# chrischoy/DeepGlobalRegistration

Measured on AMD Instinct MI355X. Metric: pair registrations/sec (FCGF x2 + 1-NN + 6-D inlier net + gate + weighted Procrustes + SE(3) refinement), higher is better.
Workload: dtype f32 results via 2 x f16 split operands (3 f16 MFMA products per MAC, f32 accumulate); k = 1 convs, kNN re-evaluation and registration in exact f32, SVD in f64

## Files before the change

### deepglobalregistration_amd/_lib.py

```python
import ctypes as C
import os
import threading

import torch

_HERE = os.path.dirname(os.path.abspath(__file__))
LIB_PATH = os.environ.get('DGR_HIP_LIB') or os.path.join(_HERE, 'lib', 'libdgr_hip.so')

DGR_OK, DGR_EINVAL, DGR_EHIP, DGR_ENOMEM, DGR_ESVD, DGR_EINTERNAL = 0, -1, -2, -3, -4, -5
STATUS_OK, STATUS_LOW_CONFIDENCE, STATUS_SVD_FAILED, STATUS_SAFEGUARD = 0, 1, 2, 3
STATUS_FLAG_ICP_SKIPPED, STATUS_MASK = 0x100, 0xff

c_i32p, c_i64p, c_f32p, c_f64p = (C.POINTER(C.c_int32), C.POINTER(C.c_int64),
                                  C.POINTER(C.c_float), C.POINTER(C.c_double))
vp = C.c_void_p


class WeightDesc(C.Structure):
    _fields_ = [('name', C.c_char_p), ('data', vp), ('numel', C.c_int64)]


class Params(C.Structure):
    _fields_ = [('clip_weight_thresh', C.c_float), ('voxel_size', C.c_float),
                ('inlier_feature_type', C.c_int), ('max_iter', C.c_int),
                ('max_break_count', C.c_int), ('break_threshold_ratio', C.c_double),
                ('skip_refinement', C.c_int), ('safeguard', C.c_int), ('ransac_hypotheses', C.c_int64),
                ('ransac_seed', C.c_uint32), ('use_icp', C.c_int)]


class PgParams(C.Structure):
    _fields_ = [('mu', C.c_double), ('reference_node', C.c_int), ('max_iter', C.c_int), ('rel_tol', C.c_double)]


SIGNATURES = {
    'dgr_last_error': (C.c_char_p, []),
    'dgr_version': (C.c_char_p, []),
    'dgr_ctx_create': (C.c_int, [C.c_int, C.POINTER(vp)]),
    'dgr_ctx_destroy': (None, [vp]),
    'dgr_ctx_workspace_bytes': (C.c_int64, [vp]),
    'dgr_ctx_create_partition_stream': (C.c_int, [vp, C.c_int, C.c_int, C.POINTER(vp)]),
    'dgr_voxelize': (C.c_int, [vp, vp, C.c_int, C.c_int64, C.c_double, C.c_int32, vp, vp, vp, c_i64p, vp]),
    'dgr_net_create': (C.c_int, [vp, C.c_int, C.c_int, C.c_int, C.c_int, C.c_int,
                                 C.POINTER(WeightDesc), C.c_int, C.POINTER(vp)]),
    'dgr_net_create_device': (C.c_int, [vp, C.c_int, C.c_int, C.c_int, C.c_int, C.c_int,
                                        C.POINTER(WeightDesc), C.c_int, C.POINTER(vp)]),
    'dgr_net_destroy': (None, [vp]),
    'dgr_net_param_bytes': (C.c_int64, [vp]),
    'dgr_net_share': (C.c_int, [vp, vp, C.POINTER(vp)]),
    'dgr_net_sharers': (C.c_int, [vp]),
    'dgr_resunet_forward': (C.c_int, [vp, vp, vp, vp, C.c_int64, vp, vp]),
    'dgr_net_get_intermediate': (C.c_int, [vp, vp, C.c_char_p, vp, C.c_int64, c_i64p, c_i64p]),
    'dgr_net_layer_stats': (C.c_int, [vp, vp, C.c_int, c_i64p]),
    'dgr_net_num_layers': (C.c_int, [vp]),
    'dgr_net_rerun_layer': (C.c_int, [vp, vp, C.c_int, C.c_int, c_f32p, c_f32p]),
    'dgr_maps_create': (C.c_int, [vp, vp, C.c_int64, C.c_int, C.c_int, C.POINTER(vp), vp]),
    'dgr_maps_destroy': (None, [vp]),
    'dgr_maps_get_coords': (C.c_int, [vp, C.c_int, vp, C.c_int64, c_i64p]),
    'dgr_maps_get_kernel_map': (C.c_int, [vp, C.c_int, C.c_int, vp, C.c_int64, vp, vp, C.c_int64,
                                          c_i64p, c_i64p]),
    'dgr_knn1_l2': (C.c_int, [vp, vp, C.c_int64, vp, C.c_int64, C.c_int, C.c_int, vp, vp, vp]),
    'dgr_knn1_l2_batch': (C.c_int, [vp, vp, c_i64p, vp, c_i64p, C.c_int, C.c_int, C.c_int, vp, vp, vp]),
    'dgr_knn_l2': (C.c_int, [vp, vp, C.c_int64, vp, C.c_int64, C.c_int, C.c_int, C.c_int, vp, vp, vp]),
    'dgr_knn_l2_batch': (C.c_int, [vp, vp, c_i64p, vp, c_i64p, C.c_int, C.c_int, C.c_int, C.c_int, vp, vp,
                                   vp]),
    'dgr_inlier_inputs': (C.c_int, [vp, vp, vp, C.c_int64, vp, vp, C.c_int64, vp, C.c_int, vp, vp, vp]),
    'dgr_sigmoid_clip_sum': (C.c_int, [vp, vp, C.c_int64, C.c_float, vp, c_f64p, vp]),
    'dgr_gather_rows3': (C.c_int, [vp, vp, vp, C.c_int64, vp, vp]),
    'dgr_weighted_procrustes': (C.c_int, [vp, vp, vp, vp, C.c_int64, C.c_float, c_f32p, c_f32p, vp]),
    'dgr_se3_refine': (C.c_int, [vp, vp, vp, vp, C.c_int64, C.c_float, C.c_int, C.c_int, C.c_double,
                                 c_f32p, c_f32p, c_i32p, c_f32p, c_i32p, vp]),
    'dgr_register_batch': (C.c_int, [vp, vp, vp, vp, vp, c_i64p, vp, vp, c_i64p, C.c_int,
                                     C.POINTER(Params), vp, vp, c_f32p, c_i32p, c_f32p, vp]),
    'dgr_register_pairs': (C.c_int, [vp, vp, vp, vp, vp, c_i64p, C.c_int, C.c_int, c_i32p, C.c_int,
                                     C.POINTER(Params), vp, vp, c_f32p, c_i32p, c_f32p, vp]),
    'dgr_register_batch_f64': (C.c_int, [vp, c_f64p, C.c_int64, c_i64p]),
    'dgr_register_batch_output': (C.c_int, [vp, C.c_int, vp, C.c_int64, c_i64p, vp]),
    'dgr_ctx_set_profiling': (C.c_int, [vp, C.c_int]),
    'dgr_icp_point_to_point': (C.c_int, [vp, vp, C.c_int64, vp, C.c_int64, C.c_double, c_f64p, C.c_int, C.c_double,
                                          C.c_double, c_f64p, c_f64p, vp]),
    'dgr_ransac_correspondence': (C.c_int, [vp, vp, vp, C.c_int64, C.c_double, C.c_int64, C.c_uint32, c_f64p, c_f64p, vp]),
    'dgr_ctx_stage_times': (C.c_int, [vp, c_f32p]),
    'dgr_ctx_stage_times_v2': (C.c_int, [vp, c_f32p, C.c_int, C.POINTER(C.c_int)]),
    'dgr_ctx_conv_launches': (C.c_int64, [vp]),
    'dgr_ctx_conv_launch_times': (C.c_int, [vp, c_f32p, c_f32p, C.c_int64, C.POINTER(C.c_int64)]),
    'dgr_ctx_conv_launch_kernel_us': (C.c_int, [vp, c_f32p, C.c_int64, C.POINTER(C.c_int64)]),
    'dgr_ctx_conv_launch_kinds': (C.c_int, [vp, C.c_char_p, C.c_int64, C.POINTER(C.c_int64)]),
    'dgr_radius_pairs_batch': (C.c_int, [vp, vp, c_i64p, vp, c_i64p, C.c_int, c_f64p, C.c_double, C.c_int, vp, vp,
                                         C.c_int64, c_i64p, vp]),
    'dgr_pairs_isin_batch': (C.c_int, [vp, vp, c_i64p, vp, c_i64p, C.c_int, c_i64p, vp, vp]),
    'dgr_validation_counts': (C.c_int, [vp, vp, vp, C.c_float, c_i64p, C.c_int, c_i64p, vp]),
    'dgr_score_pairs': (C.c_int, [vp, vp, c_i64p, C.c_int, c_i32p, C.c_int, c_f64p, C.c_double, c_f64p, vp]),
    'dgr_pose_graph_optimize': (C.c_int, [vp, C.c_int, c_i64p, c_i64p, c_i32p, c_f64p, c_f64p, C.POINTER(C.c_uint8), c_f64p,
                                          C.POINTER(PgParams), c_f64p, c_f64p, c_f64p, vp]),
    'dgr_voxel_mean': (C.c_int, [vp, vp, C.c_int, c_i64p, C.c_int, c_i32p, C.c_int, c_f64p, c_f64p, C.c_double, vp, vp, vp, vp,
                                 vp, c_i64p, c_i64p, vp]),
    'dgr_tsdf_fragment': (C.c_int, [vp, vp, C.c_int, C.c_int, C.c_int, c_f64p, c_f64p, c_f64p, C.c_double, C.c_double,
                                    C.c_double, C.c_double, C.c_int, C.c_int, C.c_int, vp, C.c_int64, vp, vp, vp, C.c_int64,
                                    c_i64p, c_i64p, c_i64p, vp]),
    'dgr_debug_ortho2rotation': (C.c_int, [vp, vp, C.c_int64, vp, vp, vp, vp]),
    'dgr_debug_se3_refine_from': (C.c_int, [vp, vp, vp, vp, C.c_int64, C.c_float, C.c_int, C.c_int, C.c_double,
                                            c_f64p, c_f64p, vp]),
    'dgr_debug_smooth_l1': (C.c_int, [vp, vp, vp, C.c_int64, C.c_float, vp, vp]),
    'dgr_debug_conv_layer': (C.c_int, [vp, vp, C.c_int, vp, vp, C.c_int, C.c_int64, vp, vp]),
}

_lib = None


def load():
    global _lib
    if _lib is not None:
        return _lib
    if not os.path.exists(LIB_PATH):
        raise RuntimeError(
            f'{LIB_PATH} not found: the HIP extension is not built.  Run '
            '`python -c "import __graft_entry__ as g; g.build()"` (or `make -C '
            'deepglobalregistration_amd/csrc`).  There is no CPU fallback.')
    lib = C.CDLL(LIB_PATH)
    for name, (res, args) in SIGNATURES.items():
        fn = getattr(lib, name)
        fn.restype = res
        fn.argtypes = args
    _lib = lib
    return lib


class DgrError(RuntimeError):
    def __init__(self, code, message):
        super().__init__(f'libdgr_hip error {code}: {message}')
        self.code = code


class DgrInvalidArgument(DgrError, ValueError):

    def __init__(self, message):
        RuntimeError.__init__(self, f'libdgr_hip: {message}')
        self.code = DGR_EINVAL


def check(rc):
    if rc == DGR_OK:
        return
    msg = load().dgr_last_error().decode('utf-8', 'replace')
    if rc == DGR_EINVAL:
        raise DgrInvalidArgument(msg)
    raise DgrError(rc, msg)


_ctxs = {}
_tls = threading.local()


def new_ctx(device):
    lib = load()
    device = torch.device(device)
    idx = device.index if device.index is not None else torch.cuda.current_device()
    h = vp()
    check(lib.dgr_ctx_create(idx, C.byref(h)))
    return h


def use_ctx(handle):
    _tls.ctx = handle


def get_ctx(device=None):
    lib = load()
    if getattr(_tls, 'ctx', None) is not None:
        return _tls.ctx
    if not torch.cuda.is_available():
        raise RuntimeError('deepglobalregistration_amd needs a ROCm GPU (torch.cuda.is_available() is '
                           'False); there is no CPU fallback')
    if device is None:
        idx = torch.cuda.current_device()
    else:
        device = torch.device(device)
        if device.type != 'cuda':
            raise RuntimeError(f'deepglobalregistration_amd runs on the GPU only, got device {device}')
        idx = device.index if device.index is not None else torch.cuda.current_device()
    if idx not in _ctxs:
        h = vp()
        check(lib.dgr_ctx_create(idx, C.byref(h)))
        _ctxs[idx] = h
    return _ctxs[idx]


def stream_ptr(device_index=None):
    return vp(torch.cuda.current_stream(device_index).cuda_stream)


def ptr(t):
    if t is None:
        return vp(0)
    assert t.is_contiguous(), 'tensor must be contiguous'
    return vp(t.data_ptr())
```

### deepglobalregistration_amd/csrc/conv_dense.hip

```cpp
#include "dgr_internal.h"
#include "split.h"

typedef float f32x4 __attribute__((ext_vector_type(4)));
typedef float f32x2 __attribute__((ext_vector_type(2)));
typedef int i32x4 __attribute__((ext_vector_type(4)));
typedef _Float16 f16x8 __attribute__((ext_vector_type(8)));
typedef _Float16 f16x2 __attribute__((ext_vector_type(2)));
typedef unsigned int u32x2 __attribute__((ext_vector_type(2)));
typedef unsigned int u32x4 __attribute__((ext_vector_type(4)));

#ifndef DGR_DENSE_RG
#define DGR_DENSE_RG 2
#endif
#ifndef DGR_DENSE_RG32
#define DGR_DENSE_RG32 2
#endif
#ifndef DGR_DENSE_WD
#define DGR_DENSE_WD 8
#endif
struct ConvDenseArgs {
  const float *in;
  float *out;
  const float *shift, *res;
  const u32x4 *wb;
  int64_t piece_stride;
  const int32_t *nbr, *n_out_dev;
  int64_t n_pad;
  int in_ld, in_relu, out_ld, out_relu, res_ld, res_relu;
  const uint32_t *row_amax;
  uint32_t *out_amax, *out_amax2;
  float w_unscale;
  uint32_t in_bytes;
  const unsigned char *in_ds;
  unsigned char *out_ds;
};

template <int CIN, int COUT, int RG, int WAVES, bool PS>
__global__ void __launch_bounds__(64 * WAVES, 2) sparse_conv_dense_f16x2(ConvDenseArgs a) {
  constexpr int KV = 27;
  constexpr int S = CIN / 32, NCB = COUT / 16;
  constexpr int THREADS = 64 * WAVES;
  constexpr int MB = WAVES * RG * 16;
  constexpr int NST = S * NCB;
  constexpr int WD = NST >= 8 ? DGR_DENSE_WD : NST >= 4 ? 4 : 2;
  static_assert(NST % WD == 0, "the weight ring turns a whole number of times per offset (static register indexing)");
  __shared__ int nbr_s[KV][MB];

  const int tid = threadIdx.x, lane = tid & 63;
  const int wave = __builtin_amdgcn_readfirstlane(tid >> 6);
  const int n_out = *a.n_out_dev;
  const int nblocks = (n_out + MB - 1) / MB;
  const int per = (nblocks + 7) >> 3;
  const int j = blockIdx.x >> 3;
  const int blk = (blockIdx.x & 7) * per + j;
  if (j >= per || blk >= nblocks) return;
  const int64_t row0 = (int64_t)blk * MB;

  u32x4 rh[WD], rm[WD];
  const u32x4 *wph = a.wb + lane, *wpm = a.wb + a.piece_stride + lane;
  auto wreq = [&](int g, int i) {
    const int gc = min(g, KV * NST - 1);
    const int k = gc / NST, jj = gc - k * NST;
    const int gg = k * NST + (jj % S) * NCB + jj / S;
    rh[i] = wph[(int64_t)gg * 64];
    rm[i] = wpm[(int64_t)gg * 64];
  };
  for (int e = tid; e < KV * MB; e += THREADS) {
    const int k = e / MB, r = e - k * MB;
    nbr_s[k][r] = (row0 + r < n_out) ? a.nbr[(int64_t)k * a.n_pad + row0 + r] : -1;
  }
  const int lr = lane & 15, lq = lane >> 4;
  f32x4 total[RG][NCB];
#pragma unroll
  for (int cb = 0; cb < NCB; ++cb) {
    const f32x4 sh = a.shift ? *reinterpret_cast<const f32x4 *>(a.shift + 16 * cb + 4 * lq) : f32x4{0.f, 0.f, 0.f, 0.f};
#pragma unroll
    for (int rg = 0; rg < RG; ++rg) {
      f32x4 v = sh;
      const int64_t row = row0 + (wave * RG + rg) * 16 + lr;
      if (a.res && row < n_out) {
        f32x4 x = *reinterpret_cast<const f32x4 *>(a.res + row * a.res_ld + 16 * cb + 4 * lq);
        if (a.res_relu) { x.x = fmaxf(x.x, 0.f); x.y = fmaxf(x.y, 0.f); x.z = fmaxf(x.z, 0.f); x.w = fmaxf(x.w, 0.f); }
        v += x;
      }
      total[rg][cb] = v;
    }
  }
  __syncthreads();

  const __amdgpu_buffer_rsrc_t in_rsrc = __builtin_amdgcn_make_buffer_rsrc(
      PS ? (void *)const_cast<unsigned char *>(a.in_ds) : (void *)const_cast<float *>(a.in), 0, a.in_bytes, 0x00020000);
  struct RowSet { f32x4 raw[RG][S][2]; uint32_t mx[RG]; int nv[RG]; };
  auto gather = [&](int k, RowSet &g) {
#pragma unroll
    for (int rg = 0; rg < RG; ++rg) {
      const int n = nbr_s[k][(wave * RG + rg) * 16 + (lane >> 2)];
      const int ne = max(n, 0);
      const uint32_t off = n >= 0 ? (uint32_t)n * (uint32_t)((PS ? CIN : a.in_ld) * 4) + 16u * (lane & 3) : a.in_bytes;
      const uint32_t mv = a.row_amax[ne];
#pragma unroll
      for (int s = 0; s < S; ++s) {
        if constexpr (PS) {
          g.raw[rg][s][0] = __builtin_bit_cast(f32x4, __builtin_amdgcn_raw_buffer_load_b128(in_rsrc, off + 64 * s, 0, 0));
          g.raw[rg][s][1] = __builtin_bit_cast(f32x4, __builtin_amdgcn_raw_buffer_load_b128(in_rsrc, off + 2 * CIN + 64 * s, 0, 0));
        } else {
          g.raw[rg][s][0] = __builtin_bit_cast(f32x4, __builtin_amdgcn_raw_buffer_load_b128(in_rsrc, off + 128 * s, 0, 0));
          g.raw[rg][s][1] = __builtin_bit_cast(f32x4, __builtin_amdgcn_raw_buffer_load_b128(in_rsrc, off + 128 * s + 64, 0, 0));
        }
      }
      g.mx[rg] = mv;
      g.nv[rg] = n;
    }
  };
  constexpr int DEPTH = 1;
  static_assert(DEPTH == 1 || DEPTH == 2, "prefetch depth");
  RowSet gA, gB;
  gather(0, gA);
  if (DEPTH == 2) gather(1, gB);
#pragma unroll
  for (int i = 0; i < WD; ++i) wreq(i, i);
  const int relu_lo = a.in_relu ? 0 : (int)0x80000000;

  auto body = [&](int k, RowSet &g) {
    f16x8 bh[RG][S], bm[RG][S];
    float fold[RG];
    const int from = 4 * (4 * (lane & 15) + (lane >> 4));
#pragma unroll
    for (int rg = 0; rg < RG; ++rg) {
      const float sx = g.nv[rg] >= 0 ? dgr_row_scale_of(g.mx[rg]) : 0.f;
      const float fl = sx != 0.f ? dgr_inv_pow2(sx) * a.w_unscale : 0.f;
      fold[rg] = __builtin_bit_cast(float, __builtin_amdgcn_ds_bpermute(16 * (lane & 15), __builtin_bit_cast(int, fl)));
#pragma unroll
      for (int s = 0; s < S; ++s) {
        i32x4 hw, mw;
        if constexpr (PS) {
          hw = __builtin_bit_cast(i32x4, g.raw[rg][s][0]);
          mw = __builtin_bit_cast(i32x4, g.raw[rg][s][1]);
        } else
#pragma unroll
        for (int h = 0; h < 2; ++h) {
          const i32x4 v = __builtin_bit_cast(i32x4, g.raw[rg][s][h]);
#pragma unroll
          for (int u = 0; u < 4; u += 2) {
            const f32x2 xs = f32x2{__builtin_bit_cast(float, max(v[u], relu_lo)), __builtin_bit_cast(float, max(v[u + 1], relu_lo))} * sx;
            const f16x2 hh = __builtin_convertvector(xs, f16x2);
            const f16x2 mm = __builtin_convertvector(xs - __builtin_convertvector(hh, f32x2), f16x2);
            hw[2 * h + u / 2] = __builtin_bit_cast(int, hh);
            mw[2 * h + u / 2] = __builtin_bit_cast(int, mm);
          }
        }
#pragma unroll
        for (int d = 0; d < 4; ++d) {
          hw[d] = __builtin_amdgcn_ds_bpermute(from, hw[d]);
          mw[d] = __builtin_amdgcn_ds_bpermute(from, mw[d]);
        }
        bh[rg][s] = __builtin_bit_cast(f16x8, hw);
        bm[rg][s] = __builtin_bit_cast(f16x8, mw);
      }
    }
    __builtin_amdgcn_sched_barrier(0);
    gather(min(k + DEPTH, KV - 1), g);
    __builtin_amdgcn_sched_barrier(0);
    f32x4 prev[RG];
#pragma unroll
    for (int cb = 0; cb < NCB; ++cb) {
      f32x4 tmp[RG];
#pragma unroll
      for (int rg = 0; rg < RG; ++rg) tmp[rg] = f32x4{0.f, 0.f, 0.f, 0.f};
#pragma unroll
      for (int s = 0; s < S; ++s) {
        const int j = cb * S + s;
        const f16x8 wh = __builtin_bit_cast(f16x8, rh[j % WD]);
        const f16x8 wm = __builtin_bit_cast(f16x8, rm[j % WD]);
#pragma unroll
        for (int rg = 0; rg < RG; ++rg) tmp[rg] = __builtin_amdgcn_mfma_f32_16x16x32_f16(wm, bh[rg][s], tmp[rg], 0, 0, 0);
#pragma unroll
        for (int rg = 0; rg < RG; ++rg) tmp[rg] = __builtin_amdgcn_mfma_f32_16x16x32_f16(wh, bm[rg][s], tmp[rg], 0, 0, 0);
#pragma unroll
        for (int rg = 0; rg < RG; ++rg) tmp[rg] = __builtin_amdgcn_mfma_f32_16x16x32_f16(wh, bh[rg][s], tmp[rg], 0, 0, 0);
        wreq(k * NST + j + WD, j % WD);
        if (s == 0 && cb > 0) {
#pragma unroll
          for (int rg = 0; rg < RG; ++rg) total[rg][cb - 1] += prev[rg] * fold[rg];
        }
        __builtin_amdgcn_sched_barrier(0);
      }
#pragma unroll
      for (int rg = 0; rg < RG; ++rg) prev[rg] = tmp[rg];
    }
#pragma unroll
    for (int rg = 0; rg < RG; ++rg) total[rg][NCB - 1] += prev[rg] * fold[rg];
  };
  if (DEPTH == 1) {
#pragma unroll 1
    for (int k = 0; k < KV; ++k) body(k, gA);
  } else {
#pragma unroll 1
    for (int k = 0; k < KV - 1; k += 2) {
      body(k, gA);
      body(k + 1, gB);
    }
    body(KV - 1, gA);
  }

  const float out_lo = a.out_relu ? 0.f : -__builtin_inff();
  const int out_relu_lo = a.out_relu ? 0 : (int)0x80000000;
#pragma unroll
  for (int rg = 0; rg < RG; ++rg) {
    const int64_t row = row0 + (wave * RG + rg) * 16 + lr;
    uint32_t mx = 0;
#pragma unroll
    for (int cb = 0; cb < NCB; ++cb) {
      f32x4 v = total[rg][cb];
      v.x = fmaxf(v.x, out_lo); v.y = fmaxf(v.y, out_lo); v.z = fmaxf(v.z, out_lo); v.w = fmaxf(v.w, out_lo);
      total[rg][cb] = v;
      if (row < n_out) {
        if (a.out) *reinterpret_cast<f32x4 *>(a.out + row * a.out_ld + 16 * cb + 4 * lq) = v;
        const i32x4 b = __builtin_bit_cast(i32x4, v);
        mx = max(mx, max(max((uint32_t)b.x & 0x7fffffffu, (uint32_t)b.y & 0x7fffffffu), max((uint32_t)b.z & 0x7fffffffu, (uint32_t)b.w & 0x7fffffffu)));
      }
    }
    if (a.out_amax || a.out_amax2 || a.out_ds) {
      mx = max(mx, (uint32_t)__shfl_xor((int)mx, 16, 64));
      mx = max(mx, (uint32_t)__shfl_xor((int)mx, 32, 64));
      if (lq == 0 && row < n_out) {
        if (a.out_amax) atomicMax(a.out_amax + row, mx);
        if (a.out_amax2) atomicMax(a.out_amax2 + row, mx);
      }
    }
    if (a.out_ds && row < n_out) {
      const float sx = dgr_row_scale_of(mx);
      unsigned char *dst = a.out_ds + row * (int64_t)(4 * COUT) + 16 * lq;
#pragma unroll
      for (int s = 0; s < COUT / 32; ++s) {
        u32x4 hw, mw;
#pragma unroll
        for (int h = 0; h < 2; ++h) {
          const i32x4 v = __builtin_bit_cast(i32x4, total[rg][2 * s + h]);
#pragma unroll
          for (int u = 0; u < 4; u += 2) {
            const f32x2 xs = f32x2{__builtin_bit_cast(float, max(v[u], out_relu_lo)), __builtin_bit_cast(float, max(v[u + 1], out_relu_lo))} * sx;
            const f16x2 hh = __builtin_convertvector(xs, f16x2);
            const f16x2 mm = __builtin_convertvector(xs - __builtin_convertvector(hh, f32x2), f16x2);
            hw[2 * h + u / 2] = __builtin_bit_cast(uint32_t, hh);
            mw[2 * h + u / 2] = __builtin_bit_cast(uint32_t, mm);
          }
        }
        *reinterpret_cast<u32x4 *>(dst + 64 * s) = hw;
        *reinterpret_cast<u32x4 *>(dst + 2 * COUT + 64 * s) = mw;
      }
    }
  }
}

bool dgr_conv_dense_supported(int cin, int cin_pad, int cout) {
  return cin == cin_pad && (cin == 32 || cin == 64) && (cout == 32 || cout == 64);
}

template <int CIN, int COUT>
static int launch_dense(const ConvDenseArgs &ka, int64_t n_out_cap, hipStream_t stream) {
  constexpr int RG = (CIN == 32 && COUT == 32) ? DGR_DENSE_RG32 : DGR_DENSE_RG, WAVES = 4, MB = WAVES * RG * 16;
  int64_t blocks = dgr_ceil_div(n_out_cap, MB);
  blocks = (blocks + 7) / 8 * 8;
  if (ka.in_ds)
    sparse_conv_dense_f16x2<CIN, COUT, RG, WAVES, true><<<(unsigned)blocks, 64 * WAVES, 0, stream>>>(ka);
  else
    sparse_conv_dense_f16x2<CIN, COUT, RG, WAVES, false><<<(unsigned)blocks, 64 * WAVES, 0, stream>>>(ka);
  DGR_LAUNCH_CHECK();
  return DGR_OK;
}

int dgr_conv_dense_launch(const DgrConvOsLaunch &a, hipStream_t stream, const char **kernel_name) {
  DGR_REQUIRE(a.nbr && a.nbr->built && a.nbr->K == 27, "dense-tile conv: no neighbour table");
  DGR_REQUIRE(dgr_conv_dense_supported(a.cin, a.cin_pad, a.cout), "dense-tile conv: Cin = %d, Cout = %d not built", a.cin, a.cout);
  DGR_REQUIRE(a.wbd && a.row_amax, "dense-tile conv: needs the split weights in its operand order and the input rows' maxima");
  DGR_REQUIRE((a.in_ld & 3) == 0 && (a.out_ld & 3) == 0 && (a.res == nullptr || (a.res_ld & 3) == 0),
              "dense-tile conv: row strides must be multiples of 4");
  ConvDenseArgs ka;
  ka.in = a.in; ka.out = a.out; ka.shift = a.shift; ka.res = a.res;
  ka.wb = static_cast<const u32x4 *>(a.wbd); ka.piece_stride = a.piece_stride;
  ka.nbr = a.nbr->nbr; ka.n_out_dev = a.n_out_dev; ka.n_pad = a.nbr->n_pad;
  ka.in_ld = a.in_ld; ka.in_relu = a.in_relu; ka.out_ld = a.out_ld; ka.out_relu = a.out_relu;
  ka.res_ld = a.res_ld; ka.res_relu = a.res_relu;
  ka.row_amax = a.row_amax; ka.w_unscale = a.w_unscale;
  ka.out_amax = a.out_amax; ka.out_amax2 = a.out_amax2;
  ka.in_ds = a.in_dsplit; ka.out_ds = a.out_dsplit;
  DGR_REQUIRE(a.out || a.out_dsplit, "dense-tile conv: no output");
  DGR_REQUIRE(a.n_in_cap > 0 && a.n_in_cap * (int64_t)a.in_ld * 4 < (1ll << 31), "dense-tile conv: input tensor beyond 2 GB");
  ka.in_bytes = (uint32_t)(a.n_in_cap * (int64_t)(a.in_dsplit ? a.cin : a.in_ld) * 4);
#define DGR_DENSE(CI, CO)                                                                   \
  if (a.cin == CI && a.cout == CO) {                                                        \
    if (kernel_name) *kernel_name = a.in_dsplit ? "sparse_conv_dense_f16x2<" #CI ", " #CO ", ps>" : "sparse_conv_dense_f16x2<" #CI ", " #CO ">"; \
    return launch_dense<CI, CO>(ka, a.n_out_cap, stream);                                   \
  }
  DGR_DENSE(32, 32) DGR_DENSE(32, 64) DGR_DENSE(64, 32) DGR_DENSE(64, 64)
#undef DGR_DENSE
  return DGR_EINVAL;
}
```

### deepglobalregistration_amd/csrc/conv_os.hip

```cpp
#include <stdlib.h>

#include <type_traits>

#include "dgr_internal.h"
#include "split.h"

typedef float f32x4 __attribute__((ext_vector_type(4)));
typedef int i32x4 __attribute__((ext_vector_type(4)));
typedef unsigned int u32x2 __attribute__((ext_vector_type(2)));
typedef __bf16 bf16x8 __attribute__((ext_vector_type(8)));
typedef _Float16 f16x8 __attribute__((ext_vector_type(8)));
typedef _Float16 f16x2 __attribute__((ext_vector_type(2)));

#ifdef DGR_OS_STAGE_CLK
__device__ unsigned long long dgr_os_stage_clk[8];
#define DGR_OS_CLK(i) do { if (threadIdx.x == 0) { const unsigned long long t_ = __builtin_amdgcn_s_memrealtime(); atomicAdd(&dgr_os_stage_clk[i], t_ - t_prev); t_prev = t_; } } while (0)
extern "C" int dgr_debug_os_stage_clk(unsigned long long *out8, int reset) {
  if (out8 && hipMemcpyFromSymbol(out8, HIP_SYMBOL(dgr_os_stage_clk), 8 * sizeof(unsigned long long)) != hipSuccess) return -1;
  if (reset) { unsigned long long z[8] = {0, 0, 0, 0, 0, 0, 0, 0}; if (hipMemcpyToSymbol(HIP_SYMBOL(dgr_os_stage_clk), z, sizeof(z)) != hipSuccess) return -1; }
  return 0;
}
#else
#define DGR_OS_CLK(i) do { } while (0)
#endif
// ... 5 lines not shown
  int64_t piece_stride;
  const int32_t *nbr, *n_out_dev;
  int64_t n_pad;
  int in_ld, in_relu, out_ld, out_relu, res_ld, res_relu;
  int cin, cout, nb16;
  const uint32_t *row_amax;
  float w_unscale;
  uint32_t *out_amax, *out_amax2;
};

template <int CP, int CS, int MB, int CK, int TM, int PM, int GW>
__global__ void __launch_bounds__(CS * 4 * (TM / 16 / GW)) sparse_conv_os(ConvOsArgs a) {
  constexpr bool BF3 = PM != 0;
  static_assert(PM == 0 || PM == 2, "arithmetic mode");
  constexpr int NP = PM == 0 ? 1 : 2;
  constexpr int GP = TM / 16;
  constexpr int NCW = CS / 16;
  constexpr int NWR = GP / GW;
  static_assert(GP % GW == 0, "groups per wave must divide the groups per tile");
  constexpr int NW = NCW * NWR;
  constexpr int THREADS = 64 * NW;
  constexpr int KV = 27;
  constexpr int PPT = CP / CK;
  constexpr int LDA = CK + 4, LDC = CS + 4;
  constexpr int C4K = CK / 4;
  constexpr int NCH = (TM * C4K + THREADS - 1) / THREADS;
  constexpr bool PIECE_GUARD = TM * C4K % THREADS != 0;
  constexpr int G = CK / 16;
  constexpr int GT = CP / 16;
  constexpr int KPW = (KV + NW - 1) / NW;
  constexpr int NGMAX = KV * ((MB / 16 + GP - 1) / GP * GP) + GP;
  static_assert(CP % CK == 0, "shape");
  constexpr int LDP = CK + 8;
  constexpr int PLANE = TM * LDP;
  constexpr int G32 = CK / 32;
  constexpr int ABYTES = BF3 ? 2 * NP * PLANE * 2 : 2 * TM * LDA * 4;
  __shared__ __attribute__((aligned(16))) char abuf[ABYTES];
  float (*As)[TM][LDA] = reinterpret_cast<float (*)[TM][LDA]>(abuf);
  unsigned short *Ps = reinterpret_cast<unsigned short *>(abuf);
  __shared__ __attribute__((aligned(16))) float acc_s[MB][LDC];
  __shared__ int in_idx[KV][MB];
  __shared__ float in_scale[PM == 2 ? KV : 1][MB];
  __shared__ unsigned char out_loc[KV][MB];
  __shared__ int cnt[KV];
  __shared__ int grp[NGMAX + GP];
  __shared__ int n_grp;

  const int tid = threadIdx.x;
  const int lane = tid & 63;
  const int wave = __builtin_amdgcn_readfirstlane(tid >> 6);
  const int cw = wave % NCW;
  const int rb0 = (wave / NCW) * GW;
  const int n_out = *a.n_out_dev;
  const int nblocks = (n_out + MB - 1) / MB;
  const int per = (nblocks + 7) >> 3;
  const int j = blockIdx.x >> 3;
  const int blk = (blockIdx.x & 7) * per + j;
  if (j >= per || blk >= nblocks) return;
  const int slice = blockIdx.y;
  const int64_t row0 = (int64_t)blk * MB;
#ifdef DGR_OS_STAGE_CLK
  unsigned long long t_prev = __builtin_amdgcn_s_memrealtime();
#endif

  if constexpr (PM == 2)
    for (int e = tid; e < KV * MB; e += THREADS) (&in_scale[0][0])[e] = 1.f;
  __syncthreads();
  {
    int v[KPW];
#pragma unroll
    for (int u = 0; u < KPW; ++u) {
      const int k = wave + u * NW;
      v[u] = (k < KV && lane < MB) ? a.nbr[(int64_t)k * a.n_pad + row0 + lane] : -1;
    }
#pragma unroll
    for (int u = 0; u < KPW; ++u) {
      const int k = wave + u * NW;
      if (k < KV) {
        const unsigned long long m = __ballot(v[u] >= 0);
        if (v[u] >= 0) {
          const int pos = __popcll(m & ((1ull << lane) - 1ull));
          in_idx[k][pos] = v[u];
          out_loc[k][pos] = (unsigned char)lane;
          if constexpr (PM == 2) in_scale[k][pos] = dgr_row_scale_of(a.row_amax[v[u]]);
        }
        if (lane == 0) cnt[k] = __popcll(m);
      }
    }
  }
  DGR_OS_CLK(0);
  for (int e = tid; e < MB * (CS / 4); e += THREADS) {
    const int r = e / (CS / 4), c = (e % (CS / 4)) * 4;
    f32x4 v = a.shift ? *reinterpret_cast<const f32x4 *>(a.shift + slice * CS + c) : f32x4{0.f, 0.f, 0.f, 0.f};
    if (a.res && row0 + r < n_out) {
      f32x4 x = *reinterpret_cast<const f32x4 *>(a.res + (row0 + r) * a.res_ld + slice * CS + c);
      if (a.res_relu) { x.x = fmaxf(x.x, 0.f); x.y = fmaxf(x.y, 0.f); x.z = fmaxf(x.z, 0.f); x.w = fmaxf(x.w, 0.f); }
      v += x;
    }
    *reinterpret_cast<f32x4 *>(&acc_s[r][c]) = v;
  }
  __syncthreads();
  if (wave == 0) {
    const int c = lane < KV ? cnt[lane] : 0;
    const int ng = NWR > 1 ? (((c + 15) >> 4) + GP - 1) / GP * GP : ((c + 15) >> 4);
    int x = ng;
#pragma unroll
    for (int d = 1; d < 32; d <<= 1) {
      const int y = __shfl_up(x, d, 64);
      if (lane >= d) x += y;
    }
    const int first = x - ng;
    for (int u = 0; u < ng; ++u) grp[first + u] = lane | ((16 * u) << 8) | (max(0, min(16, c - 16 * u)) << 16);
    if (lane == KV - 1) {
      n_grp = x;
      for (int u = 0; u < GP; ++u) grp[x + u] = 0;
    }
  }
  __syncthreads();
  const int NG = n_grp;
  const int NT = (NG + GP - 1) / GP;
  const int NQ = NT * PPT;
  DGR_OS_CLK(1);

  f32x4 Gr[NCH];
  auto gather = [&](int q) {
    const int t = q / PPT, cbase = (q % PPT) * CK;
#pragma unroll
    for (int i = 0; i < NCH; ++i) {
      const int ch = PIECE_GUARD ? min(tid + i * THREADS, TM * C4K - 1) : tid + i * THREADS;
      const int r = ch / C4K, c = cbase + (ch % C4K) * 4;
      const int info = grp[GP * t + (r >> 4)];
      const int row = in_idx[info & 255][((info >> 8) & 255) + (r & 15)];
      const uint32_t off = (uint32_t)(((r & 15) < (info >> 16)) ? row : 0) * (uint32_t)a.in_ld + (uint32_t)c;
      Gr[i] = *reinterpret_cast<const f32x4 *>(a.in + off);
    }
  };
  const int relu_lo = a.in_relu ? 0 : (int)0x80000000;
  auto land = [&](int q) {
#pragma unroll
    for (int i = 0; i < NCH; ++i) {
      const int ch = tid + i * THREADS;
      if (PIECE_GUARD && ch >= TM * C4K) continue;
      i32x4 v = __builtin_bit_cast(i32x4, Gr[i]);
      v.x = max(v.x, relu_lo); v.y = max(v.y, relu_lo); v.z = max(v.z, relu_lo); v.w = max(v.w, relu_lo);
      if constexpr (!BF3) {
        *reinterpret_cast<i32x4 *>(&As[q & 1][0][0] + (ch / C4K) * LDA + (ch % C4K) * 4) = v;
      } else {
        const int r = ch / C4K;
        const int info = grp[GP * (min(q, NQ - 1) / PPT) + (r >> 4)];
        const float sx = in_scale[info & 255][min(((info >> 8) & 255) + (r & 15), MB - 1)];
        _Float16 hh[4], mm[4];
#pragma unroll
        for (int u = 0; u < 4; ++u) {
          const int vi = v[u];
          const float xs = __builtin_bit_cast(float, vi) * sx;
          hh[u] = (_Float16)xs;
          mm[u] = (_Float16)(xs - (float)hh[u]);
        }
        unsigned short *dst = Ps + (q & 1) * NP * PLANE + r * LDP + (ch % C4K) * 4;
        *reinterpret_cast<u32x2 *>(dst) = u32x2{__builtin_bit_cast(uint32_t, f16x2{hh[0], hh[1]}),
                                                __builtin_bit_cast(uint32_t, f16x2{hh[2], hh[3]})};
        *reinterpret_cast<u32x2 *>(dst + PLANE) = u32x2{__builtin_bit_cast(uint32_t, f16x2{mm[0], mm[1]}),
                                                        __builtin_bit_cast(uint32_t, f16x2{mm[2], mm[3]})};
      }
    }
  };
  const int jb = slice * NCW + cw;
  constexpr int WREGS = BF3 ? NP * G32 : G;
  struct WSet { uint4 v[WREGS]; };
  auto wstep = [&](int qq, int u, WSet &w) {
    const int q = min(qq, NQ - 1);
    const int k = __builtin_amdgcn_readfirstlane(grp[GP * (q / PPT) + rb0 + u]) & 255;
    if constexpr (!BF3) {
      const uint4 *p = reinterpret_cast<const uint4 *>(a.w16) + (int64_t)jb * 64 + lane + (int64_t)(k * GT + (q % PPT) * G) * a.nb16 * 64;
#pragma unroll
      for (int g = 0; g < G; ++g) w.v[g] = p[(int64_t)g * a.nb16 * 64];
    } else {
      const uint4 *p = a.wb3 + (int64_t)jb * 64 + lane + (int64_t)(k * (CP / 32) + (q % PPT) * G32) * a.nb16 * 64;
#pragma unroll
      for (int g = 0; g < G32; ++g)
#pragma unroll
        for (int pc = 0; pc < NP; ++pc) w.v[NP * g + pc] = p[(int64_t)pc * a.piece_stride + (int64_t)g * a.nb16 * 64];
    }
  };

  f32x4 acc[GW];
  WSet w[GW];
  auto mfma_group = [&](int u, int buf) {
    const int rb = rb0 + u;
    if constexpr (!BF3) {
      const float *arow = &As[buf][lane & 15][4 * (lane >> 4)];
#pragma unroll
      for (int g = 0; g < G; ++g) {
        const f32x4 av = *reinterpret_cast<const f32x4 *>(arow + rb * 16 * LDA + g * 16);
        const f32x4 wv = __builtin_bit_cast(f32x4, w[u].v[g]);
#pragma unroll
        for (int c = 0; c < 4; ++c) acc[u] = __builtin_amdgcn_mfma_f32_16x16x4f32(wv[c], av[c], acc[u], 0, 0, 0);
      }
    } else {
      const unsigned short *prow = Ps + buf * NP * PLANE + (rb * 16 + (lane & 15)) * LDP + 8 * (lane >> 4);
#pragma unroll
      for (int g = 0; g < G32; ++g) {
        const f16x8 ah = __builtin_bit_cast(f16x8, *reinterpret_cast<const uint4 *>(prow + 32 * g));
        const f16x8 am = __builtin_bit_cast(f16x8, *reinterpret_cast<const uint4 *>(prow + PLANE + 32 * g));
        const f16x8 wh = __builtin_bit_cast(f16x8, w[u].v[2 * g]), wm = __builtin_bit_cast(f16x8, w[u].v[2 * g + 1]);
        acc[u] = __builtin_amdgcn_mfma_f32_16x16x32_f16(wm, ah, acc[u], 0, 0, 0);
        acc[u] = __builtin_amdgcn_mfma_f32_16x16x32_f16(wh, am, acc[u], 0, 0, 0);
        acc[u] = __builtin_amdgcn_mfma_f32_16x16x32_f16(wh, ah, acc[u], 0, 0, 0);
      }
    }
  };
  if (NQ > 0) {
    gather(0);
#pragma unroll
    for (int u = 0; u < GW; ++u) wstep(0, u, w[u]);
    land(0);
    gather(NQ > 1 ? 1 : 0);
  }
  __syncthreads();

  for (int q = 0; q < NQ; ++q) {
    const int t = q / PPT, h = q % PPT;
    land(q + 1);
    gather(min(q + 2, NQ - 1));
    if (PPT == 1 || h == 0) {
#pragma unroll
      for (int u = 0; u < GW; ++u) acc[u] = f32x4{0.f, 0.f, 0.f, 0.f};
    }
#pragma unroll
    for (int u = 0; u < GW; ++u) {
      const int n_rows = __builtin_amdgcn_readfirstlane(grp[GP * t + rb0 + u]) >> 16;
      __builtin_amdgcn_sched_barrier(0);
      if (u == 0 || n_rows > 0) mfma_group(u, q & 1);
      wstep(q + 1, u, w[u]);
    }
    if (PPT == 1 || h == PPT - 1) {
#pragma unroll
      for (int u = 0; u < GW; ++u) {
        const int info = grp[GP * t + rb0 + u];
        if ((lane & 15) < (info >> 16)) {
          const int e = ((info >> 8) & 255) + (lane & 15);
          float *p = &acc_s[out_loc[info & 255][e]][16 * cw + 4 * (lane >> 4)];
          f32x4 v = *reinterpret_cast<f32x4 *>(p);
          if constexpr (PM == 2) {
            const float f = __builtin_bit_cast(float, 0x7f000000u - __builtin_bit_cast(uint32_t, in_scale[info & 255][e])) * a.w_unscale;
            v += acc[u] * f;
          } else {
            v += acc[u];
          }
          *reinterpret_cast<f32x4 *>(p) = v;
        }
      }
    }
    __syncthreads();
  }
  DGR_OS_CLK(2);
#ifdef DGR_OS_STAGE_CLK
  if (threadIdx.x == 0) { atomicAdd(&dgr_os_stage_clk[4], 1ull); atomicAdd(&dgr_os_stage_clk[5], (unsigned long long)NQ); }
#endif
  const float out_lo = a.out_relu ? 0.f : -__builtin_inff();
  static_assert(MB * (CS / 4) % THREADS == 0 || THREADS % (CS / 4) == 0, "row lanes stay inside a wave");
  for (int e0 = 0; e0 < MB * (CS / 4); e0 += THREADS) {
    const int e = e0 + tid;
    const bool live = e < MB * (CS / 4);
    const int r = live ? e / (CS / 4) : 0, c = (e % (CS / 4)) * 4;
    uint32_t mx = 0;
    if (live && row0 + r < n_out) {
      f32x4 v = *reinterpret_cast<const f32x4 *>(&acc_s[r][c]);
      v.x = fmaxf(v.x, out_lo); v.y = fmaxf(v.y, out_lo); v.z = fmaxf(v.z, out_lo); v.w = fmaxf(v.w, out_lo);
      *reinterpret_cast<f32x4 *>(a.out + (row0 + r) * a.out_ld + slice * CS + c) = v;
      const i32x4 b = __builtin_bit_cast(i32x4, v);
      mx = max(max((uint32_t)b.x & 0x7fffffffu, (uint32_t)b.y & 0x7fffffffu), max((uint32_t)b.z & 0x7fffffffu, (uint32_t)b.w & 0x7fffffffu));
    }
    if (a.out_amax || a.out_amax2) {
#pragma unroll
      for (int d = CS / 8; d >= 1; d >>= 1) mx = max(mx, (uint32_t)__shfl_xor((int)mx, d, 64));
      if (live && (e % (CS / 4)) == 0 && row0 + r < n_out) {
        if (a.out_amax) atomicMax(a.out_amax + row0 + r, mx);
        if (a.out_amax2) atomicMax(a.out_amax2 + row0 + r, mx);
      }
    }
  }
  DGR_OS_CLK(3);
}

template <int CP, int CS, int MB, int CK, int TM>
static int launch_os(const ConvOsArgs &ka, int64_t n_out_cap, hipStream_t stream) {
  constexpr int GW = (MB >= 64 && CP <= 64) ? 1 : TM / 16;
  int64_t blocks = dgr_ceil_div(n_out_cap, MB);
  blocks = (blocks + 7) / 8 * 8;
  dim3 grid((unsigned)blocks, (unsigned)(ka.cout / CS));
  constexpr int threads = CS * 4 * (TM / 16 / GW);
  if (ka.wb3 && ka.row_amax)
    sparse_conv_os<CP, CS, MB, CK, TM, 2, GW><<<grid, threads, 0, stream>>>(ka);
  else
    sparse_conv_os<CP, CS, MB, CK, TM, 0, GW><<<grid, threads, 0, stream>>>(ka);
  DGR_LAUNCH_CHECK();
  return DGR_OK;
}

int dgr_conv_os_launch(const DgrConvOsLaunch &a, hipStream_t stream, const char **kernel_name) {
  if (a.dense) return dgr_conv_dense_launch(a, stream, kernel_name);
  if (a.up) return dgr_conv_up_launch(a, stream, kernel_name);
  DGR_REQUIRE(a.nbr && a.nbr->built && a.nbr->K == 27, "output-stationary conv: no neighbour table");
  DGR_REQUIRE((a.cin & 3) == 0 && (a.in_ld & 3) == 0 && (a.out_ld & 3) == 0 && (a.res == nullptr || (a.res_ld & 3) == 0),
              "output-stationary conv: channel counts and row strides must be multiples of 4");
  DGR_REQUIRE(a.cout % 32 == 0 && a.cin == a.cin_pad, "output-stationary conv: Cin = %d, Cout = %d must be multiples of 32",
              a.cin, a.cout);
  DGR_REQUIRE(a.n_in_cap > 0 && a.n_in_cap * (int64_t)a.in_ld < (1ll << 32) / 4 * 4,
              "output-stationary conv: input tensor beyond 32-bit element offsets");
  ConvOsArgs ka;
  ka.in = a.in; ka.out = a.out; ka.w16 = a.w16; ka.shift = a.shift; ka.res = a.res;
  ka.wb3 = dgr_exact_f32() ? nullptr : static_cast<const uint4 *>(a.wb3);
  ka.piece_stride = a.piece_stride;
  ka.row_amax = ka.wb3 ? a.row_amax : nullptr;
  ka.w_unscale = a.w_unscale;
  ka.out_amax = a.out_amax; ka.out_amax2 = a.out_amax2;
  DGR_REQUIRE(!ka.wb3 || ka.row_amax, "output-stationary conv: the split weights need the input rows' maxima");
  ka.nbr = a.nbr->nbr; ka.n_out_dev = a.n_out_dev; ka.n_pad = a.nbr->n_pad;
  ka.in_ld = a.in_ld; ka.in_relu = a.in_relu; ka.out_ld = a.out_ld; ka.out_relu = a.out_relu;
  ka.res_ld = a.res_ld; ka.res_relu = a.res_relu;
  ka.cin = a.cin; ka.cout = a.cout; ka.nb16 = a.cout / 16;
#define DGR_OS_TM 32
#define DGR_OS_MBBIG 64
#define DGR_STR2(x) #x
#define DGR_STR(x) DGR_STR2(x)
#define DGR_OS(CPV, CSV, MBV, CKV)                                                                      \
  do {                                                                                                  \
    constexpr int tm = (MBV) < DGR_OS_TM ? ((MBV) < 32 ? 32 : (MBV)) : DGR_OS_TM;                       \
    if (kernel_name) *kernel_name = ka.row_amax ? "sparse_conv_os<" #CPV ", " #CSV ", " DGR_STR(MBV) ", " DGR_STR(CKV) ", f16x2>"  \
                                                 : "sparse_conv_os<" #CPV ", " #CSV ", " DGR_STR(MBV) ", " DGR_STR(CKV) ", f32>"; \
    return launch_os<CPV, CSV, MBV, CKV, tm>(ka, a.n_out_cap, stream);                                  \
  } while (0)
  const int mb = a.rows_per_block;
  const bool narrow = a.cout == 32;
#define DGR_OS_MB(CPV, CKV)                                                 \
  do {                                                                      \
    if (narrow) { DGR_OS(CPV, 32, DGR_OS_MBBIG, CKV); }                     \
    else if (mb == 64) { DGR_OS(CPV, 64, DGR_OS_MBBIG, CKV); }              \
    else if (mb == 32) { DGR_OS(CPV, 64, 32, CKV); }                        \
    else { DGR_OS(CPV, 64, 16, CKV); }                                      \
  } while (0)
  const bool ck128 = a.phase_channels == 128;
  switch (a.cin_pad) {
    case 32: DGR_OS_MB(32, 32);
    case 64: DGR_OS_MB(64, 64);
    case 128: if (ck128) DGR_OS_MB(128, 128); else DGR_OS_MB(128, 64);
    case 256: if (ck128) DGR_OS_MB(256, 128); else DGR_OS_MB(256, 64);
    default: break;
  }
#undef DGR_OS_MB
#undef DGR_OS
  dgr_set_error("output-stationary conv: no instantiation for Cin (padded) %d", a.cin_pad);
  return DGR_EINVAL;
}
```

### deepglobalregistration_amd/csrc/conv_up.hip

```cpp
#include "dgr_internal.h"
#include "split.h"

typedef float f32x4 __attribute__((ext_vector_type(4)));
typedef float f32x2 __attribute__((ext_vector_type(2)));
typedef int i32x4 __attribute__((ext_vector_type(4)));
typedef _Float16 f16x8 __attribute__((ext_vector_type(8)));
typedef _Float16 f16x2 __attribute__((ext_vector_type(2)));
typedef unsigned int u32x4 __attribute__((ext_vector_type(4)));

struct ConvUpArgs {
  const float *in;
  float *out;
  const float *shift;
  const u32x4 *wb;
  int64_t piece_stride;
  const int32_t *nbr;
  int64_t n_pad;
  const int32_t *perm, *cls_count;
  int64_t cls_cap;
  int in_ld, in_relu, out_ld, out_relu;
  int nb16;
  const uint32_t *row_amax;
  uint32_t *out_amax, *out_amax2;
  float w_unscale;
  uint32_t in_bytes;
};

template <int CIN, int RG, int WAVES>
__global__ void __launch_bounds__(64 * WAVES, 2) sparse_conv_up_f16x2(ConvUpArgs a) {
  constexpr int NCB = 4;
  constexpr int NCH = CIN / 64;
  constexpr int S_T = CIN / 32;
  constexpr int THREADS = 64 * WAVES;
  constexpr int MB = WAVES * RG * 16;
  constexpr int NST = 2 * NCB;
  constexpr int WD = NST;
  __shared__ int nbr_s[8][MB];
  __shared__ int rows_s[MB];

  const int tid = threadIdx.x, lane = tid & 63;
  const int wave = __builtin_amdgcn_readfirstlane(tid >> 6);
  const int slice = blockIdx.y;
  int cls = -1, lb = 0, n_cls = 0;
  {
    int b = blockIdx.x;
#pragma unroll
    for (int c = 0; c < 8; ++c) {
      const int n = a.cls_count[c];
      const int nb = (n + MB - 1) / MB;
      if (cls < 0 && b < nb) { cls = c; lb = b; n_cls = n; }
      b -= nb;
    }
  }
  if (cls < 0) return;
  unsigned long long kpack = 0;
  int NL = 0;
  for (int k = 0; k < 27; ++k) {
    const int dx = k % 3 - 1, dy = (k / 3) % 3 - 1, dz = k / 9 - 1;
    if ((dx != 0) == ((cls & 1) != 0) && (dy != 0) == ((cls & 2) != 0) && (dz != 0) == ((cls & 4) != 0)) {
      kpack |= (unsigned long long)k << (5 * NL);
      ++NL;
    }
  }
  auto k_of = [&](int li) { return (int)((kpack >> (5 * li)) & 31ull); };
  const int NIT = NL * NCH;

  for (int i = tid; i < MB; i += THREADS) {
    const int64_t idx = (int64_t)lb * MB + i;
    rows_s[i] = idx < n_cls ? a.perm[(int64_t)cls * a.cls_cap + idx] : -1;
  }
  __syncthreads();
  for (int e = tid; e < NL * MB; e += THREADS) {
    const int li = e / MB, i = e - li * MB;
    const int r = rows_s[i];
    nbr_s[li][i] = r >= 0 ? a.nbr[(int64_t)k_of(li) * a.n_pad + r] : -1;
  }

  u32x4 rh[WD], rm[WD];
  const u32x4 *wph = a.wb + lane, *wpm = a.wb + a.piece_stride + lane;
  auto wreq = [&](int g, int i) {
    const int gc = min(g, NIT * NST - 1);
    const int it = gc / NST, jj = gc - it * NST;
    const int li = it / NCH, ch = it - li * NCH;
    const int64_t frag = ((int64_t)k_of(li) * S_T + 2 * ch + (jj & 1)) * a.nb16 + slice * NCB + (jj >> 1);
    rh[i] = wph[frag * 64];
    rm[i] = wpm[frag * 64];
  };
  const int lr = lane & 15, lq = lane >> 4;
  f32x4 total[RG][NCB];
#pragma unroll
  for (int cb = 0; cb < NCB; ++cb) {
    const f32x4 sh = a.shift ? *reinterpret_cast<const f32x4 *>(a.shift + 64 * slice + 16 * cb + 4 * lq) : f32x4{0.f, 0.f, 0.f, 0.f};
#pragma unroll
    for (int rg = 0; rg < RG; ++rg) total[rg][cb] = sh;
  }
  __syncthreads();

  const __amdgpu_buffer_rsrc_t in_rsrc = __builtin_amdgcn_make_buffer_rsrc(const_cast<float *>(a.in), 0, a.in_bytes, 0x00020000);
  struct RowSet { f32x4 raw[RG][2][2]; uint32_t mx[RG]; int nv[RG]; };
  auto gather = [&](int it, RowSet &g) {
    const int li = it / NCH, ch = it - li * NCH;
#pragma unroll
    for (int rg = 0; rg < RG; ++rg) {
      const int n = nbr_s[li][(wave * RG + rg) * 16 + (lane >> 2)];
      const int ne = max(n, 0);
      const uint32_t off = n >= 0 ? (uint32_t)n * (uint32_t)(a.in_ld * 4) + 256u * ch + 16u * (lane & 3) : a.in_bytes;
      const uint32_t mv = a.row_amax[ne];
#pragma unroll
      for (int s = 0; s < 2; ++s) {
        g.raw[rg][s][0] = __builtin_bit_cast(f32x4, __builtin_amdgcn_raw_buffer_load_b128(in_rsrc, off + 128 * s, 0, 0));
        g.raw[rg][s][1] = __builtin_bit_cast(f32x4, __builtin_amdgcn_raw_buffer_load_b128(in_rsrc, off + 128 * s + 64, 0, 0));
      }
      g.mx[rg] = mv;
      g.nv[rg] = n;
    }
  };
  RowSet gA;
  gather(0, gA);
#pragma unroll
  for (int i = 0; i < WD; ++i) wreq(i, i);
  const int relu_lo = a.in_relu ? 0 : (int)0x80000000;

  f32x4 tmp[RG][NCB];
#pragma unroll 1
  for (int it = 0; it < NIT; ++it) {
    const int ch = it % NCH;
    f16x8 bh[RG][2], bm[RG][2];
    float fold[RG];
    const int from = 4 * (4 * (lane & 15) + (lane >> 4));
#pragma unroll
    for (int rg = 0; rg < RG; ++rg) {
      const float sx = gA.nv[rg] >= 0 ? dgr_row_scale_of(gA.mx[rg]) : 0.f;
      const float fl = sx != 0.f ? dgr_inv_pow2(sx) * a.w_unscale : 0.f;
      fold[rg] = __builtin_bit_cast(float, __builtin_amdgcn_ds_bpermute(16 * (lane & 15), __builtin_bit_cast(int, fl)));
#pragma unroll
      for (int s = 0; s < 2; ++s) {
        i32x4 hw, mw;
#pragma unroll
        for (int h = 0; h < 2; ++h) {
          const i32x4 v = __builtin_bit_cast(i32x4, gA.raw[rg][s][h]);
#pragma unroll
          for (int u = 0; u < 4; u += 2) {
            const f32x2 xs = f32x2{__builtin_bit_cast(float, max(v[u], relu_lo)), __builtin_bit_cast(float, max(v[u + 1], relu_lo))} * sx;
            const f16x2 hh = __builtin_convertvector(xs, f16x2);
            const f16x2 mm = __builtin_convertvector(xs - __builtin_convertvector(hh, f32x2), f16x2);
            hw[2 * h + u / 2] = __builtin_bit_cast(int, hh);
            mw[2 * h + u / 2] = __builtin_bit_cast(int, mm);
          }
        }
#pragma unroll
        for (int d = 0; d < 4; ++d) {
          hw[d] = __builtin_amdgcn_ds_bpermute(from, hw[d]);
          mw[d] = __builtin_amdgcn_ds_bpermute(from, mw[d]);
        }
        bh[rg][s] = __builtin_bit_cast(f16x8, hw);
        bm[rg][s] = __builtin_bit_cast(f16x8, mw);
      }
    }
    __builtin_amdgcn_sched_barrier(0);
    gather(min(it + 1, NIT - 1), gA);
    __builtin_amdgcn_sched_barrier(0);
    if (ch == 0) {
#pragma unroll
      for (int rg = 0; rg < RG; ++rg)
#pragma unroll
        for (int cb = 0; cb < NCB; ++cb) tmp[rg][cb] = f32x4{0.f, 0.f, 0.f, 0.f};
    }
#pragma unroll
    for (int cb = 0; cb < NCB; ++cb) {
#pragma unroll
      for (int s = 0; s < 2; ++s) {
        const int j = cb * 2 + s;
        const f16x8 wh = __builtin_bit_cast(f16x8, rh[j]);
        const f16x8 wm = __builtin_bit_cast(f16x8, rm[j]);
#pragma unroll
        for (int rg = 0; rg < RG; ++rg) tmp[rg][cb] = __builtin_amdgcn_mfma_f32_16x16x32_f16(wm, bh[rg][s], tmp[rg][cb], 0, 0, 0);
#pragma unroll
        for (int rg = 0; rg < RG; ++rg) tmp[rg][cb] = __builtin_amdgcn_mfma_f32_16x16x32_f16(wh, bm[rg][s], tmp[rg][cb], 0, 0, 0);
#pragma unroll
        for (int rg = 0; rg < RG; ++rg) tmp[rg][cb] = __builtin_amdgcn_mfma_f32_16x16x32_f16(wh, bh[rg][s], tmp[rg][cb], 0, 0, 0);
        wreq((it + 1) * NST + j, j);
        __builtin_amdgcn_sched_barrier(0);
      }
    }
    if (ch == NCH - 1) {
#pragma unroll
      for (int rg = 0; rg < RG; ++rg)
#pragma unroll
        for (int cb = 0; cb < NCB; ++cb) total[rg][cb] += tmp[rg][cb] * fold[rg];
    }
  }

  const float out_lo = a.out_relu ? 0.f : -__builtin_inff();
#pragma unroll
  for (int rg = 0; rg < RG; ++rg) {
    const int64_t row = rows_s[(wave * RG + rg) * 16 + lr];
    uint32_t mx = 0;
    if (row >= 0) {
#pragma unroll
      for (int cb = 0; cb < NCB; ++cb) {
        f32x4 v = total[rg][cb];
        v.x = fmaxf(v.x, out_lo); v.y = fmaxf(v.y, out_lo); v.z = fmaxf(v.z, out_lo); v.w = fmaxf(v.w, out_lo);
        *reinterpret_cast<f32x4 *>(a.out + row * a.out_ld + 64 * slice + 16 * cb + 4 * lq) = v;
        const i32x4 b = __builtin_bit_cast(i32x4, v);
        mx = max(mx, max(max((uint32_t)b.x & 0x7fffffffu, (uint32_t)b.y & 0x7fffffffu), max((uint32_t)b.z & 0x7fffffffu, (uint32_t)b.w & 0x7fffffffu)));
      }
    }
    if (a.out_amax || a.out_amax2) {
      mx = max(mx, (uint32_t)__shfl_xor((int)mx, 16, 64));
      mx = max(mx, (uint32_t)__shfl_xor((int)mx, 32, 64));
      if (lq == 0 && row >= 0) {
        if (a.out_amax) atomicMax(a.out_amax + row, mx);
        if (a.out_amax2) atomicMax(a.out_amax2 + row, mx);
      }
    }
  }
}

bool dgr_conv_up_supported(int cin, int cin_pad, int cout) {
  return cin == cin_pad && (cin == 128 || cin == 256) && cout % 64 == 0 && cout >= 64;
}

int dgr_conv_up_launch(const DgrConvOsLaunch &a, hipStream_t stream, const char **kernel_name) {
  DGR_REQUIRE(a.nbr && a.nbr->built && a.nbr->K == 27 && a.nbr->perm && a.nbr->cls_count,
              "parity-class transposed conv: no neighbour table with a class row list");
  DGR_REQUIRE(dgr_conv_up_supported(a.cin, a.cin_pad, a.cout), "parity-class transposed conv: Cin = %d, Cout = %d not built", a.cin, a.cout);
  DGR_REQUIRE(a.wbd && a.row_amax, "parity-class transposed conv: needs the split weights in the dense-tile operand order and the input rows' maxima");
  DGR_REQUIRE(a.res == nullptr, "parity-class transposed conv: no residual input");
  DGR_REQUIRE((a.in_ld & 3) == 0 && (a.out_ld & 3) == 0, "parity-class transposed conv: row strides must be multiples of 4");
  DGR_REQUIRE(a.n_in_cap > 0 && a.n_in_cap * (int64_t)a.in_ld * 4 < (1ll << 31), "parity-class transposed conv: input tensor beyond 2 GB");
  ConvUpArgs ka;
  ka.in = a.in; ka.out = a.out; ka.shift = a.shift;
  ka.wb = static_cast<const u32x4 *>(a.wbd); ka.piece_stride = a.piece_stride;
  ka.nbr = a.nbr->nbr; ka.n_pad = a.nbr->n_pad;
  ka.perm = a.nbr->perm; ka.cls_count = a.nbr->cls_count; ka.cls_cap = a.nbr->cls_cap;
  ka.in_ld = a.in_ld; ka.in_relu = a.in_relu; ka.out_ld = a.out_ld; ka.out_relu = a.out_relu;
  ka.nb16 = a.cout / 16;
  ka.row_amax = a.row_amax; ka.out_amax = a.out_amax; ka.out_amax2 = a.out_amax2;
  ka.w_unscale = a.w_unscale;
  ka.in_bytes = (uint32_t)(a.n_in_cap * (int64_t)a.in_ld * 4);
  constexpr int RG = 2, WAVES = 4, MB = WAVES * RG * 16;
  const dim3 grid((unsigned)(dgr_ceil_div(a.n_out_cap, MB) + 8), (unsigned)(a.cout / 64));
  if (a.cin == 128) {
    if (kernel_name) *kernel_name = "sparse_conv_up_f16x2<128>";
    sparse_conv_up_f16x2<128, RG, WAVES><<<grid, 64 * WAVES, 0, stream>>>(ka);
  } else {
    if (kernel_name) *kernel_name = "sparse_conv_up_f16x2<256>";
    sparse_conv_up_f16x2<256, RG, WAVES><<<grid, 64 * WAVES, 0, stream>>>(ka);
  }
  DGR_LAUNCH_CHECK();
  return DGR_OK;
}
```

### deepglobalregistration_amd/csrc/dgr_internal.h

```cpp
#pragma once
#include <hip/hip_runtime.h>
#include <stdint.h>
#include <stdio.h>
#include <stdlib.h>
#include <string>
#include <vector>

#include "../../include/dgr_hip.h"

void dgr_set_error(const char *fmt, ...);

#define DGR_HIP_CHECK(expr)                                                                  \
  do {                                                                                       \
    hipError_t _e = (expr);                                                                  \
    if (_e != hipSuccess) {                                                                  \
      dgr_set_error("%s:%d: %s failed: %s", __FILE__, __LINE__, #expr, hipGetErrorString(_e)); \
      return DGR_EHIP;                                                                       \
    }                                                                                        \
  } while (0)

#define DGR_CHECK(expr)          \
  do {                           \
    int _r = (expr);             \
    if (_r != DGR_OK) return _r; \
  } while (0)

#define DGR_REQUIRE(cond, ...)     \
  do {                             \
    if (!(cond)) {                 \
      dgr_set_error(__VA_ARGS__);  \
      return DGR_EINVAL;           \
    }                              \
  } while (0)

#define DGR_LAUNCH_CHECK() DGR_HIP_CHECK(hipGetLastError())

inline bool dgr_exact_f32() {
  static const bool on = getenv("DGR_EXACT_F32") != nullptr;
  return on;
}

struct DgrArena {
  struct Chunk {
    char *base;
    size_t size;
  };
  std::vector<Chunk> chunks;
  size_t cur = 0;
  size_t offset = 0;
  size_t high_water = 0, used_total = 0;
  uint64_t generation = 0;

  struct Mark {
    size_t cur, offset, used_total;
  };
  Mark mark() const { return {cur, offset, used_total}; }
  void rewind(const Mark &m) { cur = m.cur; offset = m.offset; used_total = m.used_total; }
  void *alloc(size_t bytes);
  int reset();
  void release();
  size_t reserved() const;
  template <typename T>
  T *get(size_t n) {
    return static_cast<T *>(alloc(n * sizeof(T)));
  }
};

#define DGR_ALLOC(ptr, arena, T, n)                       \
  do {                                                    \
    (ptr) = (arena).get<T>((size_t)(n) > 0 ? (size_t)(n) : 1); \
    if (!(ptr)) return DGR_ENOMEM;                        \
  } while (0)

constexpr int DGR_TILE_M = 64;

struct DgrCoordMap {
  int32_t *coords = nullptr;
  int32_t *n_dev = nullptr;
  int64_t n_cap = 0;
  int ts = 1;
  int32_t *table = nullptr;
  uint32_t table_mask = 0;
  int32_t *canon = nullptr;
};

struct DgrHalfBuckets {
  int32_t *bkeys = nullptr;
  int32_t *table = nullptr;
  uint32_t mask = 0;
  int32_t *start = nullptr;
  int4 *second = nullptr;
  bool built = false;
};

struct DgrKernelMap {
  int K = 0;
  int32_t *rule_ptr = nullptr;
  int32_t *tile_ptr = nullptr;
  int4 *tile_desc = nullptr;
  int64_t tile_cap = 0;
  int32_t *pair_in = nullptr;
  int32_t *pair_out = nullptr;
  int32_t *out_ptr = nullptr, *out_pos = nullptr;
  uint16_t *pair_k = nullptr;
  int32_t *in_ptr = nullptr, *in_pos = nullptr;
  int64_t pair_cap = 0;
  bool built = false;
};

constexpr int DGR_OS_ROWS = 64;
struct DgrNbrTable {
  int32_t *nbr = nullptr;
  int64_t n_pad = 0;
  int K = 27;
  bool built = false;
  int32_t *perm = nullptr, *cls_count = nullptr;
  int64_t cls_cap = 0;
};

struct DgrMapSet {
  int D = 3, nc = 4, conv1_ks = 3;
  bool use_nbr = false;
  DgrNbrTable nsame[4];
  DgrNbrTable ndown[3];
  DgrNbrTable nup[3];
  DgrCoordMap cm[4];
  DgrHalfBuckets hb[4];
  DgrKernelMap same[4];
  DgrKernelMap conv1;
  DgrKernelMap down[3];
  int32_t *overflow = nullptr;
};

int dgr_build_maps(DgrArena &arena, const int32_t *coords, int64_t N, int D, int conv1_ks,
                   DgrMapSet *ms, hipStream_t stream, bool skip_conv1_map = false, bool lean = false,
                   bool nbr_tables = false);
int dgr_nbr_counts(const DgrNbrTable &t, const int32_t *n_out_dev, int64_t counts[27]);
int dgr_conv1_probe(DgrArena &arena, const DgrCoordMap &cm, int ks, const float *in, int in_ld, int cin,
                    const float *w_tiled, const float *shift, float *out, int out_ld, int32_t *pair_count,
                    hipStream_t stream, const float *w_compact = nullptr, const char **kernel_name = nullptr,
                    uint32_t *out_amax = nullptr);
int dgr_unique_rows(DgrArena &arena, const int32_t *keys, int64_t n, int nc, int32_t *first_flag,
                    int32_t *rank, int32_t *n_unique_dev, int32_t **table_out, uint32_t *mask_out,
                    hipStream_t stream);
int dgr_exclusive_scan_i32(DgrArena &arena, const int32_t *in, int32_t *out, int64_t n,
                           int32_t *total_out, hipStream_t stream);
constexpr int DGR_SCAN_MAX = 24;
int dgr_exclusive_scan_multi(DgrArena &arena, int count, const int32_t *const *in, int32_t *const *out, const int64_t *n,
                             int32_t *const *total_out, hipStream_t stream);

struct DgrConvLaunch {
  const float *in;
  int in_ld;
  int in_relu;
  float *out;
  int out_ld;
  float *y;
  const float *shift;
  const float *w;
  int cin, cin_pad, cout, cout_pad, K;
  const int32_t *pair_in, *pair_out, *tile_ptr, *rule_ptr;
  const int4 *tile_desc;
  const int32_t *n_rows_dev;
  int64_t tile_bound;
  int l2_normalize = 0;
  unsigned long long *clk = nullptr;
};
int dgr_conv_launch(const DgrConvLaunch &a, int num_cus, hipStream_t stream, const char **kernel_name = nullptr);
struct DgrSplitRows {
  unsigned char *planes = nullptr;
  float *scale = nullptr;
  int channels = 0;
};
bool dgr_conv_wide_supported(int cin_pad, int cin, int cout);
int dgr_conv_wide_launch(const DgrConvLaunch &a, const DgrSplitRows &in, const void *wb, int64_t piece_stride,
                         float w_unscale, int num_cus, hipStream_t stream, const char **kernel_name = nullptr);
int dgr_row_amax(const float *in, int in_ld, int cin, int relu, const int32_t *n_dev, int64_t n_cap, uint32_t *out,
                 hipStream_t stream);
int dgr_split_rows(const float *in, int in_ld, int relu, const int32_t *n_dev, int64_t n_cap, const DgrSplitRows &out,
                   hipStream_t stream);
int dgr_reduce_rows(const float *y, int cout, const int32_t *ptr, const int32_t *pos, const int32_t *n_dev,
                    int64_t n_cap, float *out, int out_ld, const float *shift, const float *res, int res_ld,
                    int res_relu, hipStream_t stream, const DgrSplitRows *split = nullptr, int out_relu = 0);
int dgr_conv_small_cin(const float *in, int in_ld, int in_relu, int cin, const float *w_tiled, const float *w_quad,
                       const float *shift, const DgrKernelMap &km, const int32_t *n_out_dev, int64_t n_out_cap, float *out,
                       int out_ld, hipStream_t stream);
struct DgrConvOsLaunch {
  const float *in; int in_ld, in_relu;
  float *out; int out_ld, out_relu;
  const float *w16, *shift;
  const void *wb3; int64_t piece_stride;
  const void *wbd = nullptr;
  const uint32_t *row_amax = nullptr; float w_unscale = 1.f;
  uint32_t *out_amax = nullptr, *out_amax2 = nullptr;
  int64_t n_in_cap = 0;
  const float *res; int res_ld, res_relu;
  int rows_per_block;
  int phase_channels = 64;
  const DgrNbrTable *nbr;
  const int32_t *n_out_dev;
  int64_t n_out_cap;
  int cin, cin_pad, cout;
  bool dense = false;
  bool up = false;
  const unsigned char *in_dsplit = nullptr;
  unsigned char *out_dsplit = nullptr;
};
int dgr_conv_os_launch(const DgrConvOsLaunch &a, hipStream_t stream, const char **kernel_name = nullptr);
bool dgr_conv_dense_supported(int cin, int cin_pad, int cout);
int dgr_conv_dense_launch(const DgrConvOsLaunch &a, hipStream_t stream, const char **kernel_name = nullptr);
bool dgr_conv_up_supported(int cin, int cin_pad, int cout);
int dgr_conv_up_launch(const DgrConvOsLaunch &a, hipStream_t stream, const char **kernel_name = nullptr);
int dgr_l2_normalize_rows(const float *in, int in_ld, float *out, int out_ld, int c, int relu,
                          const int32_t *n_dev, int64_t n_cap, hipStream_t stream);

struct DgrBatchOutputs {
  const void *ptr[5] = {nullptr, nullptr, nullptr, nullptr, nullptr};
  int64_t numel[5] = {0, 0, 0, 0, 0};
  uint64_t generation = 0;
};

struct DgrEventPool {
  std::vector<hipEvent_t> ev;
  size_t used = 0;
  hipEvent_t next();
  void release();
};

struct dgr_ctx {
  int device = 0;
  int num_cus = 256;
  DgrArena arena;
  bool profiling = false;
  float stage_ms[9] = {0, 0, 0, 0, 0, 0, 0, 0, 0};
  int64_t conv_launches = 0;
  DgrBatchOutputs last;
  std::vector<double> last_T64;
  DgrEventPool events;
  std::vector<std::pair<hipEvent_t, hipEvent_t>> conv_spans, gemm_spans, map3_spans, map6_spans;
  std::vector<float> conv_span_ms, gemm_span_ms;
  std::vector<unsigned long long *> conv_clks;
  std::vector<float> conv_clk_us;
  std::vector<const char *> conv_kinds;
  int32_t *flag_dev = nullptr;
  hipEvent_t wait_ev = nullptr;
  long last_wait_ns = 0;
  double batch_ns_per_row = 0;
  double pairs_ns_per_row = 0;
  unsigned char *pin = nullptr;
  size_t pin_bytes = 0;
  hipStream_t part_stream = nullptr;
  int all_cus = 256;
};

int dgr_ctx_pinned(dgr_ctx *ctx, size_t bytes, unsigned char **out);
int dgr_flag_error(int32_t flag);

int dgr_ctx_wait(dgr_ctx *ctx, hipStream_t stream, long predicted_ns = 0);

int dgr_resunet_forward_impl(dgr_ctx *ctx, dgr_net *net, const int32_t *coords, const float *feats,
                             int64_t N, float *out, hipStream_t stream);
int dgr_ctx_collect_profile(dgr_ctx *ctx);
void dgr_ctx_begin_profile(dgr_ctx *ctx);

int dgr_knn1_batch_impl(dgr_ctx *ctx, const float *F0, const int64_t *off0, const float *F1, const int64_t *off1,
                        int npairs, int C, int squared, int64_t *idx_out, float *dist_out, hipStream_t stream);
int dgr_knn1_impl(dgr_ctx *ctx, const float *F0, int64_t N0, const float *F1, int64_t N1, int C,
                  int squared, int64_t *idx_out, float *dist_out, hipStream_t stream);
int dgr_inlier_inputs_impl(const int32_t *coords0, const float *xyz0, int64_t N0,
                           const int32_t *coords1, const float *xyz1, const int64_t *idx1,
                           int feature_type, int32_t *coords6, float *feats, hipStream_t stream);
int dgr_icp_impl(dgr_ctx *ctx, const float *src, int64_t N0, const float *dst, int64_t N1, double max_dist,
                 const double *T_init, int max_iter, double rel_fitness, double rel_rmse, double *T_out,
                 double *stats_out, hipStream_t stream);
int dgr_ransac_impl(dgr_ctx *ctx, const float *X, const float *Y, int64_t N, double max_dist, int64_t num_hypotheses,
                    uint32_t seed, double *T_out, double *stats_out, hipStream_t stream);
struct DgrIcpJob {
  const float *src = nullptr, *dst = nullptr;
  int64_t N0 = 0, N1 = 0;
  double max_dist = 0;
  int nblocks = 0;
  void *st = nullptr;
  double *P = nullptr, *sorted = nullptr, *partial = nullptr;
  int32_t ncell = 0;
  double host_state[64];
};
int dgr_icp_begin(dgr_ctx *ctx, const float *src, int64_t N0, const float *dst, int64_t N1, double max_dist,
                  const double *T_init_dev , DgrIcpJob *job, hipStream_t stream);
int dgr_icp_run(dgr_ctx *ctx, DgrIcpJob *job, int max_iter, double rel_fitness, double rel_rmse, hipStream_t stream);
void dgr_icp_finish(const DgrIcpJob *job, double *T_out, double *stats_out);
constexpr int DGR_RANSAC_RESULT_DOUBLES = 19;
int dgr_ransac_begin(dgr_ctx *ctx, const float *X, const float *Y, int64_t N, double max_dist, int64_t num_hypotheses,
                     uint32_t seed, double **result_dev, hipStream_t stream);
struct DgrRegResult {
  float R[9];
  float t[3];
  float loss;
  float wsum;
  int32_t iterations;
  int32_t break_count;
  int32_t status;
  int32_t pad;
};
static inline int64_t dgr_ceil_div(int64_t a, int64_t b) { return (a + b - 1) / b; }
static inline uint32_t dgr_next_pow2(uint64_t v) {
  uint32_t p = 1;
  while (p < v) p <<= 1;
  return p;
}
```

### deepglobalregistration_amd/csrc/net.hip

```cpp
#include <math.h>
#include <stdlib.h>
#include <string.h>

#include <algorithm>
#include <map>
#include <memory>
#include <string>

#include "dgr_internal.h"

static const int CH[5] = {0, 32, 64, 128, 256};
static const int TR[5] = {0, 64, 64, 64, 128};
static constexpr float BN_EPS = 1e-5f;

struct DgrLayer {
  std::string name;
  int K, cin, cout, cin_pad, cout_pad;
  float *w = nullptr;
  float *w16 = nullptr;
  void *w16b = nullptr;
  void *w16d = nullptr;
  int64_t w16b_piece = 0;
  float *wc = nullptr;
  float *wq = nullptr;
  void *wb = nullptr;
  int64_t wb_piece = 0;
  float w_unscale = 1.f;
  float *shift = nullptr;
};

struct LayerRun {
  const int32_t *rule_ptr = nullptr;
  const int32_t *n_in = nullptr, *n_out = nullptr;
  int K = 1;
  DgrConvLaunch launch;
  DgrSplitRows split_in, split_out;
  int out_relu = 0;
  bool split_only = false;
  bool small_cin = false;
  const int32_t *fused_pairs = nullptr;
  bool os = false;
  DgrConvOsLaunch os_launch;
  DgrNbrTable nbr;
  DgrKernelMap km;
  bool has_reduce = false;
  const int32_t *red_ptr = nullptr, *red_pos = nullptr;
  int64_t n_out_cap = 0;
  const float *res = nullptr;
  int res_ld = 0, res_relu = 0;
};

struct DgrTensorRef {
  const float *ptr = nullptr;
  int ld = 0, cols = 0;
  const int32_t *n_dev = nullptr;
  const int32_t *canon = nullptr;
};

struct DgrWeights {
  std::vector<DgrLayer> layers;
  std::vector<void *> allocs;
  int64_t param_bytes = 0;
  int device = 0;
  template <class T> int alloc(T **p, size_t n) {
    DGR_HIP_CHECK(hipMalloc((void **)p, n * sizeof(T)));
    allocs.push_back(*p);
    return DGR_OK;
  }
  ~DgrWeights() {
    int cur = -1;
    (void)hipGetDevice(&cur);
    (void)hipSetDevice(device);
    (void)hipDeviceSynchronize();
    for (void *p : allocs) (void)hipFree(p);
    if (cur >= 0 && cur != device) (void)hipSetDevice(cur);
  }
};

struct dgr_net {
  dgr_ctx *ctx;
  int D, cin, cout, conv1_ks, normalize;
  std::shared_ptr<DgrWeights> W;
  LayerRun runs[23];
  std::map<std::string, DgrTensorRef> inter;
  uint64_t run_generation = 0;
};

static int round_up(int v, int m) { return (v + m - 1) / m * m; }

static const dgr_weight_desc *find_desc(const dgr_weight_desc *w, int n, const std::string &name) {
  for (int i = 0; i < n; ++i)
    if (name == w[i].name) return &w[i];
  return nullptr;
}

template <class F>
__global__ void __launch_bounds__(256) dgr_fill_kernel(int64_t n, F f) {
  for (int64_t o = (int64_t)blockIdx.x * 256 + threadIdx.x; o < n; o += (int64_t)gridDim.x * 256) f(o);
}
template <class F>
static int dgr_fill(hipStream_t s, int64_t n, F f) {
  if (n <= 0) return DGR_OK;
  const int64_t blocks = std::min<int64_t>((n + 255) / 256, 1 << 16);
  dgr_fill_kernel<<<(int)blocks, 256, 0, s>>>(n, f);
  DGR_LAUNCH_CHECK();
  return DGR_OK;
}
__device__ __forceinline__ uint16_t dgr_f16_bits_dev(float x) {
  const _Float16 h = (_Float16)x;
  return __builtin_bit_cast(uint16_t, h);
}
__device__ __forceinline__ float dgr_f16_val_dev(float x) { return (float)(_Float16)x; }
__global__ void __launch_bounds__(256) dgr_absmax_scaled_kernel(const float *__restrict__ w, const float *__restrict__ scale,
                                                                int64_t n, int cout, uint32_t *out_bits) {
  float mx = 0.f;
  for (int64_t o = (int64_t)blockIdx.x * 256 + threadIdx.x; o < n; o += (int64_t)gridDim.x * 256)
    mx = fmaxf(mx, fabsf(__fmul_rn(w[o], scale[o % cout])));
  for (int d = 32; d > 0; d >>= 1) mx = fmaxf(mx, __shfl_xor(mx, d, 64));
  if ((threadIdx.x & 63) == 0) atomicMax(out_bits, __float_as_uint(mx));
}

struct WeightPrep {
  bool dev;
  hipStream_t s = nullptr;
  float *sc = nullptr;
  uint32_t *mxb = nullptr;
  float *staging = nullptr;
  size_t staging_n = 0;
  ~WeightPrep() {
    if (s) (void)hipStreamSynchronize(s);
    (void)hipFree(sc); (void)hipFree(mxb); (void)hipFree(staging);
    if (s) (void)hipStreamDestroy(s);
  }
};

static int make_layer(dgr_net *net, WeightPrep &P, const dgr_weight_desc *descs, int nd, const std::string &name, int K,
                      int cin, int cout, const char *bn, bool bias) {
  DgrLayer L;
  L.name = name;
  L.K = K; L.cin = cin; L.cout = cout;
  L.cin_pad = round_up(cin, 8);
  L.cout_pad = cout <= 32 ? 32 : cout <= 64 ? 64 : cout <= 128 ? 128 : 256;
  if (L.cout_pad == 32 && L.cin_pad > 8) {
    DGR_REQUIRE(cin <= 64, "%s: %d input channels (at most 64 into a 32-channel layer)", name.c_str(), cin);
    L.cin_pad = cin <= 32 ? 32 : 64;
  }
  DGR_REQUIRE(cout <= 256 && cin <= 256, "%s: channel count above 256 not supported", name.c_str());
  const dgr_weight_desc *kd = find_desc(descs, nd, name + ".kernel");
  DGR_REQUIRE(kd != nullptr, "state_dict is missing '%s.kernel'", name.c_str());
  DGR_REQUIRE(kd->numel == (int64_t)K * cin * cout, "'%s.kernel' has %lld elements, expected %d x %d x %d",
              name.c_str(), (long long)kd->numel, K, cin, cout);
  std::vector<float> scale(cout, 1.f), shift(cout, 0.f);
  bool has_shift = false;
  std::vector<std::vector<float>> small;
  auto host_of = [&](const dgr_weight_desc *d) -> const float * {
    if (!P.dev) return d->data;
    small.emplace_back((size_t)d->numel);
    if (hipMemcpy(small.back().data(), d->data, (size_t)d->numel * sizeof(float), hipMemcpyDeviceToHost) != hipSuccess) return nullptr;
    return small.back().data();
  };
  if (bn) {
    std::string p = std::string(bn) + ".bn.";
    const dgr_weight_desc *g = find_desc(descs, nd, p + "weight"), *b = find_desc(descs, nd, p + "bias"),
                          *m = find_desc(descs, nd, p + "running_mean"),
                          *v = find_desc(descs, nd, p + "running_var");
    DGR_REQUIRE(g && b && m && v, "state_dict is missing batch-norm tensors '%s*'", p.c_str());
    DGR_REQUIRE(g->numel == cout && b->numel == cout && m->numel == cout && v->numel == cout,
                "batch-norm '%s' has the wrong width", p.c_str());
    const float *gd = host_of(g), *bd2 = host_of(b), *md = host_of(m), *vd = host_of(v);
    DGR_REQUIRE(gd && bd2 && md && vd, "batch-norm '%s': device tensors could not be read", p.c_str());
    for (int c = 0; c < cout; ++c) {
      float s = gd[c] / sqrtf(vd[c] + BN_EPS);
      scale[c] = s;
      shift[c] = bd2[c] - md[c] * s;
    }
    has_shift = true;
  }
  if (bias) {
    const dgr_weight_desc *bd = find_desc(descs, nd, name + ".bias");
    DGR_REQUIRE(bd && bd->numel == cout, "state_dict is missing '%s.bias' [1,%d]", name.c_str(), cout);
    const float *bh = host_of(bd);
    DGR_REQUIRE(bh, "'%s.bias': device tensor could not be read", name.c_str());
    for (int c = 0; c < cout; ++c) shift[c] += bh[c];
    has_shift = true;
  }
  DgrWeights &W = *net->W;
  hipStream_t s = P.s;
  const float *src = kd->data;
  if (!P.dev) {
    const size_t n = (size_t)kd->numel;
    if (n > P.staging_n) {
      DGR_HIP_CHECK(hipStreamSynchronize(s));
      DGR_HIP_CHECK(hipFree(P.staging));
      P.staging = nullptr;
      DGR_HIP_CHECK(hipMalloc((void **)&P.staging, n * sizeof(float)));
      P.staging_n = n;
    }
    DGR_HIP_CHECK(hipMemcpyAsync(P.staging, kd->data, n * sizeof(float), hipMemcpyHostToDevice, s));
    src = P.staging;
  }
  const float *sc = P.sc;
  DGR_HIP_CHECK(hipMemcpyAsync(P.sc, scale.data(), (size_t)cout * sizeof(float), hipMemcpyHostToDevice, s));
  if (has_shift) {
    DGR_CHECK(W.alloc(&L.shift, cout));
    DGR_HIP_CHECK(hipMemcpyAsync(L.shift, shift.data(), (size_t)cout * sizeof(float), hipMemcpyHostToDevice, s));
  }
  const int64_t nw = (int64_t)K * cin * cout;
  DGR_HIP_CHECK(hipMemsetAsync(P.mxb, 0, sizeof(uint32_t), s));
  dgr_absmax_scaled_kernel<<<(int)std::min<int64_t>((nw + 255) / 256, 4096), 256, 0, s>>>(src, sc, nw, cout, P.mxb);
  DGR_LAUNCH_CHECK();
  uint32_t bits = 0;
  DGR_HIP_CHECK(hipMemcpyAsync(&bits, P.mxb, sizeof(bits), hipMemcpyDeviceToHost, s));
  DGR_HIP_CHECK(hipStreamSynchronize(s));
  float mx;
  memcpy(&mx, &bits, 4);
  int ex = 0;
  if (mx > 0.f && std::isfinite(mx)) (void)frexpf(mx, &ex);
  ex = std::min(std::max(ex, -100), 100);
  const float w_scale = ldexpf(1.f, 15 - ex);
  L.w_unscale = ldexpf(1.f, ex - 15);
  const bool use_wide = K > 1 && !dgr_exact_f32() && dgr_conv_wide_supported(L.cin_pad, cin, cout) && !(net->D == 3 && K == 27);
  if (use_wide) {
    const int S16 = cin / 16, NB32 = cout / 32;
    L.wb_piece = (int64_t)K * S16 * NB32 * 64;
    const int64_t ne = L.wb_piece * 8;
    uint16_t *dst;
    DGR_CHECK(W.alloc(&dst, (size_t)2 * ne));
    L.wb = dst;
    DGR_CHECK(dgr_fill(s, ne, [=] __device__(int64_t o) {
      const int e = (int)(o & 7), lane = (int)((o >> 3) & 63);
      const int64_t r = o >> 9;
      const int nb = (int)(r % NB32), s2 = (int)((r / NB32) % S16), k = (int)(r / ((int64_t)NB32 * S16));
      const int col = 32 * nb + (lane & 31), row = 16 * s2 + 8 * (lane >> 5) + e;
      const float xs = __fmul_rn(__fmul_rn(src[((size_t)k * cin + row) * cout + col], sc[col]), w_scale);
      dst[o] = dgr_f16_bits_dev(xs);
      dst[ne + o] = dgr_f16_bits_dev(xs - dgr_f16_val_dev(xs));
    }));
    W.param_bytes += (size_t)2 * ne * sizeof(uint16_t);
  } else {
    const int S = L.cin_pad / 8, NBLK = L.cout_pad / 32;
    const int64_t ne = (int64_t)K * S * NBLK * 256;
    DGR_CHECK(W.alloc(&L.w, ne));
    float *const dst = L.w;
    DGR_CHECK(dgr_fill(s, ne, [=] __device__(int64_t o) {
      const int c = (int)(o & 3), lane = (int)((o >> 2) & 63);
      const int64_t r = o >> 8;
      const int nb = (int)(r % NBLK), s2 = (int)((r / NBLK) % S), k = (int)(r / ((int64_t)NBLK * S));
      const int row = 8 * s2 + 4 * (lane >> 5) + c, col = 32 * nb + (lane & 31);
      dst[o] = (row < cin && col < cout) ? __fmul_rn(src[((size_t)k * cin + row) * cout + col], sc[col]) : 0.f;
    }));
    W.param_bytes += (size_t)ne * sizeof(float);
  }
  if (net->D == 3 && K == 27 && L.cin_pad % 16 == 0 && cout % 32 == 0) {
    const int GT = L.cin_pad / 16, NB = cout / 16;
    {
      const int64_t ne = (int64_t)K * GT * NB * 256;
      DGR_CHECK(W.alloc(&L.w16, ne));
      float *const dst = L.w16;
      DGR_CHECK(dgr_fill(s, ne, [=] __device__(int64_t o) {
        const int c = (int)(o & 3), lane = (int)((o >> 2) & 63);
        const int64_t r = o >> 8;
        const int jb = (int)(r % NB), g = (int)((r / NB) % GT), k = (int)(r / ((int64_t)NB * GT));
        const int col = 16 * jb + (lane & 15), row = 16 * g + 4 * (lane >> 4) + c;
        dst[o] = row < cin ? __fmul_rn(src[((size_t)k * cin + row) * cout + col], sc[col]) : 0.f;
      }));
      W.param_bytes += (size_t)ne * sizeof(float);
    }
    if (cin % 32 == 0) {
      const int S32 = cin / 32;
      L.w16b_piece = (int64_t)K * S32 * NB * 64;
      const int64_t ne = L.w16b_piece * 8;
      uint16_t *pcs;
      DGR_CHECK(W.alloc(&pcs, (size_t)2 * ne));
      L.w16b = pcs;
      DGR_CHECK(dgr_fill(s, ne, [=] __device__(int64_t o) {
        const int e = (int)(o & 7), lane = (int)((o >> 3) & 63);
        const int64_t r = o >> 9;
        const int jb = (int)(r % NB), sI = (int)((r / NB) % S32), k = (int)(r / ((int64_t)NB * S32));
        const int col = 16 * jb + (lane & 15), row = 32 * sI + 8 * (lane >> 4) + e;
        const float xs = __fmul_rn(__fmul_rn(src[((size_t)k * cin + row) * cout + col], sc[col]), w_scale);
        pcs[o] = dgr_f16_bits_dev(xs);
        pcs[ne + o] = dgr_f16_bits_dev(xs - dgr_f16_val_dev(xs));
      }));
      W.param_bytes += (size_t)2 * ne * sizeof(uint16_t);
      if (net->D == 3 && K == 27 && (dgr_conv_dense_supported(cin, L.cin_pad, cout) || dgr_conv_up_supported(cin, L.cin_pad, cout))) {
        uint16_t *pd;
        DGR_CHECK(W.alloc(&pd, (size_t)2 * ne));
        L.w16d = pd;
        DGR_CHECK(dgr_fill(s, 2 * ne, [=] __device__(int64_t o) {
          const int e = (int)(o & 3), h = (int)((o >> 2) & 1);
          const int64_t f = o >> 3, base = f & ~(int64_t)63;
          const int lane = (int)(f & 63), col = lane & 15, lq = lane >> 4;
          const int64_t srcf = base + col + 16 * ((lq >> 1) + 2 * h);
          pd[o] = pcs[srcf * 8 + 4 * (lq & 1) + e];
        }));
        W.param_bytes += (size_t)2 * ne * sizeof(uint16_t);
      }
    }
  }
  if (net->D == 3 && name == "conv1" && cin == 1 && cout == 32 && K <= 343) {
    int ks = 1;
    while (ks * ks * ks < K) ++ks;
    const int ks2 = ks * ks, steps = (ks2 + 3) / 4;
    const int64_t ne = (int64_t)ks * steps * 128;
    DGR_CHECK(W.alloc(&L.wc, ne));
    float *const dst = L.wc;
    DGR_CHECK(dgr_fill(s, ne, [=] __device__(int64_t o) {
      const int j = (int)(o & 1), lane = (int)((o >> 1) & 63);
      const int64_t r = o >> 7;
      const int s2 = (int)(r % steps), kz = (int)(r / steps);
      const int kk = 4 * s2 + (lane >> 4), col = (lane & 15) + 16 * j;
      dst[o] = kk < ks2 ? __fmul_rn(src[(size_t)(kz * ks2 + kk) * cout + col], sc[col]) : 0.f;
    }));
  }
  if (name == "conv1" && cin == 6 && cout == 32 && K > 1) {
    const int64_t ne = (int64_t)K * 192;
    DGR_CHECK(W.alloc(&L.wq, ne));
    float *const dst = L.wq;
    DGR_CHECK(dgr_fill(s, ne, [=] __device__(int64_t o) {
      const int e = (int)(o & 3), q = (int)((o >> 2) & 3);
      const int i = (int)((o >> 4) % 12), k = (int)(o / 192);
      const int ci = i >> 1, co = 8 * q + 4 * (i & 1) + e;
      dst[o] = __fmul_rn(src[((size_t)k * cin + ci) * cout + co], sc[co]);
    }));
    W.param_bytes += (size_t)ne * sizeof(float);
  }
  W.layers.push_back(L);
  return DGR_OK;
}

static int net_create(dgr_ctx *ctx, int D, int in_channels, int out_channels, int conv1_kernel_size, int normalize_feature,
                      const dgr_weight_desc *weights, int n_weights, dgr_net **out, bool dev) {
  DGR_REQUIRE(ctx && weights && out, "dgr_net_create: NULL argument");
  if (dev) {
    for (int i = 0; i < n_weights; ++i) {
      hipPointerAttribute_t at;
      const hipError_t e = hipPointerGetAttributes(&at, weights[i].data);
      if (e != hipSuccess) (void)hipGetLastError();
      DGR_REQUIRE(e == hipSuccess && at.type == hipMemoryTypeDevice && at.device == ctx->device,
                  "dgr_net_create_device: '%s' is not a device pointer on device %d (use dgr_net_create for host tensors)",
                  weights[i].name ? weights[i].name : "?", ctx->device);
    }
  }
  DGR_REQUIRE(D == 3 || D == 6, "dgr_net_create: D=%d (ResUNetBN2C is used with D=3 and D=6)", D);
  DGR_REQUIRE(in_channels >= 1 && in_channels <= 256 && out_channels >= 1 && out_channels <= 64,
              "dgr_net_create: unsupported channel counts in=%d out=%d", in_channels, out_channels);
  DGR_REQUIRE(conv1_kernel_size % 2 == 1, "conv1 kernel size must be odd");
  DGR_HIP_CHECK(hipSetDevice(ctx->device));
  WeightPrep P{dev};
  DGR_HIP_CHECK(hipStreamCreate(&P.s));
  DGR_HIP_CHECK(hipMalloc((void **)&P.sc, 256 * sizeof(float)));
  DGR_HIP_CHECK(hipMalloc((void **)&P.mxb, sizeof(uint32_t)));
  dgr_net *net = new dgr_net();
  net->ctx = ctx;
  net->W = std::make_shared<DgrWeights>();
  net->W->device = ctx->device;
  net->D = D; net->cin = in_channels; net->cout = out_channels;
  net->conv1_ks = conv1_kernel_size; net->normalize = normalize_feature;
  int k3 = 1, k1 = 1;
  for (int d = 0; d < D; ++d) { k3 *= 3; k1 *= conv1_kernel_size; }
  int rc = DGR_OK;
  auto L = [&](const std::string &name, int K, int ci, int co, const char *bn, bool bias = false) {
    if (rc == DGR_OK) rc = make_layer(net, P, weights, n_weights, name, K, ci, co, bn, bias);
  };
  auto block = [&](const std::string &b, int c) {
    L(b + ".conv1", k3, c, c, (b + ".norm1").c_str());
    L(b + ".conv2", k3, c, c, (b + ".norm2").c_str());
  };
  L("conv1", k1, in_channels, CH[1], "norm1");          block("block1", CH[1]);
  L("conv2", k3, CH[1], CH[2], "norm2");                block("block2", CH[2]);
  L("conv3", k3, CH[2], CH[3], "norm3");                block("block3", CH[3]);
  L("conv4", k3, CH[3], CH[4], "norm4");                block("block4", CH[4]);
  L("conv4_tr", k3, CH[4], TR[4], "norm4_tr");          block("block4_tr", TR[4]);
  L("conv3_tr", k3, CH[3] + TR[4], TR[3], "norm3_tr");  block("block3_tr", TR[3]);
  L("conv2_tr", k3, CH[2] + TR[3], TR[2], "norm2_tr");  block("block2_tr", TR[2]);
  L("conv1_tr", 1, CH[1] + TR[2], TR[1], nullptr);
  L("final", 1, TR[1], out_channels, nullptr, true);
  if (rc == DGR_OK) rc = [&] { DGR_HIP_CHECK(hipStreamSynchronize(P.s)); return DGR_OK; }();
  if (rc != DGR_OK) {
    dgr_net_destroy(net);
    return rc;
  }
  *out = net;
  return DGR_OK;
}

extern "C" int dgr_net_create(dgr_ctx *ctx, int D, int in_channels, int out_channels,
                              int conv1_kernel_size, int normalize_feature,
                              const dgr_weight_desc *weights, int n_weights, dgr_net **out) {
  return net_create(ctx, D, in_channels, out_channels, conv1_kernel_size, normalize_feature, weights, n_weights, out, false);
}

extern "C" int dgr_net_create_device(dgr_ctx *ctx, int D, int in_channels, int out_channels,
                                     int conv1_kernel_size, int normalize_feature,
                                     const dgr_weight_desc *weights, int n_weights, dgr_net **out) {
  return net_create(ctx, D, in_channels, out_channels, conv1_kernel_size, normalize_feature, weights, n_weights, out, true);
}

extern "C" void dgr_net_destroy(dgr_net *net) {
  if (!net) return;
  delete net;
}

extern "C" int dgr_net_share(dgr_ctx *ctx, const dgr_net *src, dgr_net **out) {
  DGR_REQUIRE(ctx && src && out, "dgr_net_share: NULL argument");
  DGR_REQUIRE(ctx->device == src->W->device, "dgr_net_share: the weights live on device %d, the context on device %d",
              src->W->device, ctx->device);
  dgr_net *net = new dgr_net();
  net->ctx = ctx;
  net->D = src->D; net->cin = src->cin; net->cout = src->cout;
  net->conv1_ks = src->conv1_ks; net->normalize = src->normalize;
  net->W = src->W;
  *out = net;
  return DGR_OK;
}

extern "C" int dgr_net_sharers(const dgr_net *net) { return net ? (int)net->W.use_count() : 0; }
extern "C" int64_t dgr_net_param_bytes(const dgr_net *net) { return net ? net->W->param_bytes : 0; }
extern "C" int dgr_net_num_layers(const dgr_net *net) { return net ? (int)net->W->layers.size() : 0; }

struct Tensor {
  float *ptr;
  int ld;
  int relu;
  DgrSplitRows split;
  bool split_only = false;
  uint32_t *amax = nullptr, *amax2 = nullptr;
  unsigned char *dsplit = nullptr;
  bool dsplit_only = false;
};

struct Fwd {
  dgr_ctx *ctx;
  dgr_net *net;
  hipStream_t stream;
  DgrMapSet ms;
  bool prof;
  bool l2_next = false;

  float *ybuf = nullptr;

  int conv(int li, const Tensor &in, const DgrKernelMap *km, bool swapped, int lvl_in, int lvl_out,
           const Tensor &out, const Tensor *res) {
    const DgrLayer &L = net->W->layers[li];
    const DgrCoordMap &cin_map = ms.cm[lvl_in], &cout_map = ms.cm[lvl_out];
    DgrConvLaunch a;
    a.in = in.ptr; a.in_ld = in.ld; a.in_relu = in.relu;
    a.out = out.ptr; a.out_ld = out.ld;
    a.y = ybuf; a.shift = L.shift;
    a.w = L.w;
    a.cin = L.cin; a.cin_pad = L.cin_pad; a.cout = L.cout; a.cout_pad = L.cout_pad; a.K = L.K;
    if (km && ms.use_nbr) {
      a.pair_in = a.pair_out = a.tile_ptr = a.rule_ptr = nullptr;
      a.tile_desc = nullptr; a.n_rows_dev = nullptr; a.tile_bound = 0;
    } else if (km) {
      a.pair_in = swapped ? km->pair_out : km->pair_in;
      a.pair_out = swapped ? km->pair_in : km->pair_out;
      a.tile_ptr = km->tile_ptr; a.rule_ptr = km->rule_ptr; a.tile_desc = km->tile_desc;
      a.n_rows_dev = nullptr;
      a.tile_bound = km->pair_cap / DGR_TILE_M + km->K;
      DGR_REQUIRE(km->K == L.K, "layer %s: kernel volume mismatch", L.name.c_str());
      DGR_REQUIRE(!swapped || km->in_ptr, "layer %s: map has no in-major CSR", L.name.c_str());
    } else {
      DGR_REQUIRE(res == nullptr, "identity conv with residual not supported");
      a.pair_in = a.pair_out = a.tile_ptr = a.rule_ptr = nullptr;
      a.tile_desc = nullptr;
      a.n_rows_dev = cout_map.n_dev;
      a.tile_bound = dgr_ceil_div(cout_map.n_cap, DGR_TILE_M);
      a.l2_normalize = l2_next ? 1 : 0;
      l2_next = false;
    }
    hipEvent_t e0 = nullptr, em = nullptr, e1 = nullptr;
    if (prof) {
      e0 = ctx->events.next(); em = ctx->events.next(); e1 = ctx->events.next();
      if (!e0 || !em || !e1) return DGR_EHIP;
      DGR_HIP_CHECK(hipEventRecord(e0, stream));
    }
    if (km && ms.use_nbr) {
      const DgrNbrTable *t = nullptr;
      for (int l = 0; l < 4; ++l)
        if (km == &ms.same[l]) t = &ms.nsame[l];
      for (int l = 0; l < 3; ++l)
        if (km == &ms.down[l]) t = swapped ? &ms.nup[l] : &ms.ndown[l];
      DGR_REQUIRE(t && t->built && L.w16, "layer %s: no neighbour table / 16x16 weights", L.name.c_str());
      DgrConvOsLaunch o;
      o.in = in.ptr; o.in_ld = in.ld; o.in_relu = in.relu;
      o.out = out.ptr; o.out_ld = out.ld; o.out_relu = out.relu;
      o.rows_per_block = lvl_out <= 1 ? 64 : lvl_out == 2 ? (L.cin_pad >= 128 ? 64 : 32) : 16;
      o.phase_channels = (L.cin_pad >= 256 || (L.cin_pad == 128 && lvl_out >= 2)) ? 128 : 64;
      if (const char *e = getenv(lvl_out == 2 ? "DGR_OS_MB2" : lvl_out == 3 ? "DGR_OS_MB3" : "DGR_OS_MB01")) o.rows_per_block = atoi(e);
      if (const char *e = getenv("DGR_OS_CK")) o.phase_channels = atoi(e);
      o.w16 = L.w16; o.shift = L.shift;
      o.wb3 = L.w16b; o.piece_stride = L.w16b_piece;
      o.wbd = L.w16d;
      o.w_unscale = L.w_unscale; o.n_in_cap = cin_map.n_cap;
      if (L.w16b && !dgr_exact_f32()) {
        o.row_amax = in.amax;
        if (!o.row_amax) {
          uint32_t *mx;
          DGR_ALLOC(mx, ctx->arena, uint32_t, cin_map.n_cap);
          DGR_CHECK(dgr_row_amax(in.ptr, in.ld, L.cin, in.relu, cin_map.n_dev, cin_map.n_cap, mx, stream));
          o.row_amax = mx;
        }
      }
      o.out_amax = out.amax; o.out_amax2 = out.amax2;
      o.res = res ? res->ptr : nullptr; o.res_ld = res ? res->ld : 0; o.res_relu = res ? res->relu : 0;
      o.nbr = t; o.n_out_dev = cout_map.n_dev; o.n_out_cap = cout_map.n_cap;
      o.cin = L.cin; o.cin_pad = L.cin_pad; o.cout = L.cout;
      static const bool os_lists = getenv("DGR_OS_LISTS") != nullptr;
      bool same_stride = false;
      for (int l = 0; l < 4; ++l) same_stride = same_stride || t == &ms.nsame[l];
      o.dense = same_stride && o.row_amax && o.wbd && !os_lists && dgr_conv_dense_supported(L.cin, L.cin_pad, L.cout) &&
                cin_map.n_cap * (int64_t)in.ld * 4 < (1ll << 31);
      DGR_REQUIRE(o.dense || (!in.dsplit_only && !out.dsplit_only), "layer %s: dense split rows outside the dense-tile kernel", L.name.c_str());
      static const bool no_up = getenv("DGR_NO_UP") != nullptr;
      o.up = swapped && !o.dense && !no_up && !os_lists && o.row_amax && o.wbd && t->perm && res == nullptr &&
             dgr_conv_up_supported(L.cin, L.cin_pad, L.cout) && cin_map.n_cap * (int64_t)in.ld * 4 < (1ll << 31);
      if (o.dense) {
        o.in_dsplit = in.dsplit;
        o.out_dsplit = out.dsplit;
        if (out.dsplit_only) o.out = nullptr;
      }
      const char *kname = "sparse_conv_os";
      DGR_CHECK(dgr_conv_os_launch(o, stream, &kname));
      if (prof) {
        DGR_HIP_CHECK(hipEventRecord(e1, stream));
        ctx->conv_spans.push_back({e0, e1});
        ctx->gemm_spans.push_back({e0, e1});
        ctx->conv_kinds.push_back(kname);
      }
      LayerRun &r = net->runs[li];
      r = LayerRun();
      r.os = true;
      r.os_launch = o;
      r.nbr = *t;
      r.os_launch.nbr = &r.nbr;
      r.n_in = cin_map.n_dev; r.n_out = cout_map.n_dev; r.K = L.K;
      r.n_out_cap = cout_map.n_cap;
      return DGR_OK;
    }
    const bool small_cin = km && !swapped && !res && L.cin <= 8 && L.cout == 32 && L.cin_pad == 8;
    const char *kname = (L.cin == 6 && L.wq) ? "conv_cin6_quad_kernel" : L.cin == 1 ? "conv_small_cin_row_kernel" : "conv_small_cin_kernel";
    unsigned long long *clk = nullptr;
    const bool wide = L.wb && km;
    if (small_cin)
      DGR_CHECK(dgr_conv_small_cin(in.ptr, in.ld, in.relu, L.cin, L.w, L.wq, L.shift, *km, cout_map.n_dev, cout_map.n_cap,
                                   out.ptr, out.ld, stream));
    else if (wide) {
      DGR_REQUIRE(in.split.planes, "layer %s: the wide-layer kernel needs its input as split rows", L.name.c_str());
      if (prof) {
        DGR_ALLOC(a.clk, ctx->arena, unsigned long long, 2);
        DGR_HIP_CHECK(hipMemsetAsync(a.clk, 0xff, sizeof(unsigned long long), stream));
        DGR_HIP_CHECK(hipMemsetAsync(a.clk + 1, 0, sizeof(unsigned long long), stream));
        clk = a.clk;
      }
      DGR_CHECK(dgr_conv_wide_launch(a, in.split, L.wb, L.wb_piece, L.w_unscale, ctx->num_cus, stream, &kname));
    } else
      DGR_CHECK(dgr_conv_launch(a, ctx->num_cus, stream, &kname));
    if (prof) DGR_HIP_CHECK(hipEventRecord(em, stream));
    DGR_REQUIRE(!out.split.planes || (km && !small_cin), "layer %s: only a reduction can write split rows", L.name.c_str());
    if (km && !small_cin)
      DGR_CHECK(dgr_reduce_rows(ybuf, L.cout, swapped ? km->in_ptr : km->out_ptr, swapped ? km->in_pos : km->out_pos,
                                cout_map.n_dev, cout_map.n_cap, out.split_only ? nullptr : out.ptr, out.ld, L.shift, res ? res->ptr : nullptr,
                                res ? res->ld : 0, res ? res->relu : 0, stream, out.split.planes ? &out.split : nullptr,
                                out.relu));
    if (prof) {
      DGR_HIP_CHECK(hipEventRecord(e1, stream));
      ctx->conv_spans.push_back({e0, e1});
      ctx->gemm_spans.push_back({e0, em});
      ctx->conv_kinds.push_back(kname);
      ctx->conv_clks.resize(ctx->conv_spans.size(), nullptr);
      ctx->conv_clks.back() = clk;
    }
    LayerRun &r = net->runs[li];
    a.clk = nullptr;
    r.launch = a;
    r.split_in = wide ? in.split : DgrSplitRows();
    r.split_out = out.split;
    r.out_relu = out.relu;
    r.split_only = out.split_only;
    r.has_reduce = km != nullptr;
    r.small_cin = small_cin;
    if (km) r.km = *km;
    if (km) {
      r.red_ptr = swapped ? km->in_ptr : km->out_ptr;
      r.red_pos = swapped ? km->in_pos : km->out_pos;
    }
    r.n_out_cap = cout_map.n_cap;
    r.res = res ? res->ptr : nullptr; r.res_ld = res ? res->ld : 0; r.res_relu = res ? res->relu : 0;
    r.rule_ptr = km ? km->rule_ptr : nullptr;
    r.n_in = cin_map.n_dev; r.n_out = cout_map.n_dev; r.K = L.K;
    return DGR_OK;
  }
};

int dgr_resunet_forward_impl(dgr_ctx *ctx, dgr_net *net, const int32_t *coords, const float *feats,
                             int64_t N, float *out, hipStream_t stream) {
  DgrArena &A = ctx->arena;
  Fwd f;
  f.ctx = ctx; f.net = net; f.stream = stream; f.prof = ctx->profiling;
  hipEvent_t m0 = nullptr, m1 = nullptr;
  if (f.prof) {
    m0 = ctx->events.next(); m1 = ctx->events.next();
    DGR_HIP_CHECK(hipEventRecord(m0, stream));
  }
  f.ms.overflow = ctx->flag_dev;
  const bool use_nbr = net->D == 3 && net->cin <= 8 && net->conv1_ks <= 7;
  const bool conv1_fused = use_nbr;
  DGR_CHECK(dgr_build_maps(A, coords, N, net->D, net->conv1_ks, &f.ms, stream, conv1_fused, true, use_nbr));
  if (f.prof) {
    DGR_HIP_CHECK(hipEventRecord(m1, stream));
    (net->D == 3 ? ctx->map3_spans : ctx->map6_spans).push_back({m0, m1});
  }
  {
    const DgrMapSet &m = f.ms;
    int64_t need = m.use_nbr ? 64 : m.conv1.pair_cap * 32;
    const int64_t same_c[4] = {64, 64, 128, 256}, down_c[3] = {64, 128, 256};
    for (int l = 0; l < 4; ++l) need = std::max(need, m.same[l].pair_cap * same_c[l]);
    for (int l = 0; l < 3; ++l) need = std::max(need, m.down[l].pair_cap * down_c[l]);
    DGR_ALLOC(f.ybuf, A, float, need);
  }
  const DgrMapSet &ms = f.ms;
  const int64_t n1 = ms.cm[0].n_cap, n2 = ms.cm[1].n_cap, n4 = ms.cm[2].n_cap, n8 = ms.cm[3].n_cap;
  auto buf = [&](int64_t rows, int cols) -> float * { return A.get<float>((size_t)rows * cols); };
  float *t1 = buf(n1, 32), *y1 = buf(n1, 32), *cat1 = buf(n1, 96);
  float *t2 = buf(n2, 64), *y2 = buf(n2, 64), *cat2 = buf(n2, 128);
  float *t4 = buf(n4, 128), *y4 = buf(n4, 128), *cat4 = buf(n4, 256);
  float *t8 = buf(n8, 256), *y8 = buf(n8, 256), *s8 = buf(n8, 256);
  float *u4 = buf(n4, 128), *v4 = buf(n4, 128);
  float *u2 = buf(n2, 64), *v2 = buf(n2, 64);
  float *u1 = buf(n1, 64), *v1 = buf(n1, 64);
  float *h = buf(n1, 64);
  const bool fuse_l2 = net->normalize && net->cout <= 32;
  float *fin = (net->normalize && !fuse_l2) ? buf(n1, net->cout) : out;
  if (!t1 || !y1 || !cat1 || !t2 || !y2 || !cat2 || !t4 || !y4 || !cat4 || !t8 || !y8 || !s8 || !u4 ||
      !v4 || !u2 || !v2 || !u1 || !v1 || !h || !fin)
    return DGR_ENOMEM;

  const Tensor X{const_cast<float *>(feats), net->cin, 0};
  Tensor T1{t1, 32, 0}, Y1{y1, 32, 1}, S1{cat1 + 64, 96, 1};
  Tensor T2{t2, 64, 0}, Y2{y2, 64, 1};
  Tensor S2{cat2 + 64, 128, 1};
  Tensor T4{t4, 128, 0}, Y4{y4, 128, 1}, S4{cat4 + 128, 256, 1};
  Tensor T8{t8, 256, 0}, Y8{y8, 256, 1}, S8{s8, 256, 1};
  Tensor U4{u4, 128, 0}, V4{v4, 128, 1};
  Tensor U2{u2, 64, 0}, V2{v2, 64, 1};
  Tensor U1{u1, 64, 0}, V1{v1, 64, 1};
  Tensor S4T{cat4, 256, 1};
  {
    struct { Tensor *t; int consumer, channels; int64_t rows; bool middle; } sp[] = {
        {&T2, 4, 64, n2, false}, {&Y2, 5, 64, n2, true},
        {&S2, 6, 64, n2, false}, {&T4, 7, 128, n4, false}, {&Y4, 8, 128, n4, true}, {&S4, 9, 128, n4, false},
        {&T8, 10, 256, n8, false}, {&Y8, 11, 256, n8, true}, {&S8, 12, 256, n8, false}, {&U4, 13, 128, n4, false},
        {&V4, 14, 128, n4, true}, {&U2, 16, 64, n2, false}, {&V2, 17, 64, n2, true}, {&U1, 19, 64, n1, false},
        {&V1, 20, 64, n1, true}};
    for (auto &e : sp) {
      if (!net->W->layers[e.consumer].wb) continue;
      e.t->split.channels = e.channels;
      e.t->split_only = e.middle;
      DGR_ALLOC(e.t->split.planes, A, unsigned char, (size_t)e.rows * 4 * e.channels);
      DGR_ALLOC(e.t->split.scale, A, float, e.rows);
    }
  }
  Tensor S2T{cat2, 128, 1};
  const Tensor S1T{cat1, 96, 1};
  const Tensor H{h, 64, 1}, FIN{fin, net->cout, 0};
  Tensor CAT4{cat4, 256, 1}, CAT2{cat2, 128, 1};
  if (use_nbr) {
    const int64_t words = 5 * n1 + 6 * n2 + 6 * n4 + 3 * n8;
    uint32_t *pool;
    DGR_ALLOC(pool, A, uint32_t, words);
    DGR_HIP_CHECK(hipMemsetAsync(pool, 0, (size_t)words * sizeof(uint32_t), stream));
    auto take = [&](int64_t n) { uint32_t *p = pool; pool += n; return p; };
    for (Tensor *t : {&T1, &Y1, &S1, &U1, &V1}) t->amax = take(n1);
    for (Tensor *t : {&T2, &Y2, &S2, &CAT2, &U2, &V2}) t->amax = take(n2);
    for (Tensor *t : {&T4, &Y4, &S4, &CAT4, &U4, &V4}) t->amax = take(n4);
    for (Tensor *t : {&T8, &Y8, &S8}) t->amax = take(n8);
    S2.amax2 = CAT2.amax; S2T.amax2 = CAT2.amax;
    S4.amax2 = CAT4.amax; S4T.amax2 = CAT4.amax;
  }

  if (use_nbr && !getenv("DGR_NO_DSPLIT")) {
    static const bool os_lists = getenv("DGR_OS_LISTS") != nullptr;
    auto dense_layer = [&](int l, int64_t rows) {
      const DgrLayer &L = net->W->layers[l];
      return L.w16b && L.w16d && !dgr_exact_f32() && !os_lists && dgr_conv_dense_supported(L.cin, L.cin_pad, L.cout) &&
             rows * (int64_t)L.cin * 4 < (1ll << 31);
    };
    struct { Tensor *t; int producer; int64_t rows; } mid[] = {{&Y1, 1, n1}, {&Y2, 4, n2}, {&V2, 16, n2}, {&V1, 19, n1}};
    for (auto &e : mid)
      if (dense_layer(e.producer, e.rows) && dense_layer(e.producer + 1, e.rows) && e.t->ld == net->W->layers[e.producer].cout) {
        e.t->dsplit = reinterpret_cast<unsigned char *>(e.t->ptr);
        e.t->dsplit_only = true;
      }
  }

  int li = 0;
  if (conv1_fused) {
    const DgrLayer &L0 = net->W->layers[0];
    int32_t *pc;
    DGR_ALLOC(pc, A, int32_t, 1);
    hipEvent_t e0 = nullptr, e1 = nullptr;
    if (f.prof) {
      e0 = ctx->events.next(); e1 = ctx->events.next();
      DGR_HIP_CHECK(hipEventRecord(e0, stream));
    }
    const char *k1name = "conv1_grid_kernel";
    DGR_CHECK(dgr_conv1_probe(A, ms.cm[0], net->conv1_ks, feats, net->cin, net->cin, L0.w, L0.shift, t1, 32, pc, stream,
                              L0.wc, &k1name, T1.amax));
    if (f.prof) {
      DGR_HIP_CHECK(hipEventRecord(e1, stream));
      ctx->conv_spans.push_back({e0, e1});
      ctx->gemm_spans.push_back({e0, e1});
      ctx->conv_kinds.push_back(k1name);
    }
    LayerRun &r0 = net->runs[0];
    r0 = LayerRun();
    r0.n_in = r0.n_out = ms.cm[0].n_dev;
    r0.K = L0.K;
    r0.fused_pairs = pc;
    li++;
  } else {
    DGR_CHECK(f.conv(li++, X, &ms.conv1, false, 0, 0, T1, nullptr));
  }
  DGR_CHECK(f.conv(li++, T1, &ms.same[0], false, 0, 0, Y1, nullptr));
  DGR_CHECK(f.conv(li++, Y1, &ms.same[0], false, 0, 0, S1, &T1));
  DGR_CHECK(f.conv(li++, S1, &ms.down[0], false, 0, 1, T2, nullptr));
  DGR_CHECK(f.conv(li++, T2, &ms.same[1], false, 1, 1, Y2, nullptr));
  DGR_CHECK(f.conv(li++, Y2, &ms.same[1], false, 1, 1, S2, &T2));
  DGR_CHECK(f.conv(li++, S2, &ms.down[1], false, 1, 2, T4, nullptr));
  DGR_CHECK(f.conv(li++, T4, &ms.same[2], false, 2, 2, Y4, nullptr));
  DGR_CHECK(f.conv(li++, Y4, &ms.same[2], false, 2, 2, S4, &T4));
  DGR_CHECK(f.conv(li++, S4, &ms.down[2], false, 2, 3, T8, nullptr));
  DGR_CHECK(f.conv(li++, T8, &ms.same[3], false, 3, 3, Y8, nullptr));
  DGR_CHECK(f.conv(li++, Y8, &ms.same[3], false, 3, 3, S8, &T8));
  DGR_CHECK(f.conv(li++, S8, &ms.down[2], true, 3, 2, U4, nullptr));
  DGR_CHECK(f.conv(li++, U4, &ms.same[2], false, 2, 2, V4, nullptr));
  DGR_CHECK(f.conv(li++, V4, &ms.same[2], false, 2, 2, S4T, &U4));
  DGR_CHECK(f.conv(li++, CAT4, &ms.down[1], true, 2, 1, U2, nullptr));
  DGR_CHECK(f.conv(li++, U2, &ms.same[1], false, 1, 1, V2, nullptr));
  DGR_CHECK(f.conv(li++, V2, &ms.same[1], false, 1, 1, S2T, &U2));
  DGR_CHECK(f.conv(li++, CAT2, &ms.down[0], true, 1, 0, U1, nullptr));
  DGR_CHECK(f.conv(li++, U1, &ms.same[0], false, 0, 0, V1, nullptr));
  DGR_CHECK(f.conv(li++, V1, &ms.same[0], false, 0, 0, S1T, &U1));
  const Tensor CAT1{cat1, 96, 1};
  DGR_CHECK(f.conv(li++, CAT1, nullptr, false, 0, 0, H, nullptr));
  f.l2_next = fuse_l2;
  DGR_CHECK(f.conv(li++, H, nullptr, false, 0, 0, FIN, nullptr));
  if (net->normalize && !fuse_l2)
    DGR_CHECK(dgr_l2_normalize_rows(fin, net->cout, out, net->cout, net->cout, 0, ms.cm[0].n_dev, n1, stream));

  auto &I = net->inter;
  net->run_generation = ctx->arena.generation;
  I.clear();
  I["s1"] = {S1.ptr, 96, 32, ms.cm[0].n_dev};
  I["s2"] = {S2.ptr, 128, 64, ms.cm[1].n_dev, ms.cm[1].canon};
  I["s4"] = {S4.ptr, 256, 128, ms.cm[2].n_dev, ms.cm[2].canon};
  I["s8"] = {S8.ptr, 256, 256, ms.cm[3].n_dev, ms.cm[3].canon};
  I["s4_tr"] = {cat4, 256, 128, ms.cm[2].n_dev, ms.cm[2].canon};
  I["s2_tr"] = {cat2, 128, 64, ms.cm[1].n_dev, ms.cm[1].canon};
  I["s1_tr"] = {cat1, 96, 64, ms.cm[0].n_dev};

  return DGR_OK;
}

void dgr_ctx_begin_profile(dgr_ctx *ctx) {
  ctx->events.used = 0;
  ctx->conv_spans.clear();
  ctx->gemm_spans.clear();
  ctx->conv_kinds.clear();
  ctx->conv_clks.clear();
  ctx->map3_spans.clear();
  ctx->map6_spans.clear();
  ctx->conv_launches = 0;
}

int dgr_ctx_collect_profile(dgr_ctx *ctx) {
  auto total = [](const std::vector<std::pair<hipEvent_t, hipEvent_t>> &v, float *out) -> int {
    float s = 0.f, t = 0.f;
    for (auto &sp : v) {
      DGR_HIP_CHECK(hipEventElapsedTime(&t, sp.first, sp.second));
      s += t;
    }
    *out = s;
    return DGR_OK;
  };
  DGR_CHECK(total(ctx->map3_spans, &ctx->stage_ms[5]));
  DGR_CHECK(total(ctx->map6_spans, &ctx->stage_ms[6]));
  DGR_CHECK(total(ctx->conv_spans, &ctx->stage_ms[7]));
  ctx->conv_launches = (int64_t)ctx->conv_spans.size();
  ctx->conv_span_ms.clear();
  ctx->gemm_span_ms.clear();
  for (auto &sp : ctx->conv_spans) {
    float t = 0.f;
    DGR_HIP_CHECK(hipEventElapsedTime(&t, sp.first, sp.second));
    ctx->conv_span_ms.push_back(t);
  }
  for (auto &sp : ctx->gemm_spans) {
    float t = 0.f;
    DGR_HIP_CHECK(hipEventElapsedTime(&t, sp.first, sp.second));
    ctx->gemm_span_ms.push_back(t);
  }
  ctx->conv_clk_us.assign(ctx->conv_spans.size(), 0.f);
  for (size_t i = 0; i < ctx->conv_clks.size() && i < ctx->conv_clk_us.size(); ++i)
    if (ctx->conv_clks[i]) {
      unsigned long long c[2] = {0, 0};
      DGR_HIP_CHECK(hipMemcpy(c, ctx->conv_clks[i], sizeof(c), hipMemcpyDeviceToHost));
      if (c[1] > c[0]) ctx->conv_clk_us[i] = (float)((double)(c[1] - c[0]) * 0.01);
    }
  return DGR_OK;
}

int dgr_flag_error(int32_t flag) {
  if (flag == 1) {
    dgr_set_error("duplicate coordinates in the sparse tensor input");
    return DGR_EINVAL;
  }
  if (flag == 2) {
    dgr_set_error("kernel-map capacity exceeded (more than the reserved pairs per output row)");
    return DGR_ENOMEM;
  }
  return DGR_OK;
}

static int check_flag(dgr_ctx *ctx, const int32_t *flag_dev, hipStream_t stream) {
  unsigned char *pin;
  DGR_CHECK(dgr_ctx_pinned(ctx, 64, &pin));
  DGR_HIP_CHECK(hipMemcpyAsync(pin, flag_dev, sizeof(int32_t), hipMemcpyDeviceToHost, stream));
  DGR_CHECK(dgr_ctx_wait(ctx, stream));
  return dgr_flag_error(*reinterpret_cast<volatile int32_t *>(pin));
}

int dgr_ctx_new_flag(dgr_ctx *ctx, hipStream_t stream) {
  DGR_ALLOC(ctx->flag_dev, ctx->arena, int32_t, 1);
  DGR_HIP_CHECK(hipMemsetAsync(ctx->flag_dev, 0, sizeof(int32_t), stream));
  return DGR_OK;
}

int dgr_ctx_check_flag(dgr_ctx *ctx, hipStream_t stream) {
  if (!ctx->flag_dev) return DGR_OK;
  return check_flag(ctx, ctx->flag_dev, stream);
}

void dgr_net_invalidate_runs(dgr_net *net) { net->run_generation = ~0ull; }
int dgr_net_out_channels(const dgr_net *net) { return net->cout; }
int dgr_net_in_channels(const dgr_net *net) { return net->cin; }
int dgr_net_dim(const dgr_net *net) { return net->D; }
const dgr_ctx *dgr_net_ctx(const dgr_net *net) { return net->ctx; }

extern "C" int dgr_resunet_forward(dgr_ctx *ctx, dgr_net *net, const int32_t *coords, const float *feats,
                                   int64_t N, float *out, dgr_stream stream_) {
  DGR_REQUIRE(ctx && net && coords && feats && out, "dgr_resunet_forward: NULL argument");
  DGR_REQUIRE(net->ctx == ctx, "dgr_resunet_forward: the net object belongs to another context (one dgr_net per context: "
                               "dgr_net_share gives a second context its own over the same weights)");
  DGR_REQUIRE(N > 0, "dgr_resunet_forward: empty sparse tensor (N=%lld)", (long long)N);
  hipStream_t stream = (hipStream_t)stream_;
  DGR_HIP_CHECK(hipSetDevice(ctx->device));
  DGR_CHECK(ctx->arena.reset());
  DGR_CHECK(dgr_ctx_new_flag(ctx, stream));
  dgr_ctx_begin_profile(ctx);
  DGR_CHECK(dgr_resunet_forward_impl(ctx, net, coords, feats, N, out, stream));
  DGR_CHECK(dgr_ctx_check_flag(ctx, stream));
  if (ctx->profiling) {
    memset(ctx->stage_ms, 0, sizeof(ctx->stage_ms));
    DGR_CHECK(dgr_ctx_collect_profile(ctx));
  }
  return DGR_OK;
}

extern "C" int dgr_debug_conv_layer(dgr_ctx *ctx, dgr_net *net, int layer, const int32_t *coords, const float *in,
                                    int in_relu, int64_t N, float *out, dgr_stream stream_) {
  DGR_REQUIRE(ctx && net && coords && in && out && N > 0, "dgr_debug_conv_layer: bad argument");
  DGR_REQUIRE(layer >= 0 && layer < (int)net->W->layers.size(), "layer %d out of range", layer);
  const DgrLayer &L = net->W->layers[layer];
  int k3 = 1;
  for (int d = 0; d < net->D; ++d) k3 *= 3;
  DGR_REQUIRE(L.K == k3 && L.cin >= 32, "dgr_debug_conv_layer: layer %s is not a 3^D conv with >= 32 input channels", L.name.c_str());
  hipStream_t stream = (hipStream_t)stream_;
  DGR_HIP_CHECK(hipSetDevice(ctx->device));
  DGR_CHECK(ctx->arena.reset());
  DGR_CHECK(dgr_ctx_new_flag(ctx, stream));
  dgr_ctx_begin_profile(ctx);
  DgrArena &A = ctx->arena;
  Fwd f;
  f.ctx = ctx; f.net = net; f.stream = stream; f.prof = false;
  f.ms.overflow = ctx->flag_dev;
  DGR_CHECK(dgr_build_maps(A, coords, N, net->D, 3, &f.ms, stream, false, true, net->D == 3));
  const int64_t n_cap = f.ms.cm[0].n_cap;
  if (!f.ms.use_nbr) DGR_ALLOC(f.ybuf, A, float, f.ms.same[0].pair_cap * L.cout);
  Tensor tin{const_cast<float *>(in), L.cin, in_relu}, tout{out, L.cout, 0};
  if (L.wb) {
    tin.split.channels = L.cin;
    DGR_ALLOC(tin.split.planes, A, unsigned char, (size_t)n_cap * 4 * L.cin);
    DGR_ALLOC(tin.split.scale, A, float, n_cap);
    DGR_CHECK(dgr_split_rows(in, L.cin, in_relu, f.ms.cm[0].n_dev, n_cap, tin.split, stream));
  }
  DGR_CHECK(f.conv(layer, tin, &f.ms.same[0], false, 0, 0, tout, nullptr));
  DGR_CHECK(dgr_ctx_check_flag(ctx, stream));
  dgr_net_invalidate_runs(net);
  return DGR_OK;
}

extern "C" int dgr_net_get_intermediate(dgr_ctx *ctx, dgr_net *net, const char *name, float *host_out,
                                        int64_t capacity, int64_t *rows, int64_t *cols) {
  DGR_REQUIRE(ctx && net && name && rows && cols, "NULL argument");
  auto it = net->inter.find(name);
  DGR_REQUIRE(it != net->inter.end() && it->second.n_dev, "no intermediate named '%s' (run a forward first)", name);
  DGR_REQUIRE(net->run_generation == ctx->arena.generation,
              "the activations of the last forward are gone: a later call on this context reused its workspace");
  const DgrTensorRef &t = it->second;
  int32_t n = 0;
  DGR_HIP_CHECK(hipDeviceSynchronize());
  DGR_HIP_CHECK(hipMemcpy(&n, t.n_dev, sizeof(int32_t), hipMemcpyDeviceToHost));
  *rows = n;
  *cols = t.cols;
  if (host_out) {
    DGR_REQUIRE(capacity >= (int64_t)n * t.cols, "host buffer too small");
    if (!t.canon) {
      DGR_HIP_CHECK(hipMemcpy2D(host_out, (size_t)t.cols * sizeof(float), t.ptr, (size_t)t.ld * sizeof(float),
                                (size_t)t.cols * sizeof(float), (size_t)n, hipMemcpyDeviceToHost));
    } else {
      std::vector<float> tmp((size_t)n * t.cols);
      std::vector<int32_t> canon(n);
      DGR_HIP_CHECK(hipMemcpy2D(tmp.data(), (size_t)t.cols * sizeof(float), t.ptr, (size_t)t.ld * sizeof(float),
                                (size_t)t.cols * sizeof(float), (size_t)n, hipMemcpyDeviceToHost));
      DGR_HIP_CHECK(hipMemcpy(canon.data(), t.canon, (size_t)n * sizeof(int32_t), hipMemcpyDeviceToHost));
      for (int32_t p = 0; p < n; ++p)
        memcpy(host_out + (size_t)canon[p] * t.cols, tmp.data() + (size_t)p * t.cols, (size_t)t.cols * sizeof(float));
    }
    for (int64_t i = 0; i < (int64_t)n * t.cols; ++i) host_out[i] = host_out[i] > 0.f ? host_out[i] : 0.f;
  }
  return DGR_OK;
}

extern "C" int dgr_net_layer_stats(dgr_ctx *ctx, dgr_net *net, int layer, int64_t stats[8]) {
  DGR_REQUIRE(ctx && net && stats, "NULL argument");
  DGR_REQUIRE(layer >= 0 && layer < (int)net->W->layers.size(), "layer %d out of range", layer);
  const LayerRun &r = net->runs[layer];
  DGR_REQUIRE(r.n_in && r.n_out, "run a forward first");
  DGR_REQUIRE(net->run_generation == ctx->arena.generation,
              "the kernel maps of the last forward are gone: a later call on this context reused its workspace");
  const DgrLayer &L = net->W->layers[layer];
  DGR_HIP_CHECK(hipDeviceSynchronize());
  int32_t n_in = 0, n_out = 0;
  DGR_HIP_CHECK(hipMemcpy(&n_in, r.n_in, sizeof(int32_t), hipMemcpyDeviceToHost));
  DGR_HIP_CHECK(hipMemcpy(&n_out, r.n_out, sizeof(int32_t), hipMemcpyDeviceToHost));
  int64_t P = n_out, kne = 1;
  if (r.os) {
    int64_t counts[27];
    DGR_CHECK(dgr_nbr_counts(r.nbr, r.n_out, counts));
    P = 0;
    kne = 0;
    for (int k = 0; k < 27; ++k) { P += counts[k]; kne += counts[k] > 0; }
  } else if (r.fused_pairs) {
    int32_t pc = 0;
    DGR_HIP_CHECK(hipMemcpy(&pc, r.fused_pairs, sizeof(int32_t), hipMemcpyDeviceToHost));
    P = pc;
    kne = r.K;
  } else if (r.rule_ptr) {
    std::vector<int32_t> rp(r.K + 1);
    DGR_HIP_CHECK(hipMemcpy(rp.data(), r.rule_ptr, (size_t)(r.K + 1) * sizeof(int32_t), hipMemcpyDeviceToHost));
    P = rp[r.K];
    kne = 0;
    for (int k = 0; k < r.K; ++k) kne += rp[k + 1] > rp[k];
  }
  stats[0] = P; stats[1] = kne; stats[2] = n_in; stats[3] = n_out;
  stats[4] = L.cin; stats[5] = L.cout; stats[6] = L.K; stats[7] = 0;
  return DGR_OK;
}

extern "C" int dgr_net_rerun_layer(dgr_ctx *ctx, dgr_net *net, int layer, int reps, float *gemm_ms, float *reduce_ms) {
  DGR_REQUIRE(ctx && net && gemm_ms && reduce_ms && reps > 0, "bad argument");
  DGR_REQUIRE(layer >= 0 && layer < (int)net->W->layers.size(), "layer %d out of range", layer);
  const LayerRun &r = net->runs[layer];
  DGR_REQUIRE(r.n_in && r.n_out, "run a forward first");
  DGR_REQUIRE(net->run_generation == ctx->arena.generation,
              "the kernel maps of the last forward are gone: a later call on this context reused its workspace");
  DGR_REQUIRE(!r.fused_pairs, "layer %d ran fused with its neighbour search; not re-runnable", layer);
  const DgrLayer &L = net->W->layers[layer];
  hipEvent_t e0, e1, e2;
  DGR_HIP_CHECK(hipEventCreate(&e0)); DGR_HIP_CHECK(hipEventCreate(&e1)); DGR_HIP_CHECK(hipEventCreate(&e2));
  float tg = 0.f, tr = 0.f;
  for (int i = 0; i < reps + 1; ++i) {
    DGR_HIP_CHECK(hipEventRecord(e0, nullptr));
    if (r.os)
      DGR_CHECK(dgr_conv_os_launch(r.os_launch, nullptr));
    else if (r.small_cin)
      DGR_CHECK(dgr_conv_small_cin(r.launch.in, r.launch.in_ld, r.launch.in_relu, L.cin, L.w, L.wq, L.shift, r.km, r.n_out,
                                   r.n_out_cap, r.launch.out, r.launch.out_ld, nullptr));
    else if (L.wb && r.has_reduce)
      DGR_CHECK(dgr_conv_wide_launch(r.launch, r.split_in, L.wb, L.wb_piece, L.w_unscale, ctx->num_cus, nullptr));
    else
      DGR_CHECK(dgr_conv_launch(r.launch, ctx->num_cus, nullptr));
    DGR_HIP_CHECK(hipEventRecord(e1, nullptr));
    if (r.has_reduce && !r.small_cin && !r.os)
      DGR_CHECK(dgr_reduce_rows(r.launch.y, L.cout, r.red_ptr, r.red_pos, r.n_out, r.n_out_cap,
                                r.split_only ? nullptr : r.launch.out, r.launch.out_ld, L.shift, r.res, r.res_ld, r.res_relu, nullptr,
                                r.split_out.planes ? &r.split_out : nullptr, r.out_relu));
    DGR_HIP_CHECK(hipEventRecord(e2, nullptr));
    DGR_HIP_CHECK(hipEventSynchronize(e2));
    float a = 0.f, b = 0.f;
    DGR_HIP_CHECK(hipEventElapsedTime(&a, e0, e1));
    DGR_HIP_CHECK(hipEventElapsedTime(&b, e1, e2));
    if (i > 0) { tg += a; tr += b; }
  }
  (void)hipEventDestroy(e0); (void)hipEventDestroy(e1); (void)hipEventDestroy(e2);
  *gemm_ms = tg / reps;
  *reduce_ms = tr / reps;
  return DGR_OK;
}
```

### deepglobalregistration_amd/ops.py

```python
import ctypes as C

import numpy as np
import torch

from . import _lib
from ._lib import check, get_ctx, ptr, stream_ptr, vp

F32_EPS = float(np.finfo(np.float32).eps)


def _dev(t):
    if not (torch.is_tensor(t) and t.is_cuda):
        raise ValueError('expected a CUDA(ROCm) tensor')
    return t.device


def _as(t, dtype, device):
    if not torch.is_tensor(t):
        t = torch.as_tensor(np.asarray(t))
    return t.to(device=device, dtype=dtype).contiguous()


def voxelize(xyz, voxel_size, batch_index=0, device='cuda'):
    lib = _lib.load()
    device = torch.device(device)
    if not torch.is_tensor(xyz):
        xyz = torch.from_numpy(np.ascontiguousarray(xyz))
    if xyz.dtype not in (torch.float32, torch.float64):
        xyz = xyz.double()
    if xyz.dim() != 2 or xyz.shape[1] != 3:
        raise ValueError(f'expected an [M,3] point array, got {tuple(xyz.shape)}')
    xyz = xyz.to(device).contiguous()
    M = xyz.shape[0]
    if M == 0:
        raise ValueError('empty point cloud')
    sel = torch.empty(M, dtype=torch.int64, device=device)
    coords = torch.empty((M, 4), dtype=torch.int32, device=device)
    out = torch.empty((M, 3), dtype=torch.float32, device=device)
    n = C.c_int64(0)
    check(lib.dgr_voxelize(get_ctx(device), ptr(xyz), int(xyz.dtype == torch.float64), M,
                           float(voxel_size), int(batch_index), ptr(sel), ptr(coords), ptr(out),
                           C.byref(n), stream_ptr(device.index)))
    n = n.value
    return out[:n], coords[:n], sel[:n]


class NetHandle:

    def __init__(self, state_dict, D, in_channels, out_channels, conv1_kernel_size,
                 normalize_feature, device='cuda', share_from=None):
        lib = _lib.load()
        self.device = torch.device(device)
        self.D, self.cin, self.cout = D, in_channels, out_channels
        self.conv1_ks, self.normalize = int(conv1_kernel_size), bool(normalize_feature)
        if share_from is not None:
            if (share_from.D, share_from.cin, share_from.cout, share_from.conv1_ks, share_from.normalize) != \
                    (D, in_channels, out_channels, self.conv1_ks, self.normalize):
                raise ValueError('share_from is a different network')
            h = vp()
            with torch.cuda.device(self.device):
                check(lib.dgr_net_share(get_ctx(self.device), share_from.handle, C.byref(h)))
            self.handle = h
            return
        keep, descs = [], []
        items = [(n, t) for n, t in state_dict.items() if not n.endswith('num_batches_tracked')]
        on_device = bool(items) and all(torch.is_tensor(t) and t.is_cuda and t.device.index == (self.device.index or 0)
                                        for _, t in items)
        self.created_on_device = on_device
        for name, t in items:
            if on_device:
                a = t.detach().to(torch.float32).contiguous()
                keep.append(a)
                descs.append(_lib.WeightDesc(name.encode(), a.data_ptr(), a.numel()))
            else:
                a = t.detach().cpu().numpy() if torch.is_tensor(t) else np.asarray(t)
                a = np.ascontiguousarray(a, dtype=np.float32)
                keep.append(a)
                descs.append(_lib.WeightDesc(name.encode(), a.ctypes.data, a.size))
        arr = (_lib.WeightDesc * len(descs))(*descs)
        h = vp()
        with torch.cuda.device(self.device):
            if on_device:
                torch.cuda.current_stream(self.device).synchronize()
            create = lib.dgr_net_create_device if on_device else lib.dgr_net_create
            check(create(get_ctx(self.device), D, in_channels, out_channels,
                         conv1_kernel_size, int(bool(normalize_feature)), arr, len(descs),
                         C.byref(h)))
        self.handle = h

    def __del__(self):
        try:
            if getattr(self, 'handle', None):
                _lib.load().dgr_net_destroy(self.handle)
                self.handle = None
        except Exception:
            pass

    @property
    def param_bytes(self):
        return _lib.load().dgr_net_param_bytes(self.handle)

    @property
    def sharers(self):
        return _lib.load().dgr_net_sharers(self.handle)

    def forward(self, coords, feats):
        lib = _lib.load()
        dev = self.device
        coords = _as(coords, torch.int32, dev)
        feats = _as(feats, torch.float32, dev)
        if coords.dim() != 2 or coords.shape[1] != self.D + 1:
            raise ValueError(f'coords must be [N,{self.D + 1}] (batch column first), got {tuple(coords.shape)}')
        if feats.dim() != 2 or feats.shape != (coords.shape[0], self.cin):
            raise ValueError(f'feats must be [{coords.shape[0]},{self.cin}], got {tuple(feats.shape)}')
        N = coords.shape[0]
        if N == 0:
            raise ValueError('empty sparse tensor')
        out = torch.empty((N, self.cout), dtype=torch.float32, device=dev)
        check(lib.dgr_resunet_forward(get_ctx(dev), self.handle, ptr(coords), ptr(feats), N, ptr(out),
                                      stream_ptr(dev.index)))
        return out

    def intermediate(self, name):
        lib = _lib.load()
        rows, cols = C.c_int64(0), C.c_int64(0)
        ctx = get_ctx(self.device)
        check(lib.dgr_net_get_intermediate(ctx, self.handle, name.encode(), None, 0, C.byref(rows), C.byref(cols)))
        buf = np.empty((rows.value, cols.value), np.float32)
        check(lib.dgr_net_get_intermediate(ctx, self.handle, name.encode(), buf.ctypes.data, buf.size,
                                           C.byref(rows), C.byref(cols)))
        return buf

    def debug_conv_layer(self, layer, coords, feats, relu=False):
        dev = self.device
        coords = _as(coords, torch.int32, dev)
        feats = _as(feats, torch.float32, dev)
        lay = _lib.load()
        st_cout = None
        ch, tr = [None, 32, 64, 128, 256], [None, 64, 64, 64, 128]
        widths = [ch[1]] * 3 + [ch[2]] * 3 + [ch[3]] * 3 + [ch[4]] * 3 + [tr[4]] * 3 + [tr[3]] * 3 + [tr[2]] * 3 + [tr[1], self.cout]
        st_cout = widths[layer]
        out = torch.empty((coords.shape[0], st_cout), dtype=torch.float32, device=dev)
        check(lay.dgr_debug_conv_layer(get_ctx(dev), self.handle, int(layer), ptr(coords), ptr(feats), int(bool(relu)),
                                       coords.shape[0], ptr(out), stream_ptr(dev.index)))
        return out

    def rerun_layer(self, layer, reps=5):
        lib = _lib.load()
        g, r = C.c_float(0), C.c_float(0)
        check(lib.dgr_net_rerun_layer(get_ctx(self.device), self.handle, layer, reps, C.byref(g), C.byref(r)))
        return g.value, r.value

    def layer_stats(self):
        lib = _lib.load()
        out = []
        for li in range(lib.dgr_net_num_layers(self.handle)):
            st = (C.c_int64 * 8)()
            check(lib.dgr_net_layer_stats(get_ctx(self.device), self.handle, li, st))
            out.append(dict(pairs=st[0], nonempty=st[1], n_in=st[2], n_out=st[3], cin=st[4], cout=st[5], K=st[6]))
        return out


class Maps:

    def __init__(self, coords, D, conv1_kernel_size=3, device='cuda'):
        lib = _lib.load()
        self.device = torch.device(device)
        coords = _as(coords, torch.int32, self.device)
        self.D = D
        h = vp()
        check(lib.dgr_maps_create(get_ctx(self.device), ptr(coords), coords.shape[0], D, conv1_kernel_size,
                                  C.byref(h), stream_ptr(self.device.index)))
        self.handle = h

    def __del__(self):
        try:
            if getattr(self, 'handle', None):
                _lib.load().dgr_maps_destroy(self.handle)
                self.handle = None
        except Exception:
            pass

    def coords(self, ts):
        lib = _lib.load()
        n = C.c_int64(0)
        check(lib.dgr_maps_get_coords(self.handle, ts, None, 0, C.byref(n)))
        out = np.empty((n.value, self.D + 1), np.int32)
        check(lib.dgr_maps_get_coords(self.handle, ts, out.ctypes.data, out.size, C.byref(n)))
        return out

    def kernel_map(self, kind, ts):
        lib = _lib.load()
        kid = {'same': 0, 'conv1': 1, 'down': 2, 'nbr_same': 3, 'nbr_down': 4, 'nbr_up': 5}[kind]
        K, P = C.c_int64(0), C.c_int64(0)
        check(lib.dgr_maps_get_kernel_map(self.handle, kid, ts, None, 0, None, None, 0, C.byref(K), C.byref(P)))
        rule = np.empty(K.value + 1, np.int32)
        pin = np.empty(P.value, np.int32)
        pout = np.empty(P.value, np.int32)
        check(lib.dgr_maps_get_kernel_map(self.handle, kid, ts, rule.ctypes.data, rule.size, pin.ctypes.data,
                                          pout.ctypes.data, pin.size, C.byref(K), C.byref(P)))
        k = np.repeat(np.arange(K.value), np.diff(rule))
        return k.astype(np.int64), pin.astype(np.int64), pout.astype(np.int64)


def knn1(F0, F1, squared=False, return_distance=False):
    lib = _lib.load()
    dev = _dev(F0)
    F0 = _as(F0, torch.float32, dev)
    F1 = _as(F1, torch.float32, dev)
    if F0.dim() != 2 or F1.dim() != 2 or F0.shape[1] != F1.shape[1]:
        raise ValueError('F0 [N0,C] and F1 [N1,C] must share the feature width')
    N0, N1 = F0.shape[0], F1.shape[0]
    idx = torch.empty(N0, dtype=torch.int64, device=dev)
    dist = torch.empty(N0, dtype=torch.float32, device=dev) if return_distance else None
    check(lib.dgr_knn1_l2(get_ctx(dev), ptr(F0), N0, ptr(F1), N1, F0.shape[1], int(squared), ptr(idx),
                          ptr(dist), stream_ptr(dev.index)))
    return (idx, dist) if return_distance else idx


def knn1_batch(F0, F1, off0, off1, squared=False, return_distance=False):
    lib = _lib.load()
    dev = _dev(F0)
    F0 = _as(F0, torch.float32, dev)
    F1 = _as(F1, torch.float32, dev)
    if F0.dim() != 2 or F1.dim() != 2 or F0.shape[1] != F1.shape[1]:
        raise ValueError('F0 [N0,C] and F1 [N1,C] must share the feature width')
    o0 = np.ascontiguousarray(off0, dtype=np.int64)
    o1 = np.ascontiguousarray(off1, dtype=np.int64)
    if len(o0) != len(o1) or len(o0) < 2 or o0[0] != 0 or o1[0] != 0 or o0[-1] != F0.shape[0] or o1[-1] != F1.shape[0]:
        raise ValueError('off0 / off1 must be [npairs+1] row offsets covering F0 / F1')
    idx = torch.empty(F0.shape[0], dtype=torch.int64, device=dev)
    dist = torch.empty(F0.shape[0], dtype=torch.float32, device=dev) if return_distance else None
    check(lib.dgr_knn1_l2_batch(get_ctx(dev), ptr(F0), o0.ctypes.data_as(_lib.c_i64p), ptr(F1),
                                o1.ctypes.data_as(_lib.c_i64p), len(o0) - 1, F0.shape[1], int(squared), ptr(idx),
                                ptr(dist), stream_ptr(dev.index)))
    return (idx, dist) if return_distance else idx


KNN_MAX_K = 32


def check_knn_k(k):
    if isinstance(k, (bool, np.bool_)) or not isinstance(k, (int, np.integer)):
        raise ValueError(f'knn must be an integer in [1, {KNN_MAX_K}], got {k!r}')
    if not 1 <= int(k) <= KNN_MAX_K:
        raise ValueError(f'knn must be an integer in [1, {KNN_MAX_K}], got {int(k)}')
    return int(k)


def knn(F0, F1, k, squared=False, return_distance=False):
    k = check_knn_k(k)
    lib = _lib.load()
    dev = _dev(F0)
    F0 = _as(F0, torch.float32, dev)
    F1 = _as(F1, torch.float32, dev)
    if F0.dim() != 2 or F1.dim() != 2 or F0.shape[1] != F1.shape[1]:
        raise ValueError('F0 [N0,C] and F1 [N1,C] must share the feature width')
    N0, N1 = F0.shape[0], F1.shape[0]
    idx = torch.empty((N0, k), dtype=torch.int64, device=dev)
    dist = torch.empty((N0, k), dtype=torch.float32, device=dev) if return_distance else None
    check(lib.dgr_knn_l2(get_ctx(dev), ptr(F0), N0, ptr(F1), N1, F0.shape[1], k, int(squared), ptr(idx), ptr(dist),
                         stream_ptr(dev.index)))
    return (idx, dist) if return_distance else idx


def knn_batch(F0, F1, off0, off1, k, squared=False, return_distance=False):
    k = check_knn_k(k)
    lib = _lib.load()
    dev = _dev(F0)
    F0 = _as(F0, torch.float32, dev)
    F1 = _as(F1, torch.float32, dev)
    if F0.dim() != 2 or F1.dim() != 2 or F0.shape[1] != F1.shape[1]:
        raise ValueError('F0 [N0,C] and F1 [N1,C] must share the feature width')
    o0 = np.ascontiguousarray(off0, dtype=np.int64)
    o1 = np.ascontiguousarray(off1, dtype=np.int64)
    if len(o0) != len(o1) or len(o0) < 2 or o0[0] != 0 or o1[0] != 0 or o0[-1] != F0.shape[0] or o1[-1] != F1.shape[0]:
        raise ValueError('off0 / off1 must be [npairs+1] row offsets covering F0 / F1')
    idx = torch.empty((F0.shape[0], k), dtype=torch.int64, device=dev)
    dist = torch.empty((F0.shape[0], k), dtype=torch.float32, device=dev) if return_distance else None
    check(lib.dgr_knn_l2_batch(get_ctx(dev), ptr(F0), o0.ctypes.data_as(_lib.c_i64p), ptr(F1),
                               o1.ctypes.data_as(_lib.c_i64p), len(o0) - 1, F0.shape[1], k, int(squared), ptr(idx),
                               ptr(dist), stream_ptr(dev.index)))
    return (idx, dist) if return_distance else idx


def inlier_inputs(coords0, xyz0, coords1, xyz1, idx1, feature_type='coords'):
    lib = _lib.load()
    dev = _dev(xyz0)
    ft = {'ones': 0, 'coords': 1}.get(feature_type)
    if ft is None:
        raise TypeError('Undefined feature type')
    coords0, coords1 = _as(coords0, torch.int32, dev), _as(coords1, torch.int32, dev)
    xyz0, xyz1 = _as(xyz0, torch.float32, dev), _as(xyz1, torch.float32, dev)
    idx1 = _as(idx1, torch.int64, dev).reshape(-1)
    N0 = coords0.shape[0]
    if idx1.shape[0] != N0:
        raise ValueError('one correspondence per row of fragment 0 expected')
    coords6 = torch.empty((N0, 7), dtype=torch.int32, device=dev)
    feats = torch.empty((N0, 6 if ft == 1 else 1), dtype=torch.float32, device=dev)
    check(lib.dgr_inlier_inputs(get_ctx(dev), ptr(coords0), ptr(xyz0), N0, ptr(coords1), ptr(xyz1),
                                coords1.shape[0], ptr(idx1), ft, ptr(coords6), ptr(feats),
                                stream_ptr(dev.index)))
    return coords6, feats


def sigmoid_clip_sum(logit, clip):
    lib = _lib.load()
    dev = _dev(logit)
    logit = _as(logit, torch.float32, dev).reshape(-1)
    w = torch.empty_like(logit)
    s = C.c_double(0)
    check(lib.dgr_sigmoid_clip_sum(get_ctx(dev), ptr(logit), logit.shape[0], float(clip), ptr(w), C.byref(s),
                                   stream_ptr(dev.index)))
    return w.reshape(-1, 1), s.value


def gather_rows3(src, idx):
    lib = _lib.load()
    dev = _dev(src)
    src = _as(src, torch.float32, dev)
    idx = _as(idx, torch.int64, dev).reshape(-1)
    out = torch.empty((idx.shape[0], 3), dtype=torch.float32, device=dev)
    check(lib.dgr_gather_rows3(get_ctx(dev), ptr(src), ptr(idx), idx.shape[0], ptr(out), stream_ptr(dev.index)))
    return out


def _xyw(X, Y, w):
    dev = _dev(X)
    X, Y = _as(X, torch.float32, dev), _as(Y, torch.float32, dev)
    w = _as(w, torch.float32, dev).reshape(-1)
    if X.shape != Y.shape or X.dim() != 2 or X.shape[1] != 3 or w.shape[0] != X.shape[0]:
        raise ValueError('X, Y must be [N,3] and w [N] / [N,1]')
    return dev, X, Y, w


def weighted_procrustes(X, Y, w, eps=F32_EPS):
    lib = _lib.load()
    dev, X, Y, w = _xyw(X, Y, w)
    R = (C.c_float * 9)()
    t = (C.c_float * 3)()
    check(lib.dgr_weighted_procrustes(get_ctx(dev), ptr(X), ptr(Y), ptr(w), X.shape[0], float(eps), R, t,
                                      stream_ptr(dev.index)))
    return np.array(R, np.float32).reshape(3, 3), np.array(t, np.float32)


def se3_refine(X, Y, w, quantization_size=1.0, max_iter=1000, max_break_count=20,
               break_threshold_ratio=1e-5):
    lib = _lib.load()
    dev, X, Y, w = _xyw(X, Y, w)
    R = (C.c_float * 9)()
    t = (C.c_float * 3)()
    it, bc, loss = C.c_int32(0), C.c_int32(0), C.c_float(0)
    check(lib.dgr_se3_refine(get_ctx(dev), ptr(X), ptr(Y), ptr(w), X.shape[0], float(quantization_size),
                             int(max_iter), int(max_break_count), float(break_threshold_ratio), R, t,
                             C.byref(it), C.byref(loss), C.byref(bc), stream_ptr(dev.index)))
    return (np.array(R, np.float32).reshape(3, 3), np.array(t, np.float32),
            {'iterations': it.value, 'loss': loss.value, 'break_count': bc.value})


def se3_refine_from(X, Y, w, state, max_iter, quantization_size=1.0, max_break_count=10 ** 9,
                    break_threshold_ratio=1e-5):
    lib = _lib.load()
    dev, X, Y, w = _xyw(X, Y, w)
    si = (C.c_double * 30)(*([float(v) for v in state['prm']] + [float(v) for v in state['m']] + [float(v) for v in state['v']]
                             + [float(state['i']), float(state['loss_prev']), float(state['breaks'])]))
    so = (C.c_double * 30)()
    check(lib.dgr_debug_se3_refine_from(get_ctx(dev), ptr(X), ptr(Y), ptr(w), X.shape[0], float(quantization_size),
                                        int(max_iter), int(max_break_count), float(break_threshold_ratio), si, so,
                                        stream_ptr(dev.index)))
    so = np.array(so, np.float64)
    return {'prm': so[:9].copy(), 'm': so[9:18].copy(), 'v': so[18:27].copy(), 'i': int(so[27]), 'loss_prev': float(so[28]),
            'breaks': int(so[29])}


def _xyz_dev(a, dev=None):
    t = a if torch.is_tensor(a) else torch.as_tensor(np.asarray(a))
    if dev is None:
        dev = t.device if t.is_cuda else torch.device('cuda', torch.cuda.current_device())
    t = t.to(device=dev, dtype=torch.float32).contiguous()
    if t.dim() != 2 or t.shape[1] != 3:
        raise ValueError(f'expected [N,3] points, got {tuple(t.shape)}')
    return t


def _xyz_any_dev(a):
    t = a if torch.is_tensor(a) else torch.from_numpy(np.ascontiguousarray(a))
    return t if t.is_cuda else t.to(torch.device('cuda', torch.cuda.current_device()))


def icp_point_to_point(source, target, max_correspondence_distance, init=None, max_iter=30,
                       relative_fitness=1e-6, relative_rmse=1e-6):
    lib = _lib.load()
    src = _xyz_dev(source)
    dst = _xyz_dev(target, src.device)
    Ti = None
    if init is not None:
        init = np.ascontiguousarray(np.asarray(init, np.float64))
        if init.shape != (4, 4):
            raise ValueError('init must be a 4x4 matrix')
        Ti = (C.c_double * 16)(*init.reshape(-1))
    T = (C.c_double * 16)()
    st = (C.c_double * 3)()
    check(lib.dgr_icp_point_to_point(get_ctx(src.device), ptr(src), src.shape[0], ptr(dst), dst.shape[0],
                                     float(max_correspondence_distance), Ti, int(max_iter), float(relative_fitness),
                                     float(relative_rmse), T, st, stream_ptr(src.device.index)))
    return np.array(T, np.float64).reshape(4, 4), float(st[0]), float(st[1]), int(st[2])


def ransac_correspondence(X, Y, distance_threshold, num_hypotheses, seed=0):
    lib = _lib.load()
    X = _xyz_dev(X)
    Y = _xyz_dev(Y, X.device)
    if X.shape != Y.shape:
        raise ValueError('X and Y must have the same shape')
    T = (C.c_double * 16)()
    st = (C.c_double * 3)()
    check(lib.dgr_ransac_correspondence(get_ctx(X.device), ptr(X), ptr(Y), X.shape[0], float(distance_threshold),
                                        int(num_hypotheses), int(seed) & 0xffffffff, T, st, stream_ptr(X.device.index)))
    return np.array(T, np.float64).reshape(4, 4), int(st[0]), int(st[1]), float(st[2])


def _offsets(off, name, total=None):
    o = np.ascontiguousarray(np.asarray(off), dtype=np.int64).reshape(-1)
    if len(o) < 2 or o[0] != 0 or bool((np.diff(o) < 0).any()):
        raise ValueError(f'{name} must be [npairs+1] row offsets that start at 0 and do not decrease')
    if total is not None and o[-1] != total:
        raise ValueError(f'{name} ends at {int(o[-1])}, the array has {int(total)} rows')
    return o


def _rows(a, width, name):
    shape = tuple(a.shape) if hasattr(a, 'shape') else np.asarray(a).shape
    if len(shape) != 2 or shape[1] != width:
        raise ValueError(f'{name} must be [N,{width}], got {shape}')
    return shape[0]


def check_radius_args(radius, K, T, npairs):
    if isinstance(radius, (bool, np.bool_)) or not isinstance(radius, (int, float, np.integer, np.floating)) \
            or not np.isfinite(radius) or radius <= 0:
        raise ValueError(f'radius must be a positive finite number, got {radius!r}')
    if K is not None and (isinstance(K, (bool, np.bool_)) or not isinstance(K, (int, np.integer)) or K < 1
                          or K > np.iinfo(np.int32).max):
        raise ValueError(f'K must be None or an integer >= 1, got {K!r}')
    T = T.detach().cpu().numpy() if torch.is_tensor(T) else np.asarray(T)
    if T.shape == (4, 4) and npairs == 1:
        T = T[None]
    if T.shape != (npairs, 4, 4):
# ... 573 lines not shown
```

### include/dgr_hip.h

```cpp
#ifndef DGR_HIP_H
#define DGR_HIP_H

#include <stdint.h>

#ifdef __cplusplus
extern "C" {
#endif

typedef struct dgr_ctx dgr_ctx;
typedef struct dgr_net dgr_net;
typedef struct dgr_maps dgr_maps;
typedef void *dgr_stream;

enum {
  DGR_OK = 0,
  DGR_EINVAL = -1,
  DGR_EHIP = -2,
  DGR_ENOMEM = -3,
  DGR_ESVD = -4,
  DGR_EINTERNAL = -5
};

enum { DGR_STATUS_OK = 0, DGR_STATUS_LOW_CONFIDENCE = 1, DGR_STATUS_SVD_FAILED = 2,
       DGR_STATUS_SAFEGUARD = 3 ,
       DGR_STATUS_FLAG_ICP_SKIPPED = 0x100, DGR_STATUS_MASK = 0xff,
       DGR_STATUS_EXCHANGE_TIMEOUT = 0x7f };

const char *dgr_last_error(void);
const char *dgr_version(void);

int dgr_ctx_create(int device, dgr_ctx **out);
void dgr_ctx_destroy(dgr_ctx *ctx);
int64_t dgr_ctx_workspace_bytes(dgr_ctx *ctx);
int dgr_ctx_create_partition_stream(dgr_ctx *ctx, int part, int nparts, dgr_stream *out);

int dgr_voxelize(dgr_ctx *ctx, const void *xyz, int is_f64, int64_t M, double voxel_size,
                 int32_t batch_index, int64_t *sel_out, int32_t *coords_out, float *xyz_out,
                 int64_t *n_out, dgr_stream stream);

typedef struct {
  const char *name;
  const float *data;
  int64_t numel;
} dgr_weight_desc;

int dgr_net_create(dgr_ctx *ctx, int D, int in_channels, int out_channels, int conv1_kernel_size,
                   int normalize_feature, const dgr_weight_desc *weights, int n_weights,
                   dgr_net **out);
int dgr_net_create_device(dgr_ctx *ctx, int D, int in_channels, int out_channels, int conv1_kernel_size,
                          int normalize_feature, const dgr_weight_desc *weights, int n_weights,
                          dgr_net **out);
void dgr_net_destroy(dgr_net *net);
int64_t dgr_net_param_bytes(const dgr_net *net);
int dgr_net_share(dgr_ctx *ctx, const dgr_net *src, dgr_net **out);
int dgr_net_sharers(const dgr_net *net);

int dgr_resunet_forward(dgr_ctx *ctx, dgr_net *net, const int32_t *coords, const float *feats,
                        int64_t N, float *out, dgr_stream stream);
int dgr_net_get_intermediate(dgr_ctx *ctx, dgr_net *net, const char *name, float *host_out,
                             int64_t capacity, int64_t *rows, int64_t *cols);
int dgr_net_layer_stats(dgr_ctx *ctx, dgr_net *net, int layer, int64_t stats[8]);
int dgr_net_num_layers(const dgr_net *net);
int dgr_net_rerun_layer(dgr_ctx *ctx, dgr_net *net, int layer, int reps, float *gemm_ms, float *reduce_ms);

int dgr_maps_create(dgr_ctx *ctx, const int32_t *coords, int64_t N, int D, int conv1_kernel_size,
                    dgr_maps **out, dgr_stream stream);
void dgr_maps_destroy(dgr_maps *maps);
int dgr_maps_get_coords(dgr_maps *maps, int ts, int32_t *host_out, int64_t capacity, int64_t *n);
int dgr_maps_get_kernel_map(dgr_maps *maps, int kind, int ts, int32_t *rule_ptr, int64_t rule_cap,
                            int32_t *pair_in, int32_t *pair_out, int64_t pair_cap, int64_t *K,
                            int64_t *P);

int dgr_knn1_l2(dgr_ctx *ctx, const float *F0, int64_t N0, const float *F1, int64_t N1, int C,
                int squared, int64_t *idx_out, float *dist_out, dgr_stream stream);

int dgr_knn1_l2_batch(dgr_ctx *ctx, const float *F0, const int64_t *off0, const float *F1,
                      const int64_t *off1, int npairs, int C, int squared, int64_t *idx_out,
                      float *dist_out, dgr_stream stream);

#define DGR_KNN_MAX_K 32
int dgr_knn_l2(dgr_ctx *ctx, const float *F0, int64_t N0, const float *F1, int64_t N1, int C, int k,
               int squared, int64_t *idx_out, float *dist_out, dgr_stream stream);

int dgr_knn_l2_batch(dgr_ctx *ctx, const float *F0, const int64_t *off0, const float *F1,
                     const int64_t *off1, int npairs, int C, int k, int squared, int64_t *idx_out,
                     float *dist_out, dgr_stream stream);

int dgr_inlier_inputs(dgr_ctx *ctx, const int32_t *coords0, const float *xyz0, int64_t N0,
                      const int32_t *coords1, const float *xyz1, int64_t N1, const int64_t *idx1,
                      int feature_type, int32_t *coords6_out, float *feats_out, dgr_stream stream);

int dgr_sigmoid_clip_sum(dgr_ctx *ctx, const float *logit, int64_t N, float clip, float *weights_out,
                         double *wsum, dgr_stream stream);

int dgr_gather_rows3(dgr_ctx *ctx, const float *src, const int64_t *idx, int64_t N, float *dst,
                     dgr_stream stream);

int dgr_weighted_procrustes(dgr_ctx *ctx, const float *X, const float *Y, const float *w, int64_t N,
                            float eps, float *R9, float *t3, dgr_stream stream);

int dgr_se3_refine(dgr_ctx *ctx, const float *X, const float *Y, const float *w, int64_t N,
                   float quantization_size, int max_iter, int max_break_count,
                   double break_threshold_ratio, float *R9, float *t3, int32_t *iterations,
                   float *loss, int32_t *break_count, dgr_stream stream);

int dgr_icp_point_to_point(dgr_ctx *ctx, const float *src, int64_t N0, const float *dst, int64_t N1,
                           double max_correspondence_distance, const double *T_init, int max_iter,
                           double relative_fitness, double relative_rmse, double *T_out, double *stats_out,
                           dgr_stream stream);

int dgr_ransac_correspondence(dgr_ctx *ctx, const float *X, const float *Y, int64_t N, double distance_threshold,
                              int64_t num_hypotheses, uint32_t seed, double *T_out, double *stats_out,
                              dgr_stream stream);

typedef struct {
  float clip_weight_thresh;
  float voxel_size;
  int inlier_feature_type;
  int max_iter;
  int max_break_count;
  double break_threshold_ratio;
  int skip_refinement;
  int safeguard;
  int64_t ransac_hypotheses;
  uint32_t ransac_seed;
  int use_icp;
} dgr_params;

int dgr_register_batch(dgr_ctx *ctx, dgr_net *fcgf, dgr_net *inlier, const int32_t *coords0,
                       const float *xyz0, const int64_t *off0, const int32_t *coords1,
                       const float *xyz1, const int64_t *off1, int npairs, const dgr_params *params,
                       const int64_t *override_idx1, const float *forced_logit, float *T_out,
                       int32_t *status_out,
                       float *stats_out, dgr_stream stream);
int dgr_register_pairs(dgr_ctx *ctx, dgr_net *inlier, const int32_t *bank_coords, const float *bank_xyz,
                       const float *bank_F, const int64_t *bank_off, int nfrag, int C, const int32_t *pair_ids,
                       int npairs, const dgr_params *params, const int64_t *override_idx1,
                       const float *forced_logit, float *T_out, int32_t *status_out, float *stats_out,
                       dgr_stream stream);
int dgr_register_batch_output(dgr_ctx *ctx, int which, void *dst_dev, int64_t capacity_bytes,
                              int64_t *numel, dgr_stream stream);
int dgr_register_batch_f64(dgr_ctx *ctx, double *T_out, int64_t capacity_pairs, int64_t *npairs);

int dgr_ctx_set_profiling(dgr_ctx *ctx, int enable);
#define DGR_NUM_STAGE_TIMES 9
int dgr_ctx_stage_times_v2(dgr_ctx *ctx, float *times_ms, int capacity, int *n);
int dgr_ctx_stage_times(dgr_ctx *ctx, float *times_ms);
int64_t dgr_ctx_conv_launches(dgr_ctx *ctx);
int dgr_ctx_conv_launch_times(dgr_ctx *ctx, float *times_ms, float *gemm_ms, int64_t capacity, int64_t *n);
int dgr_ctx_conv_launch_kernel_us(dgr_ctx *ctx, float *us, int64_t capacity, int64_t *n);
int dgr_ctx_conv_launch_kinds(dgr_ctx *ctx, char *buf, int64_t capacity, int64_t *n);

int dgr_radius_pairs_batch(dgr_ctx *ctx, const float *xyz0, const int64_t *off0, const float *xyz1,
                           const int64_t *off1, int npairs, const double *T, double radius, int K,
                           int32_t *counts_out, int64_t *pairs_out, int64_t capacity, int64_t *total_out,
                           dgr_stream stream);
int dgr_pairs_isin_batch(dgr_ctx *ctx, const int64_t *pos, const int64_t *pos_off, const int64_t *pred,
                         const int64_t *pred_off, int npairs, const int64_t *M_per_pair, uint8_t *out,
                         dgr_stream stream);
int dgr_validation_counts(dgr_ctx *ctx, const uint8_t *label, const float *weights, float threshold,
                          const int64_t *off, int npairs, int64_t *counts_out, dgr_stream stream);

#define DGR_SCORE_WIDTH 11
int dgr_score_pairs(dgr_ctx *ctx, const float *bank_xyz, const int64_t *bank_off, int nfrag, const int32_t *pair_ids,
                    int npairs, const double *T, double radius, double *sums_out, dgr_stream stream);

#define DGR_PG_MAX_NODES 128
typedef struct {
  double mu;
  int reference_node;
  int max_iter;
  double rel_tol;
} dgr_pg_params;
int dgr_pose_graph_optimize(dgr_ctx *ctx, int ngraphs, const int64_t *node_off, const int64_t *edge_off,
                            const int32_t *edge_ids, const double *edge_T, const double *edge_info,
                            const uint8_t *edge_uncertain, const double *pose_init, const dgr_pg_params *params,
                            double *pose_out, double *line_out, double *stats_out, dgr_stream stream);

#define DGR_VM_FRAC_BITS 40
int dgr_voxel_mean(dgr_ctx *ctx, const void *xyz, int is_f64, const int64_t *off, int nfrag, const int32_t *frag_ids,
                   int nsel, const double *T, const double *origin, double voxel_size, int64_t *first_out,
                   int32_t *coords_out, int32_t *count_out, int64_t *fsum_out, double *mean_out, int64_t *n_out,
                   int64_t *dropped_out, dgr_stream stream);

#define DGR_TSDF_BLOCK_LIMIT 67108864
int dgr_tsdf_fragment(dgr_ctx *ctx, const uint16_t *depth, int nframes, int height, int width, const double *intrinsic,
                      const double *pose, const double *extrinsic, double voxel_length, double sdf_trunc,
                      double depth_scale, double depth_trunc, int block, int stride, int min_weight, double *xyz_out,
                      int64_t max_points, int32_t *blocks_out, float *tsdf_out, int32_t *weight_out, int64_t max_blocks,
                      int64_t *n_blocks_out, int64_t *n_points_out, int64_t *kept_out, dgr_stream stream);

int dgr_debug_ortho2rotation(dgr_ctx *ctx, const float *p6, int64_t n, const float *grad_R9, float *R9_out,
                             float *grad_p6_out, dgr_stream stream);
int dgr_debug_se3_refine_from(dgr_ctx *ctx, const float *X, const float *Y, const float *w, int64_t N,
                              float quantization_size, int max_iter, int max_break_count,
                              double break_threshold_ratio, const double *state_in, double *state_out,
                              dgr_stream stream);
int dgr_debug_smooth_l1(dgr_ctx *ctx, const float *X, const float *Y, int64_t n, float quantization_size,
                        float *per_point_out, dgr_stream stream);

int dgr_debug_conv_layer(dgr_ctx *ctx, dgr_net *net, int layer, const int32_t *coords, const float *in, int in_relu,
                         int64_t N, float *out, dgr_stream stream);

#ifdef __cplusplus
}
#endif
#endif
```

Measured before the change: 382.7.

## Add neighbour-table dense-tile MFMA sparse conv kernel for selected layer shapes

Adds a new sparse convolution kernel that stages the 27-offset neighbour table in shared memory per output block. It gathers neighbour input rows via buffer loads, splits them on the fly into f16 hi/lo operands, and accumulates with three f16 MFMA products per step. A routing table picks which Cin/Cout shapes (same-stride and strided-down) use it instead of the output-stationary path, and the shared split/permute helpers move into a common header. It aims to replace per-pair gather/scatter work with tensor-core tiles, but adds redundant loads for missing neighbours and more kernel variants.

```diff
diff --git a/deepglobalregistration_amd/_lib.py b/deepglobalregistration_amd/_lib.py
--- a/deepglobalregistration_amd/_lib.py
+++ b/deepglobalregistration_amd/_lib.py
@@ -102,6 +102,10 @@
                                             c_f64p, c_f64p, vp]),
     'dgr_debug_smooth_l1': (C.c_int, [vp, vp, vp, C.c_int64, C.c_float, vp, vp]),
     'dgr_debug_conv_layer': (C.c_int, [vp, vp, C.c_int, vp, vp, C.c_int, C.c_int64, vp, vp]),
+    'dgr_debug_conv_layer_ex': (C.c_int, [vp, vp, C.c_int, vp, vp, C.c_int, C.c_int64, C.c_int, vp, C.c_int, vp, vp,
+                                          c_i64p, vp]),
+    'dgr_conv_nbr_routed': (C.c_int, [C.c_int, C.c_int, C.c_int]),
+    'dgr_conv_nbr_block_rows': (C.c_int, [C.c_int, C.c_int]),
 }
 
 _lib = None
diff --git a/deepglobalregistration_amd/csrc/conv_dense.hip b/deepglobalregistration_amd/csrc/conv_dense.hip
--- a/deepglobalregistration_amd/csrc/conv_dense.hip
+++ b/deepglobalregistration_amd/csrc/conv_dense.hip
@@ -1,13 +1,5 @@
 #include "dgr_internal.h"
-#include "split.h"
-
-typedef float f32x4 __attribute__((ext_vector_type(4)));
-typedef float f32x2 __attribute__((ext_vector_type(2)));
-typedef int i32x4 __attribute__((ext_vector_type(4)));
-typedef _Float16 f16x8 __attribute__((ext_vector_type(8)));
-typedef _Float16 f16x2 __attribute__((ext_vector_type(2)));
-typedef unsigned int u32x2 __attribute__((ext_vector_type(2)));
-typedef unsigned int u32x4 __attribute__((ext_vector_type(4)));
+#include "conv_tile.h"
 
 #ifndef DGR_DENSE_RG
 #define DGR_DENSE_RG 2
@@ -124,38 +116,22 @@
   auto body = [&](int k, RowSet &g) {
     f16x8 bh[RG][S], bm[RG][S];
     float fold[RG];
-    const int from = 4 * (4 * (lane & 15) + (lane >> 4));
+    const int from = dgr_tile_perm_from(lane);
 #pragma unroll
     for (int rg = 0; rg < RG; ++rg) {
-      const float sx = g.nv[rg] >= 0 ? dgr_row_scale_of(g.mx[rg]) : 0.f;
-      const float fl = sx != 0.f ? dgr_inv_pow2(sx) * a.w_unscale : 0.f;
-      fold[rg] = __builtin_bit_cast(float, __builtin_amdgcn_ds_bpermute(16 * (lane & 15), __builtin_bit_cast(int, fl)));
+      const float sx = dgr_tile_row_scale(g.nv[rg], g.mx[rg]);
+      fold[rg] = dgr_tile_fold(sx, a.w_unscale, lane);
 #pragma unroll
       for (int s = 0; s < S; ++s) {
         i32x4 hw, mw;
         if constexpr (PS) {
           hw = __builtin_bit_cast(i32x4, g.raw[rg][s][0]);
           mw = __builtin_bit_cast(i32x4, g.raw[rg][s][1]);
-        } else
-#pragma unroll
-        for (int h = 0; h < 2; ++h) {
-          const i32x4 v = __builtin_bit_cast(i32x4, g.raw[rg][s][h]);
-#pragma unroll
-          for (int u = 0; u < 4; u += 2) {
-            const f32x2 xs = f32x2{__builtin_bit_cast(float, max(v[u], relu_lo)), __builtin_bit_cast(float, max(v[u + 1], relu_lo))} * sx;
-            const f16x2 hh = __builtin_convertvector(xs, f16x2);
-            const f16x2 mm = __builtin_convertvector(xs - __builtin_convertvector(hh, f32x2), f16x2);
-            hw[2 * h + u / 2] = __builtin_bit_cast(int, hh);
-            mw[2 * h + u / 2] = __builtin_bit_cast(int, mm);
-          }
+        } else {
+          dgr_tile_split(g.raw[rg][s][0], g.raw[rg][s][1], sx, relu_lo, hw, mw);
         }
-#pragma unroll
-        for (int d = 0; d < 4; ++d) {
-          hw[d] = __builtin_amdgcn_ds_bpermute(from, hw[d]);
-          mw[d] = __builtin_amdgcn_ds_bpermute(from, mw[d]);
-        }
-        bh[rg][s] = __builtin_bit_cast(f16x8, hw);
-        bm[rg][s] = __builtin_bit_cast(f16x8, mw);
+        bh[rg][s] = dgr_tile_to_operand(hw, from);
+        bm[rg][s] = dgr_tile_to_operand(mw, from);
       }
     }
     __builtin_amdgcn_sched_barrier(0);
@@ -211,13 +187,11 @@
     uint32_t mx = 0;
 #pragma unroll
     for (int cb = 0; cb < NCB; ++cb) {
-      f32x4 v = total[rg][cb];
-      v.x = fmaxf(v.x, out_lo); v.y = fmaxf(v.y, out_lo); v.z = fmaxf(v.z, out_lo); v.w = fmaxf(v.w, out_lo);
+      const f32x4 v = dgr_tile_max(total[rg][cb], out_lo);
       total[rg][cb] = v;
       if (row < n_out) {
         if (a.out) *reinterpret_cast<f32x4 *>(a.out + row * a.out_ld + 16 * cb + 4 * lq) = v;
-        const i32x4 b = __builtin_bit_cast(i32x4, v);
-        mx = max(mx, max(max((uint32_t)b.x & 0x7fffffffu, (uint32_t)b.y & 0x7fffffffu), max((uint32_t)b.z & 0x7fffffffu, (uint32_t)b.w & 0x7fffffffu)));
+        mx = max(mx, dgr_tile_absmax(v));
       }
     }
     if (a.out_amax || a.out_amax2 || a.out_ds) {
@@ -233,21 +207,10 @@
       unsigned char *dst = a.out_ds + row * (int64_t)(4 * COUT) + 16 * lq;
 #pragma unroll
       for (int s = 0; s < COUT / 32; ++s) {
-        u32x4 hw, mw;
-#pragma unroll
-        for (int h = 0; h < 2; ++h) {
-          const i32x4 v = __builtin_bit_cast(i32x4, total[rg][2 * s + h]);
-#pragma unroll
-          for (int u = 0; u < 4; u += 2) {
-            const f32x2 xs = f32x2{__builtin_bit_cast(float, max(v[u], out_relu_lo)), __builtin_bit_cast(float, max(v[u + 1], out_relu_lo))} * sx;
-            const f16x2 hh = __builtin_convertvector(xs, f16x2);
-            const f16x2 mm = __builtin_convertvector(xs - __builtin_convertvector(hh, f32x2), f16x2);
-            hw[2 * h + u / 2] = __builtin_bit_cast(uint32_t, hh);
-            mw[2 * h + u / 2] = __builtin_bit_cast(uint32_t, mm);
-          }
-        }
-        *reinterpret_cast<u32x4 *>(dst + 64 * s) = hw;
-        *reinterpret_cast<u32x4 *>(dst + 2 * COUT + 64 * s) = mw;
+        i32x4 hw, mw;
+        dgr_tile_split(total[rg][2 * s], total[rg][2 * s + 1], sx, out_relu_lo, hw, mw);
+        *reinterpret_cast<i32x4 *>(dst + 64 * s) = hw;
+        *reinterpret_cast<i32x4 *>(dst + 2 * COUT + 64 * s) = mw;
       }
     }
   }
diff --git a/deepglobalregistration_amd/csrc/conv_nbr.hip b/deepglobalregistration_amd/csrc/conv_nbr.hip
--- /dev/null
+++ b/deepglobalregistration_amd/csrc/conv_nbr.hip
@@ -0,0 +1,230 @@
+#include "dgr_internal.h"
+#include "conv_tile.h"
+
+struct ConvNbrArgs {
+  const float *in;
+  float *out;
+  const float *shift, *res;
+  const u32x4 *wb;
+  int64_t piece_stride;
+  const int32_t *nbr, *n_out_dev;
+  int64_t n_pad;
+  int in_ld, in_relu, out_ld, out_relu, res_ld, res_relu;
+  const uint32_t *row_amax;
+  uint32_t *out_amax, *out_amax2;
+  float w_unscale;
+  uint32_t in_bytes;
+};
+
+template <int CIN, int COUT, int RG, int WAVES>
+__global__ void __launch_bounds__(64 * WAVES, 2) sparse_conv_nbr_f16x2(ConvNbrArgs a) {
+  constexpr int KV = 27;
+  constexpr int NCB = 4;
+  constexpr int SPC = CIN >= 64 ? 2 : 1;
+  constexpr int NCH = CIN / (32 * SPC);
+  constexpr int S_T = CIN / 32;
+  constexpr int NB16 = COUT / 16;
+  constexpr int THREADS = 64 * WAVES;
+  constexpr int MB = WAVES * RG * 16;
+  constexpr int NST = SPC * NCB;
+  constexpr int WD = NST;
+  constexpr int NIT = KV * NCH;
+  __shared__ int nbr_s[KV][MB];
+
+  const int tid = threadIdx.x, lane = tid & 63;
+  const int wave = __builtin_amdgcn_readfirstlane(tid >> 6);
+  const int slice = blockIdx.y;
+  const int n_out = *a.n_out_dev;
+  const int nblocks = (n_out + MB - 1) / MB;
+  const int per = (nblocks + 7) >> 3;
+  const int jx = blockIdx.x >> 3;
+  const int blk = (blockIdx.x & 7) * per + jx;
+  if (jx >= per || blk >= nblocks) return;
+  const int64_t row0 = (int64_t)blk * MB;
+
+  for (int e = tid; e < KV * MB; e += THREADS) {
+    const int k = e / MB, r = e - k * MB;
+    nbr_s[k][r] = (row0 + r < n_out) ? a.nbr[(int64_t)k * a.n_pad + row0 + r] : -1;
+  }
+
+  u32x4 rh[WD], rm[WD];
+  const u32x4 *wph = a.wb + lane, *wpm = a.wb + a.piece_stride + lane;
+  auto wreq = [&](int g, int i) {
+    const int gc = min(g, NIT * NST - 1);
+    const int it = gc / NST, jj = gc - it * NST;
+    const int k = it / NCH, ch = it - k * NCH;
+    const int64_t frag = ((int64_t)k * S_T + SPC * ch + (jj % SPC)) * NB16 + slice * NCB + (jj / SPC);
+    rh[i] = wph[frag * 64];
+    rm[i] = wpm[frag * 64];
+  };
+  const int lr = lane & 15, lq = lane >> 4;
+  f32x4 total[RG][NCB];
+#pragma unroll
+  for (int cb = 0; cb < NCB; ++cb) {
+    const int col = 64 * slice + 16 * cb + 4 * lq;
+    const f32x4 sh = a.shift ? *reinterpret_cast<const f32x4 *>(a.shift + col) : f32x4{0.f, 0.f, 0.f, 0.f};
+#pragma unroll
+    for (int rg = 0; rg < RG; ++rg) {
+      f32x4 v = sh;
+      const int64_t row = row0 + (wave * RG + rg) * 16 + lr;
+      if (a.res && row < n_out) {
+        f32x4 x = *reinterpret_cast<const f32x4 *>(a.res + row * a.res_ld + col);
+        if (a.res_relu) x = dgr_tile_max(x, 0.f);
+        v += x;
+      }
+      total[rg][cb] = v;
+    }
+  }
+  __syncthreads();
+
+  const __amdgpu_buffer_rsrc_t in_rsrc = __builtin_amdgcn_make_buffer_rsrc(const_cast<float *>(a.in), 0, a.in_bytes, 0x00020000);
+  struct RowSet { f32x4 raw[RG][SPC][2]; uint32_t mx[RG]; int nv[RG]; };
+  auto gather = [&](int it, RowSet &g) {
+    const int k = it / NCH, ch = it - k * NCH;
+#pragma unroll
+    for (int rg = 0; rg < RG; ++rg) {
+      const int n = nbr_s[k][(wave * RG + rg) * 16 + (lane >> 2)];
+      const int ne = max(n, 0);
+      const uint32_t off = n >= 0 ? (uint32_t)n * (uint32_t)(a.in_ld * 4) + (uint32_t)(128 * SPC) * ch + 16u * (lane & 3) : a.in_bytes;
+      const uint32_t mv = a.row_amax[ne];
+#pragma unroll
+      for (int s = 0; s < SPC; ++s) {
+        g.raw[rg][s][0] = __builtin_bit_cast(f32x4, __builtin_amdgcn_raw_buffer_load_b128(in_rsrc, off + 128 * s, 0, 0));
+        g.raw[rg][s][1] = __builtin_bit_cast(f32x4, __builtin_amdgcn_raw_buffer_load_b128(in_rsrc, off + 128 * s + 64, 0, 0));
+      }
+      g.mx[rg] = mv;
+      g.nv[rg] = n;
+    }
+  };
+  RowSet gA;
+  gather(0, gA);
+#pragma unroll
+  for (int i = 0; i < WD; ++i) wreq(i, i);
+  const int relu_lo = a.in_relu ? 0 : (int)0x80000000;
+  const int from = dgr_tile_perm_from(lane);
+
+  f32x4 tmp[RG][NCB];
+#pragma unroll 1
+  for (int it = 0; it < NIT; ++it) {
+    const int ch = it % NCH;
+    f16x8 bh[RG][SPC], bm[RG][SPC];
+    float fold[RG];
+#pragma unroll
+    for (int rg = 0; rg < RG; ++rg) {
+      const float sx = dgr_tile_row_scale(gA.nv[rg], gA.mx[rg]);
+      fold[rg] = dgr_tile_fold(sx, a.w_unscale, lane);
+#pragma unroll
+      for (int s = 0; s < SPC; ++s) {
+        i32x4 hw, mw;
+        dgr_tile_split(gA.raw[rg][s][0], gA.raw[rg][s][1], sx, relu_lo, hw, mw);
+        bh[rg][s] = dgr_tile_to_operand(hw, from);
+        bm[rg][s] = dgr_tile_to_operand(mw, from);
+      }
+    }
+    __builtin_amdgcn_sched_barrier(0);
+    gather(min(it + 1, NIT - 1), gA);
+    __builtin_amdgcn_sched_barrier(0);
+    if (NCH == 1 || ch == 0) {
+#pragma unroll
+      for (int rg = 0; rg < RG; ++rg)
+#pragma unroll
+        for (int cb = 0; cb < NCB; ++cb) tmp[rg][cb] = f32x4{0.f, 0.f, 0.f, 0.f};
+    }
+#pragma unroll
+    for (int cb = 0; cb < NCB; ++cb) {
+#pragma unroll
+      for (int s = 0; s < SPC; ++s) {
+        const int j = cb * SPC + s;
+        const f16x8 wh = __builtin_bit_cast(f16x8, rh[j]);
+        const f16x8 wm = __builtin_bit_cast(f16x8, rm[j]);
+#pragma unroll
+        for (int rg = 0; rg < RG; ++rg) tmp[rg][cb] = __builtin_amdgcn_mfma_f32_16x16x32_f16(wm, bh[rg][s], tmp[rg][cb], 0, 0, 0);
+#pragma unroll
+        for (int rg = 0; rg < RG; ++rg) tmp[rg][cb] = __builtin_amdgcn_mfma_f32_16x16x32_f16(wh, bm[rg][s], tmp[rg][cb], 0, 0, 0);
+#pragma unroll
+        for (int rg = 0; rg < RG; ++rg) tmp[rg][cb] = __builtin_amdgcn_mfma_f32_16x16x32_f16(wh, bh[rg][s], tmp[rg][cb], 0, 0, 0);
+        wreq((it + 1) * NST + j, j);
+        __builtin_amdgcn_sched_barrier(0);
+      }
+    }
+    if (NCH == 1 || ch == NCH - 1) {
+#pragma unroll
+      for (int rg = 0; rg < RG; ++rg)
+#pragma unroll
+        for (int cb = 0; cb < NCB; ++cb) total[rg][cb] += tmp[rg][cb] * fold[rg];
+    }
+  }
+
+  const float out_lo = a.out_relu ? 0.f : -__builtin_inff();
+#pragma unroll
+  for (int rg = 0; rg < RG; ++rg) {
+    const int64_t row = row0 + (wave * RG + rg) * 16 + lr;
+    uint32_t mx = 0;
+    if (row < n_out) {
+#pragma unroll
+      for (int cb = 0; cb < NCB; ++cb) {
+        const f32x4 v = dgr_tile_max(total[rg][cb], out_lo);
+        *reinterpret_cast<f32x4 *>(a.out + row * a.out_ld + 64 * slice + 16 * cb + 4 * lq) = v;
+        mx = max(mx, dgr_tile_absmax(v));
+      }
+    }
+    if (a.out_amax || a.out_amax2) {
+      mx = max(mx, (uint32_t)__shfl_xor((int)mx, 16, 64));
+      mx = max(mx, (uint32_t)__shfl_xor((int)mx, 32, 64));
+      if (lq == 0 && row < n_out) {
+        if (a.out_amax) atomicMax(a.out_amax + row, mx);
+        if (a.out_amax2) atomicMax(a.out_amax2 + row, mx);
+      }
+    }
+  }
+}
+
+static constexpr int NBR_RG = 2, NBR_WAVES = 4;
+static const int NBR_SHAPES[][2] = {{128, 128}, {256, 256}, {32, 64}, {64, 128}, {128, 256}};
+
+bool dgr_conv_nbr_supported(int cin, int cin_pad, int cout) {
+  for (const auto &s : NBR_SHAPES)
+    if (cin == cin_pad && s[0] == cin && s[1] == cout) return true;
+  return false;
+}
+int dgr_conv_nbr_rows_per_block(int cin, int cout) { return dgr_conv_nbr_supported(cin, cin, cout) ? NBR_WAVES * NBR_RG * 16 : 0; }
+
+template <int CIN, int COUT>
+static int launch_nbr(const ConvNbrArgs &ka, int64_t n_out_cap, hipStream_t stream) {
+  constexpr int RG = NBR_RG, WAVES = NBR_WAVES, MB = WAVES * RG * 16;
+  int64_t blocks = dgr_ceil_div(n_out_cap, MB);
+  blocks = (blocks + 7) / 8 * 8;
+  const dim3 grid((unsigned)blocks, (unsigned)(COUT / 64));
+  sparse_conv_nbr_f16x2<CIN, COUT, RG, WAVES><<<grid, 64 * WAVES, 0, stream>>>(ka);
+  DGR_LAUNCH_CHECK();
+  return DGR_OK;
+}
+
+int dgr_conv_nbr_launch(const DgrConvOsLaunch &a, hipStream_t stream, const char **kernel_name) {
+  DGR_REQUIRE(a.nbr && a.nbr->built && a.nbr->K == 27, "neighbour-table dense-tile conv: no neighbour table");
+  DGR_REQUIRE(dgr_conv_nbr_supported(a.cin, a.cin_pad, a.cout), "neighbour-table dense-tile conv: Cin = %d, Cout = %d not built", a.cin, a.cout);
+  DGR_REQUIRE(a.wbd && a.row_amax, "neighbour-table dense-tile conv: needs the split weights in the dense-tile operand order and the input rows' maxima");
+  DGR_REQUIRE(a.out, "neighbour-table dense-tile conv: no output");
+  DGR_REQUIRE((a.in_ld & 3) == 0 && (a.out_ld & 3) == 0 && (a.res == nullptr || (a.res_ld & 3) == 0),
+              "neighbour-table dense-tile conv: row strides must be multiples of 4");
+  DGR_REQUIRE(a.in_ld >= a.cin && a.out_ld >= a.cout, "neighbour-table dense-tile conv: row strides below the channel counts");
+  DGR_REQUIRE(a.n_in_cap > 0 && a.n_in_cap * (int64_t)a.in_ld * 4 < (1ll << 31), "neighbour-table dense-tile conv: input tensor beyond 2 GB");
+  DGR_REQUIRE(a.n_out_cap <= a.nbr->n_pad, "neighbour-table dense-tile conv: neighbour table smaller than the output map");
+  ConvNbrArgs ka;
+  ka.in = a.in; ka.out = a.out; ka.shift = a.shift; ka.res = a.res;
+  ka.wb = static_cast<const u32x4 *>(a.wbd); ka.piece_stride = a.piece_stride;
+  ka.nbr = a.nbr->nbr; ka.n_out_dev = a.n_out_dev; ka.n_pad = a.nbr->n_pad;
+  ka.in_ld = a.in_ld; ka.in_relu = a.in_relu; ka.out_ld = a.out_ld; ka.out_relu = a.out_relu;
+  ka.res_ld = a.res_ld; ka.res_relu = a.res_relu;
+  ka.row_amax = a.row_amax; ka.out_amax = a.out_amax; ka.out_amax2 = a.out_amax2;
+  ka.w_unscale = a.w_unscale;
+  ka.in_bytes = (uint32_t)(a.n_in_cap * (int64_t)a.in_ld * 4);
+#define DGR_NBR(CI, CO)                                                                   \
+  if (a.cin == CI && a.cout == CO) {                                                      \
+    if (kernel_name) *kernel_name = "sparse_conv_nbr_f16x2<" #CI ", " #CO ">";            \
+    return launch_nbr<CI, CO>(ka, a.n_out_cap, stream);                                   \
+  }
+  DGR_NBR(128, 128) DGR_NBR(256, 256) DGR_NBR(32, 64) DGR_NBR(64, 128) DGR_NBR(128, 256)
+#undef DGR_NBR
+  return DGR_EINVAL;
+}
diff --git a/deepglobalregistration_amd/csrc/conv_os.hip b/deepglobalregistration_amd/csrc/conv_os.hip
--- a/deepglobalregistration_amd/csrc/conv_os.hip
+++ b/deepglobalregistration_amd/csrc/conv_os.hip
@@ -331,6 +331,7 @@
 int dgr_conv_os_launch(const DgrConvOsLaunch &a, hipStream_t stream, const char **kernel_name) {
   if (a.dense) return dgr_conv_dense_launch(a, stream, kernel_name);
   if (a.up) return dgr_conv_up_launch(a, stream, kernel_name);
+  if (a.tiles) return dgr_conv_nbr_launch(a, stream, kernel_name);
   DGR_REQUIRE(a.nbr && a.nbr->built && a.nbr->K == 27, "output-stationary conv: no neighbour table");
   DGR_REQUIRE((a.cin & 3) == 0 && (a.in_ld & 3) == 0 && (a.out_ld & 3) == 0 && (a.res == nullptr || (a.res_ld & 3) == 0),
               "output-stationary conv: channel counts and row strides must be multiples of 4");
diff --git a/deepglobalregistration_amd/csrc/conv_tile.h b/deepglobalregistration_amd/csrc/conv_tile.h
--- /dev/null
+++ b/deepglobalregistration_amd/csrc/conv_tile.h
@@ -0,0 +1,48 @@
+#pragma once
+#include "split.h"
+
+typedef float f32x4 __attribute__((ext_vector_type(4)));
+typedef float f32x2 __attribute__((ext_vector_type(2)));
+typedef int i32x4 __attribute__((ext_vector_type(4)));
+typedef _Float16 f16x8 __attribute__((ext_vector_type(8)));
+typedef _Float16 f16x2 __attribute__((ext_vector_type(2)));
+typedef unsigned int u32x2 __attribute__((ext_vector_type(2)));
+typedef unsigned int u32x4 __attribute__((ext_vector_type(4)));
+
+__device__ __forceinline__ int dgr_tile_perm_from(int lane) { return 4 * (4 * (lane & 15) + (lane >> 4)); }
+
+__device__ __forceinline__ void dgr_tile_split(const f32x4 &r0, const f32x4 &r1, float sx, int lo, i32x4 &hw, i32x4 &mw) {
+#pragma unroll
+  for (int h = 0; h < 2; ++h) {
+    const i32x4 v = __builtin_bit_cast(i32x4, h == 0 ? r0 : r1);
+#pragma unroll
+    for (int u = 0; u < 4; u += 2) {
+      const f32x2 xs = f32x2{__builtin_bit_cast(float, max(v[u], lo)), __builtin_bit_cast(float, max(v[u + 1], lo))} * sx;
+      const f16x2 hh = __builtin_convertvector(xs, f16x2);
+      const f16x2 mm = __builtin_convertvector(xs - __builtin_convertvector(hh, f32x2), f16x2);
+      hw[2 * h + u / 2] = __builtin_bit_cast(int, hh);
+      mw[2 * h + u / 2] = __builtin_bit_cast(int, mm);
+    }
+  }
+}
+
+__device__ __forceinline__ f16x8 dgr_tile_to_operand(i32x4 w, int from) {
+#pragma unroll
+  for (int d = 0; d < 4; ++d) w[d] = __builtin_amdgcn_ds_bpermute(from, w[d]);
+  return __builtin_bit_cast(f16x8, w);
+}
+
+__device__ __forceinline__ float dgr_tile_row_scale(int nv, uint32_t mx) { return nv >= 0 ? dgr_row_scale_of(mx) : 0.f; }
+__device__ __forceinline__ float dgr_tile_fold(float sx, float w_unscale, int lane) {
+  const float fl = sx != 0.f ? dgr_inv_pow2(sx) * w_unscale : 0.f;
+  return __builtin_bit_cast(float, __builtin_amdgcn_ds_bpermute(16 * (lane & 15), __builtin_bit_cast(int, fl)));
+}
+
+__device__ __forceinline__ uint32_t dgr_tile_absmax(const f32x4 &v) {
+  const i32x4 b = __builtin_bit_cast(i32x4, v);
+  return max(max((uint32_t)b.x & 0x7fffffffu, (uint32_t)b.y & 0x7fffffffu), max((uint32_t)b.z & 0x7fffffffu, (uint32_t)b.w & 0x7fffffffu));
+}
+__device__ __forceinline__ f32x4 dgr_tile_max(f32x4 v, float lo) {
+  v.x = fmaxf(v.x, lo); v.y = fmaxf(v.y, lo); v.z = fmaxf(v.z, lo); v.w = fmaxf(v.w, lo);
+  return v;
+}
diff --git a/deepglobalregistration_amd/csrc/conv_up.hip b/deepglobalregistration_amd/csrc/conv_up.hip
--- a/deepglobalregistration_amd/csrc/conv_up.hip
+++ b/deepglobalregistration_amd/csrc/conv_up.hip
@@ -1,12 +1,5 @@
 #include "dgr_internal.h"
-#include "split.h"
-
-typedef float f32x4 __attribute__((ext_vector_type(4)));
-typedef float f32x2 __attribute__((ext_vector_type(2)));
-typedef int i32x4 __attribute__((ext_vector_type(4)));
-typedef _Float16 f16x8 __attribute__((ext_vector_type(8)));
-typedef _Float16 f16x2 __attribute__((ext_vector_type(2)));
-typedef unsigned int u32x4 __attribute__((ext_vector_type(4)));
+#include "conv_tile.h"
 
 struct ConvUpArgs {
   const float *in;
@@ -127,34 +120,17 @@
     const int ch = it % NCH;
     f16x8 bh[RG][2], bm[RG][2];
     float fold[RG];
-    const int from = 4 * (4 * (lane & 15) + (lane >> 4));
+    const int from = dgr_tile_perm_from(lane);
 #pragma unroll
     for (int rg = 0; rg < RG; ++rg) {
-      const float sx = gA.nv[rg] >= 0 ? dgr_row_scale_of(gA.mx[rg]) : 0.f;
-      const float fl = sx != 0.f ? dgr_inv_pow2(sx) * a.w_unscale : 0.f;
-      fold[rg] = __builtin_bit_cast(float, __builtin_amdgcn_ds_bpermute(16 * (lane & 15), __builtin_bit_cast(int, fl)));
+      const float sx = dgr_tile_row_scale(gA.nv[rg], gA.mx[rg]);
+      fold[rg] = dgr_tile_fold(sx, a.w_unscale, lane);
 #pragma unroll
       for (int s = 0; s < 2; ++s) {
         i32x4 hw, mw;
-#pragma unroll
-        for (int h = 0; h < 2; ++h) {
-          const i32x4 v = __builtin_bit_cast(i32x4, gA.raw[rg][s][h]);
-#pragma unroll
-          for (int u = 0; u < 4; u += 2) {
-            const f32x2 xs = f32x2{__builtin_bit_cast(float, max(v[u], relu_lo)), __builtin_bit_cast(float, max(v[u + 1], relu_lo))} * sx;
-            const f16x2 hh = __builtin_convertvector(xs, f16x2);
-            const f16x2 mm = __builtin_convertvector(xs - __builtin_convertvector(hh, f32x2), f16x2);
-            hw[2 * h + u / 2] = __builtin_bit_cast(int, hh);
-            mw[2 * h + u / 2] = __builtin_bit_cast(int, mm);
-          }
-        }
-#pragma unroll
-        for (int d = 0; d < 4; ++d) {
-          hw[d] = __builtin_amdgcn_ds_bpermute(from, hw[d]);
-          mw[d] = __builtin_amdgcn_ds_bpermute(from, mw[d]);
-        }
-        bh[rg][s] = __builtin_bit_cast(f16x8, hw);
-        bm[rg][s] = __builtin_bit_cast(f16x8, mw);
+        dgr_tile_split(gA.raw[rg][s][0], gA.raw[rg][s][1], sx, relu_lo, hw, mw);
+        bh[rg][s] = dgr_tile_to_operand(hw, from);
+        bm[rg][s] = dgr_tile_to_operand(mw, from);
       }
     }
     __builtin_amdgcn_sched_barrier(0);
@@ -199,11 +175,9 @@
     if (row >= 0) {
 #pragma unroll
       for (int cb = 0; cb < NCB; ++cb) {
-        f32x4 v = total[rg][cb];
-        v.x = fmaxf(v.x, out_lo); v.y = fmaxf(v.y, out_lo); v.z = fmaxf(v.z, out_lo); v.w = fmaxf(v.w, out_lo);
+        const f32x4 v = dgr_tile_max(total[rg][cb], out_lo);
         *reinterpret_cast<f32x4 *>(a.out + row * a.out_ld + 64 * slice + 16 * cb + 4 * lq) = v;
-        const i32x4 b = __builtin_bit_cast(i32x4, v);
-        mx = max(mx, max(max((uint32_t)b.x & 0x7fffffffu, (uint32_t)b.y & 0x7fffffffu), max((uint32_t)b.z & 0x7fffffffu, (uint32_t)b.w & 0x7fffffffu)));
+        mx = max(mx, dgr_tile_absmax(v));
       }
     }
     if (a.out_amax || a.out_amax2) {
diff --git a/deepglobalregistration_amd/csrc/dgr_internal.h b/deepglobalregistration_amd/csrc/dgr_internal.h
--- a/deepglobalregistration_amd/csrc/dgr_internal.h
+++ b/deepglobalregistration_amd/csrc/dgr_internal.h
@@ -203,6 +203,7 @@
   int cin, cin_pad, cout;
   bool dense = false;
   bool up = false;
+  bool tiles = false;
   const unsigned char *in_dsplit = nullptr;
   unsigned char *out_dsplit = nullptr;
 };
@@ -211,6 +212,9 @@
 int dgr_conv_dense_launch(const DgrConvOsLaunch &a, hipStream_t stream, const char **kernel_name = nullptr);
 bool dgr_conv_up_supported(int cin, int cin_pad, int cout);
 int dgr_conv_up_launch(const DgrConvOsLaunch &a, hipStream_t stream, const char **kernel_name = nullptr);
+bool dgr_conv_nbr_supported(int cin, int cin_pad, int cout);
+int dgr_conv_nbr_rows_per_block(int cin, int cout);
+int dgr_conv_nbr_launch(const DgrConvOsLaunch &a, hipStream_t stream, const char **kernel_name = nullptr);
 int dgr_l2_normalize_rows(const float *in, int in_ld, float *out, int out_ld, int c, int relu,
                           const int32_t *n_dev, int64_t n_cap, hipStream_t stream);
 
diff --git a/deepglobalregistration_amd/csrc/net.hip b/deepglobalregistration_amd/csrc/net.hip
--- a/deepglobalregistration_amd/csrc/net.hip
+++ b/deepglobalregistration_amd/csrc/net.hip
@@ -93,6 +93,25 @@
     if (name == w[i].name) return &w[i];
   return nullptr;
 }
+
+struct NbrRoute { int cin, cout, strided, routed; };
+static const NbrRoute NBR_ROUTES[] = {
+    {128, 128, 0, 1},
+    {256, 256, 0, 0},
+    {32, 64, 1, 1},
+    {64, 128, 1, 1},
+    {128, 256, 1, 0},
+};
+static int nbr_route(int cin, int cout, int strided, bool weights) {
+  if (dgr_exact_f32() || getenv("DGR_NO_NBR") || getenv("DGR_OS_LISTS")) return 0;
+  const bool all = getenv("DGR_NBR_ALL") != nullptr;
+  for (const NbrRoute &r : NBR_ROUTES)
+    if (r.cin == cin && r.cout == cout && (weights || r.strided == (strided != 0)))
+      return (r.routed || all) && dgr_conv_nbr_supported(cin, cin, cout);
+  return 0;
+}
+extern "C" int dgr_conv_nbr_routed(int cin, int cout, int strided) { return nbr_route(cin, cout, strided, false); }
+extern "C" int dgr_conv_nbr_block_rows(int cin, int cout) { return dgr_conv_nbr_rows_per_block(cin, cout); }
 
 template <class F>
 __global__ void __launch_bounds__(256) dgr_fill_kernel(int64_t n, F f) {
@@ -283,7 +302,8 @@
         pcs[ne + o] = dgr_f16_bits_dev(xs - dgr_f16_val_dev(xs));
       }));
       W.param_bytes += (size_t)2 * ne * sizeof(uint16_t);
-      if (net->D == 3 && K == 27 && (dgr_conv_dense_supported(cin, L.cin_pad, cout) || dgr_conv_up_supported(cin, L.cin_pad, cout))) {
+      if (net->D == 3 && K == 27 && (dgr_conv_dense_supported(cin, L.cin_pad, cout) || dgr_conv_up_supported(cin, L.cin_pad, cout) ||
+                                     (cin == L.cin_pad && nbr_route(cin, cout, 0, true)))) {
         uint16_t *pd;
         DGR_CHECK(W.alloc(&pd, (size_t)2 * ne));
         L.w16d = pd;
@@ -516,6 +536,10 @@
       static const bool no_up = getenv("DGR_NO_UP") != nullptr;
       o.up = swapped && !o.dense && !no_up && !os_lists && o.row_amax && o.wbd && t->perm && res == nullptr &&
              dgr_conv_up_supported(L.cin, L.cin_pad, L.cout) && cin_map.n_cap * (int64_t)in.ld * 4 < (1ll << 31);
+      bool strided_down = false;
+      for (int l = 0; l < 3; ++l) strided_down = strided_down || t == &ms.ndown[l];
+      o.tiles = !o.dense && !o.up && (same_stride || strided_down) && o.row_amax && o.wbd && L.cin == L.cin_pad &&
+                dgr_conv_nbr_routed(L.cin, L.cout, strided_down) && cin_map.n_cap * (int64_t)in.ld * 4 < (1ll << 31);
       if (o.dense) {
         o.in_dsplit = in.dsplit;
         o.out_dsplit = out.dsplit;
@@ -868,22 +892,23 @@
   return DGR_OK;
 }
 
-extern "C" int dgr_debug_conv_layer(dgr_ctx *ctx, dgr_net *net, int layer, const int32_t *coords, const float *in,
-                                    int in_relu, int64_t N, float *out, dgr_stream stream_) {
+static int debug_conv_layer(dgr_ctx *ctx, dgr_net *net, int layer, const int32_t *coords, const float *in, int in_relu,
+                            int64_t N, int strided, const float *res, int res_relu, float *out, int32_t *out_coords,
+                            int64_t *n_out, hipStream_t stream) {
   DGR_REQUIRE(ctx && net && coords && in && out && N > 0, "dgr_debug_conv_layer: bad argument");
   DGR_REQUIRE(layer >= 0 && layer < (int)net->W->layers.size(), "layer %d out of range", layer);
   const DgrLayer &L = net->W->layers[layer];
   int k3 = 1;
   for (int d = 0; d < net->D; ++d) k3 *= 3;
   DGR_REQUIRE(L.K == k3 && L.cin >= 32, "dgr_debug_conv_layer: layer %s is not a 3^D conv with >= 32 input channels", L.name.c_str());
-  hipStream_t stream = (hipStream_t)stream_;
+  DGR_REQUIRE((!strided && !res) || net->D == 3, "dgr_debug_conv_layer: strided map / residual input with the 3-D net only");
   DGR_HIP_CHECK(hipSetDevice(ctx->device));
   DGR_CHECK(ctx->arena.reset());
   DGR_CHECK(dgr_ctx_new_flag(ctx, stream));
   dgr_ctx_begin_profile(ctx);
   DgrArena &A = ctx->arena;
   Fwd f;
-  f.ctx = ctx; f.net = net; f.stream = stream; f.prof = false;
+  f.ctx = ctx; f.net = net; f.stream = stream; f.prof = ctx->profiling;
   f.ms.overflow = ctx->flag_dev;
   DGR_CHECK(dgr_build_maps(A, coords, N, net->D, 3, &f.ms, stream, false, true, net->D == 3));
   const int64_t n_cap = f.ms.cm[0].n_cap;
@@ -895,10 +920,39 @@
     DGR_ALLOC(tin.split.scale, A, float, n_cap);
     DGR_CHECK(dgr_split_rows(in, L.cin, in_relu, f.ms.cm[0].n_dev, n_cap, tin.split, stream));
   }
-  DGR_CHECK(f.conv(layer, tin, &f.ms.same[0], false, 0, 0, tout, nullptr));
+  const Tensor tres{const_cast<float *>(res), L.cout, res_relu};
+  const int lvl_out = strided ? 1 : 0;
+  DGR_CHECK(f.conv(layer, tin, strided ? &f.ms.down[0] : &f.ms.same[0], false, 0, lvl_out, tout, res ? &tres : nullptr));
+  const DgrCoordMap &om = f.ms.cm[lvl_out];
+  if (out_coords)
+    DGR_HIP_CHECK(hipMemcpyAsync(out_coords, om.coords, (size_t)om.n_cap * (1 + net->D) * sizeof(int32_t), hipMemcpyDeviceToDevice, stream));
+  int32_t *n_pin = nullptr;
+  if (n_out) {
+    unsigned char *pin;
+    DGR_CHECK(dgr_ctx_pinned(ctx, 128, &pin));
+    n_pin = reinterpret_cast<int32_t *>(pin + 64);
+    DGR_HIP_CHECK(hipMemcpyAsync(n_pin, om.n_dev, sizeof(int32_t), hipMemcpyDeviceToHost, stream));
+  }
   DGR_CHECK(dgr_ctx_check_flag(ctx, stream));
+  if (n_out) *n_out = *reinterpret_cast<volatile int32_t *>(n_pin);
+  if (ctx->profiling) {
+    memset(ctx->stage_ms, 0, sizeof(ctx->stage_ms));
+    DGR_CHECK(dgr_ctx_collect_profile(ctx));
+  }
   dgr_net_invalidate_runs(net);
   return DGR_OK;
+}
+
+extern "C" int dgr_debug_conv_layer(dgr_ctx *ctx, dgr_net *net, int layer, const int32_t *coords, const float *in,
+                                    int in_relu, int64_t N, float *out, dgr_stream stream_) {
+  return debug_conv_layer(ctx, net, layer, coords, in, in_relu, N, 0, nullptr, 0, out, nullptr, nullptr, (hipStream_t)stream_);
+}
+
+extern "C" int dgr_debug_conv_layer_ex(dgr_ctx *ctx, dgr_net *net, int layer, const int32_t *coords, const float *in,
+                                       int in_relu, int64_t N, int strided, const float *res, int res_relu, float *out,
+                                       int32_t *out_coords, int64_t *n_out, dgr_stream stream_) {
+  return debug_conv_layer(ctx, net, layer, coords, in, in_relu, N, strided, res, res_relu, out, out_coords, n_out,
+                          (hipStream_t)stream_);
 }
 
 extern "C" int dgr_net_get_intermediate(dgr_ctx *ctx, dgr_net *net, const char *name, float *host_out,
diff --git a/deepglobalregistration_amd/ops.py b/deepglobalregistration_amd/ops.py
--- a/deepglobalregistration_amd/ops.py
+++ b/deepglobalregistration_amd/ops.py
@@ -144,6 +144,30 @@
         check(lay.dgr_debug_conv_layer(get_ctx(dev), self.handle, int(layer), ptr(coords), ptr(feats), int(bool(relu)),
                                        coords.shape[0], ptr(out), stream_ptr(dev.index)))
         return out
+
+    def debug_conv_layer_ex(self, layer, coords, feats, relu=False, strided=False, res=None, res_relu=False):
+        dev = self.device
+        coords = _as(coords, torch.int32, dev)
+        feats = _as(feats, torch.float32, dev)
+        lay = _lib.load()
+        N = coords.shape[0]
+        cout = self.debug_layer_width(layer)
+        out = torch.zeros((N, cout), dtype=torch.float32, device=dev)
+        oc = torch.zeros((N, coords.shape[1]), dtype=torch.int32, device=dev)
+        if res is not None:
+            res = _as(res, torch.float32, dev)
+            if res.shape != (N, cout) or strided:
+                raise ValueError('res must be [N, Cout] of a same-stride layer')
+        n_out = C.c_int64(0)
+        check(lay.dgr_debug_conv_layer_ex(get_ctx(dev), self.handle, int(layer), ptr(coords), ptr(feats), int(bool(relu)), N,
+                                          int(bool(strided)), ptr(res) if res is not None else None, int(bool(res_relu)),
+                                          ptr(out), ptr(oc), C.byref(n_out), stream_ptr(dev.index)))
+        return (out[:n_out.value], oc[:n_out.value]) if strided else out
+
+    def debug_layer_width(self, layer):
+        ch, tr = [None, 32, 64, 128, 256], [None, 64, 64, 64, 128]
+        widths = [ch[1]] * 3 + [ch[2]] * 3 + [ch[3]] * 3 + [ch[4]] * 3 + [tr[4]] * 3 + [tr[3]] * 3 + [tr[2]] * 3 + [tr[1], self.cout]
+        return widths[layer]
 
     def rerun_layer(self, layer, reps=5):
         lib = _lib.load()
diff --git a/include/dgr_hip.h b/include/dgr_hip.h
--- a/include/dgr_hip.h
+++ b/include/dgr_hip.h
@@ -201,6 +201,11 @@
 
 int dgr_debug_conv_layer(dgr_ctx *ctx, dgr_net *net, int layer, const int32_t *coords, const float *in, int in_relu,
                          int64_t N, float *out, dgr_stream stream);
+int dgr_debug_conv_layer_ex(dgr_ctx *ctx, dgr_net *net, int layer, const int32_t *coords, const float *in, int in_relu,
+                            int64_t N, int strided, const float *res, int res_relu, float *out, int32_t *out_coords,
+                            int64_t *n_out, dgr_stream stream);
+int dgr_conv_nbr_routed(int cin, int cout, int strided);
+int dgr_conv_nbr_block_rows(int cin, int cout);
 
 #ifdef __cplusplus
 }
```

Result: faster. 390.8 (median of 6 runs) (+2.1%).
